# genome-vendor/bsmap

Measured on AMD Instinct MI355X. Metric: aligned reads/sec (whole node), 2x150 bp hg38 WGBS -v 6 -s 16, higher is better.
Workload: dtype u32; 1 GPU; C3: 2x150(->144) bp PE WGBS vs hg38-sized synthetic genome, -s 16 -v 6 -I 4 -m 28 -x 500; genome_bp=3088269832, index_entries=1475952693, parallelism=read-sharded x1, batches_in_flight=2, exact_mode=False, resident_ring_steps=4, records_flagged_BSX_F_LIMIT=0

## Files before the change

### bsmap_amd/csrc/bsx_align.hip

```cpp
#include "bsx_internal.h"
#include "bsx_dev.h"
#include "bsx_groups.h"
#include "bsx_rows.h"
#include "bsx_kernel_args.h"

namespace {

typedef unsigned long long u64;

struct __attribute__((packed, aligned(4))) U4 { uint32_t a, b, c, d; };
struct __attribute__((packed, aligned(4))) U2 { uint32_t a, b; };

#ifndef BSX_MAIN_NT
#define BSX_MAIN_NT 0
#endif
#ifndef BSX_MAIN_PREFETCH
#define BSX_MAIN_PREFETCH 1
#endif
typedef uint32_t v4u_a4 __attribute__((ext_vector_type(4), aligned(4)));
typedef uint32_t v2u_a4 __attribute__((ext_vector_type(2), aligned(4)));
__device__ __forceinline__ U4 ldm4(const uint32_t *p)
{
#if BSX_MAIN_NT
    const v4u_a4 v = __builtin_nontemporal_load(reinterpret_cast<const v4u_a4 *>(p));
    return U4{v.x, v.y, v.z, v.w};
#else
    return *reinterpret_cast<const U4 *>(p);
#endif
}
__device__ __forceinline__ U2 ldm2(const uint32_t *p)
{
#if BSX_MAIN_NT
    const v2u_a4 v = __builtin_nontemporal_load(reinterpret_cast<const v2u_a4 *>(p));
    return U2{v.x, v.y};
#else
    return *reinterpret_cast<const U2 *>(p);
#endif
}
__device__ __forceinline__ uint32_t ldm1(const uint32_t *p)
{
#if BSX_MAIN_NT
    return __builtin_nontemporal_load(p);
#else
    return *p;
#endif
}

__device__ __forceinline__ unsigned long long bsx_ballot(bool p) { return __builtin_amdgcn_ballot_w64(p); }
#define mad30(x, c) ({ uint32_t d_; asm("v_mad_u32_u24 %0, %1, 30, " #c : "=v"(d_) : "v"(x)); d_; })
__device__ __forceinline__ uint32_t rfl(uint32_t x) { return __builtin_amdgcn_readfirstlane(x); }
__device__ __forceinline__ uint32_t rl(uint32_t x, int l) { return __builtin_amdgcn_readlane(x, l); }
__device__ __forceinline__ uint32_t rl_u(uint32_t x, uint32_t l) { return __builtin_amdgcn_readlane(x, (int)__builtin_amdgcn_readfirstlane(l)); }
__device__ __forceinline__ u64 rl64(u64 x, int l) { return ((u64)rl((uint32_t)(x >> 32), l) << 32) | rl((uint32_t)x, l); }
__device__ __forceinline__ u64 lanemask_lt(int lane) { return lane ? (~0ull >> (64 - lane)) : 0ull; }
__device__ __forceinline__ void wave_fence() { __builtin_amdgcn_fence(__ATOMIC_SEQ_CST, "workgroup"); }

__device__ __forceinline__ int wave_argmin_u32(uint32_t v)
{
    uint32_t r = v;
#define BSX_DPP_MIN(ctrl) r = min(r, (uint32_t)__builtin_amdgcn_update_dpp((int)0xffffffffu, (int)r, ctrl, 0xf, 0xf, false))
    BSX_DPP_MIN(0x111); BSX_DPP_MIN(0x112); BSX_DPP_MIN(0x114); BSX_DPP_MIN(0x118);
#undef BSX_DPP_MIN
    const uint32_t m = min(min(rl(r, 15), rl(r, 31)), min(rl(r, 47), rl(r, 63)));
    return m == 0xffffffffu ? -1 : (int)__builtin_ctzll(bsx_ballot(v == m));
}
__device__ __forceinline__ uint32_t wave_sum(uint32_t v)
{
#pragma unroll
    for (int o = 32; o; o >>= 1) v += __shfl_xor(v, o);
    return v;
}

struct MateU {
    int len, raw_len, max_snp, seedseg, filtered;
    int nfull;
    uint32_t flags;
    uint32_t snp_thres;
    uint32_t nkeys;
    uint32_t index;
    int defer;
    uint32_t pad;
};
struct MateLds {
    uint8_t seq[160];
    uint8_t qual[160];
    uint32_t w[2][10], m[2][10];
    uint32_t cnt[2][160];
    uint8_t start[2][16];
    uint8_t order[2][16];
    uint32_t stale_key[2][16];
    uint8_t stale_so[2];
    MateU u, u2;
    __attribute__((aligned(16))) uint32_t fl[4][8];
};

template <bool PE> struct WaveLds { MateLds mate[PE ? 2 : 1]; };

struct BlockLds {
    uint8_t prof[16][16];
    uint8_t nt_tab[256];
    uint32_t anchor[BSX_LDS_CHR + 1], chr_size[BSX_LDS_CHR], rc_offset[BSX_LDS_CHR];
};

typedef __attribute__((address_space(3))) MateU LdsMateU;
struct Mate {
    LdsMateU *u;
    uint32_t cnt_reg;
    uint32_t key_reg;
    uint32_t bloom0, bloom1;
};
__device__ __forceinline__ LdsMateU *lds_mate(MateU *p) { return (LdsMateU *)p; }

struct Slab {
    u64 *hits;
    uint32_t *keys;
    uint32_t *kslot;
    uint32_t *hset;
    u64 *tmp;
    uint32_t rowcap, nclass;
    uint32_t kcap, hbits;
    __device__ __forceinline__ u64 *list(int orient, int w) const { return hits + ((size_t)(orient * (nclass + 1) + w)) * rowcap; }
};

struct Counters { u64 n_lookup, n_cand, sum_w, n_orient; };

__device__ __forceinline__ int nt_idx(uint32_t c)
{
    c |= 0x20;
    return c == 'a' ? 0 : c == 'c' ? 1 : c == 'g' ? 2 : c == 't' ? 3 : -1;
}

__device__ __forceinline__ uint32_t n_of(const Mate &M, int orient, int w) { return rl(M.cnt_reg, orient * 16 + w); }

__device__ void load_and_filter(const AlignArgs &A, MateLds &L, Mate &M, int mate, long j, int lane)
{
    const DevParams &P = A.P;
    const bool hist = j < 0;
    const uint64_t *off = hist ? A.hist_off[mate] : A.off[mate];
    const uint64_t jj = hist ? (uint64_t)((long)A.n_hist + j) : (uint64_t)j;
    const uint64_t b = off[jj], e = off[jj + 1];
    int len = (int)min((uint64_t)P.max_readlen, e - b);
    const uint8_t *sq = hist ? A.hist_seq[mate] : A.seq[mate], *qq = hist ? A.hist_qual[mate] : A.qual[mate];
    const uint8_t *s = sq + b, *q = qq ? qq + b : nullptr;
    for (int i = lane; i < 160; i += 64) {
        L.seq[i] = i < len ? s[i] : 0;
        L.qual[i] = (q && i < len) ? q[i] : 0;
    }
    wave_fence();
    M.u->raw_len = len;
    M.u->filtered = 0;
    if (P.n_adapter > 0 && len >= 5) {
        bool done = false;
        for (int a = 0; a < P.n_adapter && !done; a++) {
            const int al = P.adapter_len[a];
            for (int base = P.seed_size; base < len - (P.rrbs ? 5 : 4) && !done; base += 64) {
                const int pos = base + lane;
                bool hit = false;
// ... 2152 lines not shown
    uint32_t *bits = g_sector_bits;
    if (!bits) return;
    uint32_t prev = 0xffffffffu, touches = 0;
    for (int i = 0; i < n16; i++)
        for (uint32_t b = byte_off + 16u * (uint32_t)i; b <= byte_off + 16u * (uint32_t)i + 15u; b += 15u) {
            const uint32_t sct = b >> 6;
            if (sct == prev) continue;
            prev = sct; touches++;
            if (!((bits[sct >> 5] >> (sct & 31u)) & 1u)) atomicOr(&bits[sct >> 5], 1u << (sct & 31u));
        }
    const unsigned long long tw = (unsigned long long)wave_sum(touches);
    if ((threadIdx.x & 63) == 0) atomicAdd(&g_sector_touch, tw);
}
__global__ __launch_bounds__(256) void k_sector_pop(uint32_t n_words)
{
    unsigned long long c = 0;
    for (uint32_t i = blockIdx.x * 256 + threadIdx.x; i < n_words; i += gridDim.x * 256) { const uint32_t w = g_sector_bits[i]; if (w) { c += (unsigned long long)__popc(w); g_sector_bits[i] = 0; } }
    for (int o = 32; o; o >>= 1) c += __shfl_xor(c, o);
    if ((threadIdx.x & 63) == 0 && c) atomicAdd(&g_sector_distinct, c);
    if (blockIdx.x == 0 && threadIdx.x == 0) atomicAdd(&g_sector_passes, 1ull);
}
#endif

template <bool RRBS, int XP = 0>
__device__ __forceinline__ SameChunk same_load(const SameWin &W, const SameEntry &e)
{
    static_assert(XP >= 0 && XP <= 2, "r3 holds two pairs");
    SameChunk c;
    uint32_t off = W.ref_off;
    if (RRBS) {
        const uint32_t rchr = e.a & 0xffffu;
        c.valid = e.in && ((e.a ^ W.tag_xor) >> 16) == W.tag_want && e.b >= W.h;
        c.pm1 = c.valid ? W.anchor[rchr >> 1] + (e.b - W.h) - 1u : 31u;
        c.strand = rchr & 1u;
        off = c.strand ? W.rc_off : 0u;
    } else { c.valid = e.in; c.pm1 = e.a + W.h - 1u; c.strand = 0; }
    const uint8_t *src = W.plane + hp_boff(c.pm1, off);
    c.r0 = *reinterpret_cast<const U4 *>(src);
    c.r1.a = c.r1.b = c.r1.c = c.r1.d = 0; c.r2.a = c.r2.b = c.r2.c = c.r2.d = 0;
    if (W.nwr > 1) c.r1 = *reinterpret_cast<const U4 *>(src + 16);
    if (W.nwr > 3) c.r2 = *reinterpret_cast<const U4 *>(src + 32);
    c.r3.a = c.r3.b = c.r3.c = c.r3.d = 0;
    if (XP == 1) { const U2 x = *reinterpret_cast<const U2 *>(src + 48); c.r3.a = x.a; c.r3.b = x.b; }
    if (XP == 2) c.r3 = *reinterpret_cast<const U4 *>(src + 48);
#ifdef BSX_SECTOR_STATS
    if (c.valid) sector_mark(hp_boff(c.pm1, off), W.nwr > 3 ? 3 : W.nwr > 1 ? 2 : 1); else sector_mark(0u, 0);
#endif
    return c;
}

template <int NWR, bool PLAIN, bool SKIP, bool STATS>
__device__ __forceinline__ void same_counts(const uint32_t (&flo)[5], const uint32_t (&fhi)[5], uint32_t him, int nwr_rt, const uint4 &a0, const uint4 &a1, const uint4 &a2,
                                            const uint4 &a3, uint32_t thr, u64 alive, uint32_t &w0ref, uint32_t &w01ref, uint32_t &tot)
{
    static_assert(NWR != 0 || !PLAIN, "the plain form needs the word count");
    const int nwr = NWR ? NWR : nwr_rt;
#define SAME_MM(j, X, Y, M) ((PLAIN && (j) < NWR - 1) ? bsx_plane_mismatch_full(flo[j], fhi[j], X, Y) : bsx_plane_mismatch(flo[j], fhi[j], X, Y, M))
    const uint32_t m0 = SAME_MM(0, a0.x, a0.y, a0.z);
    const uint32_t c0 = __popc(m0);
    w0ref = STATS ? __popc(m0 & him) : 0u; tot = c0; w01ref = c0;
    if (nwr > 1) {
        const uint32_t m1 = SAME_MM(1, a0.w, a1.x, a1.y);
        tot = popc_acc(m1, c0); if (STATS) w01ref = popc_acc(m1 & him, c0);
        if (nwr > 2 && (!SKIP || (bsx_ballot(tot <= thr) & alive))) {
            tot = popc_acc(SAME_MM(2, a1.z, a1.w, a2.x), tot);
            if (nwr > 3) {
                tot = popc_acc(SAME_MM(3, a2.z, a2.w, a3.x), tot);
                if (nwr > 4) tot = popc_acc(SAME_MM(4, a3.y, a3.z, a3.w), tot);
            }
        }
    }
#undef SAME_MM
}

template <bool PLAIN>
__device__ __forceinline__ uint32_t same_word(int j, const uint32_t (&flo)[5], const uint32_t (&fhi)[5], const uint4 &a0, const uint4 &a1, const uint4 &a2, const uint4 &a3)
{
    uint32_t X, Y, M;
    switch (j) {
    case 0: X = a0.x; Y = a0.y; M = a0.z; break;
    case 1: X = a0.w; Y = a1.x; M = a1.y; break;
    case 2: X = a1.z; Y = a1.w; M = a2.x; break;
    case 3: X = a2.z; Y = a2.w; M = a3.x; break;
    default: X = a3.y; Y = a3.z; M = a3.w; break;
    }
    return (PLAIN && j < 4) ? bsx_plane_mismatch_full(flo[j], fhi[j], X, Y) : bsx_plane_mismatch(flo[j], fhi[j], X, Y, M);
}
template <bool PLAIN, bool FULL>
__device__ __forceinline__ u64 same_exit(const uint32_t (&flo)[5], const uint32_t (&fhi)[5], const uint4 &a0, const uint4 &a1, const uint4 &a2, const uint4 &a3,
                                         uint32_t thr, u64 valid, uint32_t &tot, uint32_t &words)
{
    u64 bp = 0;
    tot = 0;
#define SAME_STEP(i, j)                                                                \
    tot = popc_acc(same_word<PLAIN>(j, flo, fhi, a0, a1, a2, a3), tot);                \
    words = (i) + 1;                                                                   \
    if ((i) == 4 || ((HG_EXIT >> (i)) & 1)) {                                          \
        bp = bsx_ballot(tot <= thr);                                                   \
        if (!FULL) bp &= valid;                                                        \
        if (!bp) return 0;                                                             \
    }
    SAME_STEP(0, 0) SAME_STEP(1, 4) SAME_STEP(2, 3) SAME_STEP(3, 2) SAME_STEP(4, 1)
#undef SAME_STEP
    return bp;
}

template <int NWR, bool RRBS, bool PLAIN, bool FULL, bool STATS>
__device__ __forceinline__ void hs_eval_read(const uint32_t (&flo)[HG_C][5], const uint32_t (&fhi)[HG_C][5], const uint32_t (&him)[HG_C], const u64 (&vm)[HG_C],
                                             const uint32_t (&ordsh)[HG_C], const uint32_t (&hchr)[HG_C], const uint32_t (&hloc)[HG_C], int nwr, const uint4 &a0, const uint4 &a1,
                                             const uint4 &a2, const uint4 &a3, uint32_t thr, SurvRec *sv, uint32_t &nsk, uint32_t &add15)
{
#pragma unroll
    for (int u = 0; u < HG_C; u++) {
        uint32_t w0ref = 0, w01ref = 0, tot;
        u64 bp;
        if (HG_EXIT && !STATS && !RRBS && NWR == 5) {
            uint32_t words;
            bp = same_exit<PLAIN, FULL>(flo[u], fhi[u], a0, a1, a2, a3, thr, vm[u], tot, words);
#ifdef BSX_SCAN_WORDS
            if (vm[u]) add15 += 1u + (words << 16);
#else
            (void)words;
#endif
        } else {
            same_counts<NWR, PLAIN, RRBS, STATS>(flo[u], fhi[u], him[u], nwr, a0, a1, a2, a3, thr, vm[u], w0ref, w01ref, tot);
            bp = bsx_ballot(tot <= thr);
            if (!FULL) bp &= vm[u];
        }
        if (STATS) {
            u64 b1 = bsx_ballot(w0ref > thr), b5 = bsx_ballot(w01ref <= thr);
            if (!FULL) { b1 &= vm[u]; b5 &= vm[u]; }
            add15 += (uint32_t)__builtin_popcountll(b1) + ((uint32_t)__builtin_popcountll(b5) << 16);
        }
        if (bp) {
            const uint32_t pos = __builtin_amdgcn_mbcnt_hi((uint32_t)(bp >> 32), __builtin_amdgcn_mbcnt_lo((uint32_t)bp, nsk));
            if (__builtin_amdgcn_inverse_ballot_w64(bp) && pos < HS_SCAP) { SurvRec r; r.w_ord = tot | ordsh[u]; r.hchr = hchr[u]; r.hloc = hloc[u]; r.hkey = 0; sv[pos] = r; }
            nsk += (uint32_t)__builtin_popcountll(bp);
        }
    }
}

template <bool PLAIN, bool SPLIT>
__device__ __forceinline__ uint32_t lean_word(int i, const uint32_t (&flo)[5], const uint32_t (&fhi)[5], const uint4 &q0, const uint4 &q1, const uint4 &q2, const uint4 &q3)
{
    const int j = bsx_row_eval_word(i);
    if (!SPLIT) return same_word<PLAIN>(j, flo, fhi, q0, q1, q2, q3);
    uint32_t X, Y, M;
    bsx_row_word(i, q0, q1, q2, q3, X, Y, M);
    return (PLAIN && j < 4) ? bsx_plane_mismatch_full(flo[j], fhi[j], X, Y) : bsx_plane_mismatch(flo[j], fhi[j], X, Y, M);
}
template <bool PLAIN, bool FULL, bool SPLIT, int JOINT>
__device__ __forceinline__ void hs_eval_lean(const HeavyArgs &H, const uint32_t (&flo)[HG_C][5], const uint32_t (&fhi)[HG_C][5], const u64 (&vm)[HG_C], const uint32_t (&hloc)[HG_C],
                                             const uint4 &q0, const uint4 &q1, const uint4 &p2, const uint4 &p3, const uint4 *row, uint32_t thr, uint32_t k, uint32_t tid, uint32_t &nsv,
                                             int lane, uint32_t cb, uint32_t dcur, uint32_t strand, uint32_t &dgw)
{
    u64 al[HG_C];
    uint32_t tot[HG_C];
    uint4 q2 = p2, q3 = p3;
#pragma unroll
    for (int u = 0; u < HG_C; u++) { al[u] = FULL ? ~0ull : vm[u]; tot[u] = 0; }
#ifdef BSX_SCAN_WORDS
#pragma unroll
    for (int u = 0; u < HG_C; u++) if (al[u]) dgw += 1u;
#define LEAN_DG dgw += 1u << 16;
#else
#define LEAN_DG
#endif
#define LEAN_WORD(u, i) {                                                                                \
        tot[u] = popc_acc(lean_word<PLAIN, SPLIT>(i, flo[u], fhi[u], q0, q1, q2, q3), tot[u]);           \
        const u64 b_ = bsx_ballot(tot[u] <= thr);                                                        \
        al[u] = (FULL && JOINT < 2) ? b_ : (b_ & al[u]);                                                 \
        LEAN_DG }
#define LEAN_ANY() (al[0] | al[1] | al[2] | al[3])
#define LEAN_HALF() asm volatile("" : "+v"(q2.x), "+v"(q2.y), "+v"(q2.z), "+v"(q2.w), "+v"(q3.x), "+v"(q3.y), "+v"(q3.z), "+v"(q3.w));
    static_assert(HG_C == 4, "written out for four chunks");
    if (JOINT == 3 && FULL) {
#pragma unroll
        for (int i = 0; i < 5; i++) {
            if (SPLIT && i == 2) { q2 = row[2]; q3 = row[3]; LEAN_HALF() }
#pragma unroll
            for (int u = 0; u < HG_C; u++) { tot[u] = popc_acc(lean_word<PLAIN, SPLIT>(i, flo[u], fhi[u], q0, q1, q2, q3), tot[u]); LEAN_DG }
            if (HG_JOINT_FIRST && i == 0) continue;
            if (!bsx_ballot(min(min(tot[0], tot[1]), min(tot[2], tot[3])) <= thr)) return;
        }
#pragma unroll
        for (int u = 0; u < HG_C; u++) al[u] = bsx_ballot(tot[u] <= thr);
    } else if (JOINT) {
#pragma unroll
        for (int i = 0; i < 5; i++) {
            if (SPLIT && i == 2) { q2 = row[2]; q3 = row[3]; LEAN_HALF() }
#pragma unroll
            for (int u = 0; u < HG_C; u++) if (JOINT >= 2 || al[u]) LEAN_WORD(u, i)
            if (HG_JOINT_FIRST && i == 0) continue;
            if (!LEAN_ANY()) return;
        }
    } else {
#pragma unroll
        for (int u = 0; u < HG_C; u++) if (al[u]) { LEAN_WORD(u, 0) if (al[u]) LEAN_WORD(u, 1) }
        if (!LEAN_ANY()) return;
        if (SPLIT) { q2 = row[2]; q3 = row[3]; LEAN_HALF() }
#pragma unroll
        for (int u = 0; u < HG_C; u++) if (al[u]) { LEAN_WORD(u, 2) if (al[u]) { LEAN_WORD(u, 3) if (al[u]) LEAN_WORD(u, 4) } }
        if (!LEAN_ANY()) return;
    }
#undef LEAN_WORD
#undef LEAN_ANY
#undef LEAN_HALF
#undef LEAN_DG
    SurvRec *const sv = H.tout[rl_u(tid, k)].surv;
    uint32_t nsk = rl_u(nsv, k);
#pragma unroll
    for (int u = 0; u < HG_C; u++) {
        const u64 bp = al[u];
        if (bp) {
            const uint32_t pos = __builtin_amdgcn_mbcnt_hi((uint32_t)(bp >> 32), __builtin_amdgcn_mbcnt_lo((uint32_t)bp, nsk));
            if (__builtin_amdgcn_inverse_ballot_w64(bp) && pos < HS_SCAP) {
                SurvRec r; r.w_ord = tot[u] | ((cb + (uint32_t)(u * 64 + lane)) << 8); r.hchr = strand; r.hloc = hloc[u] + 32u * dcur; r.hkey = 0; sv[pos] = r;
            }
            nsk += (uint32_t)__builtin_popcountll(bp);
        }
    }
    if ((uint32_t)lane == k) nsv = nsk;
}

template <int NWR, bool RRBS, bool STATS>
__device__ __forceinline__ void hs_group(const AlignArgs &A, const HeavyArgs &H, SameLds &L, int lane, int wv, uint32_t K, uint32_t tid, uint32_t th, uint32_t tc0,
                                         uint32_t key, uint32_t n, uint32_t hh, uint32_t sub_h, uint32_t flags, uint32_t tag_xor, uint32_t tag_want)
{
    const DevParams &P = A.P;
    uint32_t *uw = &L.W[wv].UW[0][0];
    const int nwr = NWR ? NWR : (int)((flags >> 8) & 15u);
    constexpr int XD = (!RRBS && NWR == 5) ? HG_D : 0, XP = XD;
    static_assert(HG_D >= 0 && HG_D <= 2 && 6 + HG_D <= BSX_PLANE_PAD, "the gather holds two pairs more at most, and stays inside the pad behind the strand copy");
    constexpr bool LEAN = HG_LEAN && HG_EXIT == 15 && NWR == 5 && !RRBS && !STATS, SPLIT = LEAN && HG_SPLIT;
    static_assert(BSX_ROW_DWORDS == 20 && sizeof(L.W[0].UW[0]) == 4 * BSX_ROW_DWORDS, "bsx_rows.h describes a row of SameLds");
#ifdef BSX_SIGHIST_DUPS
    u64 rowsig = 0;
#endif
#ifdef BSX_SCAN_CLOCKS
    constexpr bool CLK = NWR == 5 && !RRBS && !STATS;
    u64 ck_gather = 0, ck_reads = 0;
    const u64 ck_begin = __builtin_amdgcn_s_memtime();
#endif
    if ((uint32_t)lane < K) {
        const ListReq &R = H.state[th & 0x3fffffffu].req[th >> 30];
        uint32_t *row = uw + (uint32_t)lane * 20u;
        uint32_t inner = 0xFFFFFFFFu;
#pragma unroll
        for (int j = 0; j < 5; j++) {
            const int f = 3 * j, o = j < 3 ? 0 : 1;
            const uint32_t pm = R.pm[j];
            if (!SPLIT) { row[f + o] = R.px[j]; row[f + 1 + o] = R.py[j]; row[f + 2 + o] = pm; }
            if (j < nwr - 1) inner &= pm;
        }
        const uint32_t tword = R.thres | (inner == 0xFFFFFFFFu ? 0x10000u : 0u) | (XD ? ((sub_h - hh) >> 5) << 17 : 0u);
        if (SPLIT) bsx_row_pack(row, R.px, R.py, R.pm, tword);
        else row[9] = tword;
        row[BSX_ROW_TASK] = tid; row[BSX_ROW_ORD] = tc0;
#ifdef BSX_SIGHIST_DUPS
        u64 hsh = R.thres;
#pragma unroll
        for (int j = 0; j < 5; j++) { hsh = (hsh ^ R.px[j]) * 0x9E3779B97F4A7C15ull; hsh = (hsh ^ R.py[j]) * 0xBF58476D1CE4E5B9ull; hsh = (hsh ^ R.pm[j]) * 0x94D049BB133111EBull; hsh ^= hsh >> 29; }
        rowsig = hsh;
#endif
    }
    uint32_t n_dup = 0; (void)n_dup;
#ifdef BSX_SIGHIST_DUPS
    for (uint32_t j = 1; j < K; j++) {
        const u64 sj = ((u64)rl_u((uint32_t)(rowsig >> 32), j) << 32) | rl_u((uint32_t)rowsig, j);
        if (bsx_ballot((uint32_t)lane < j && rowsig == sj)) n_dup++;
    }
#endif
    wave_fence();
    const uint32_t strand = flags & 1u;
    SameWin W;
    W.ent = P.entries + (RRBS ? 2u * (size_t)key : (size_t)key); W.n = n; W.h = hh; W.tag_xor = tag_xor; W.tag_want = tag_want; W.rc_off = P.plane_rc_off;
    W.ref_off = strand ? P.plane_rc_off : 0u; W.anchor = P.anchor; W.plane = reinterpret_cast<const uint8_t *>(P.refplane); W.nwr = nwr;
    uint32_t c15 = 0, nsv = 0;
    uint32_t n_cand = 0;
#ifdef BSX_SCAN_WORDS
    u64 dg_ev = 0, dg_words = 0;
#endif
    constexpr uint32_t STEP = 64u * HG_C;
    SameChunk nx[HG_C];
    SameEntry en[HG_C];
#if HG_PREFETCH
#pragma unroll
    for (int u = 0; u < HG_C; u++) nx[u] = same_load<RRBS, XP>(W, same_entry<RRBS>(W, (uint32_t)(u * 64 + lane)));
#pragma unroll
    for (int u = 0; u < HG_C; u++) en[u] = same_entry<RRBS>(W, STEP + (uint32_t)(u * 64 + lane));
#pragma unroll
    for (int u = 0; u < HG_C; u++) asm volatile("" :: "v"(nx[u].r0.a), "v"(nx[u].r1.a), "v"(nx[u].r2.a));
#else
#pragma unroll
    for (int u = 0; u < HG_C; u++) en[u] = same_entry<RRBS>(W, (uint32_t)(u * 64 + lane));
#endif
    for (uint32_t cb = 0; cb < n; cb += STEP) {
#ifdef BSX_SCAN_CLOCKS
        __builtin_amdgcn_sched_barrier(0);
        const u64 ck_step = __builtin_amdgcn_s_memtime();
        __builtin_amdgcn_sched_barrier(0);
#endif
#if !HG_PREFETCH
#pragma unroll
        for (int u = 0; u < HG_C; u++) nx[u] = same_load<RRBS, XP>(W, en[u]);
#pragma unroll
        for (int u = 0; u < HG_C; u++) en[u] = same_entry<RRBS>(W, cb + STEP + (uint32_t)(u * 64 + lane));
#endif
        uint32_t flo[HG_C][5], fhi[HG_C][5], xlo[HG_C][XD ? XD : 1], xhi[HG_C][XD ? XD : 1], him[HG_C], hloc[HG_C], ordsh[HG_C], hchr[HG_C];
        u64 vm[HG_C];
#pragma unroll
        for (int u = 0; u < HG_C; u++) {
            const SameChunk &c = nx[u];
            const uint32_t wd[16] = {c.r0.a, c.r0.b, c.r0.c, c.r0.d, c.r1.a, c.r1.b, c.r1.c, c.r1.d, c.r2.a, c.r2.b, c.r2.c, c.r2.d, c.r3.a, c.r3.b, c.r3.c, c.r3.d};
            const uint32_t shf = 31u - (c.pm1 & 31u);
            him[u] = 0xFFFFFFFFu << ((c.pm1 + 1u) & 15u);
#pragma unroll
            for (int t = 0; t < 5; t++) { flo[u][t] = __builtin_amdgcn_alignbit(wd[2 * t], wd[2 * t + 2], shf); fhi[u][t] = __builtin_amdgcn_alignbit(wd[2 * t + 1], wd[2 * t + 3], shf); }
#pragma unroll
            for (int t = 5; t < 5 + XD; t++) { xlo[u][t - 5] = __builtin_amdgcn_alignbit(wd[2 * t], wd[2 * t + 2], shf); xhi[u][t - 5] = __builtin_amdgcn_alignbit(wd[2 * t + 1], wd[2 * t + 3], shf); }
            if (!XD) xlo[u][0] = xhi[u][0] = 0;
            hloc[u] = c.pm1 + 1u;
            hchr[u] = RRBS ? c.strand : strand;
            ordsh[u] = (cb + (uint32_t)(u * 64 + lane)) << 8;
            vm[u] = bsx_ballot(c.valid);
            if (RRBS) n_cand += (uint32_t)__builtin_popcountll(vm[u]);
        }
#if HG_PREFETCH
        if (cb + STEP < n) {
#pragma unroll
            for (int u = 0; u < HG_C; u++) nx[u] = same_load<RRBS, XP>(W, en[u]);
#pragma unroll
            for (int u = 0; u < HG_C; u++) en[u] = same_entry<RRBS>(W, cb + 2u * STEP + (uint32_t)(u * 64 + lane));
        }
#endif
        const bool full = !RRBS && cb + STEP <= n;
#ifdef BSX_SCAN_CLOCKS
#pragma unroll
        for (int u = 0; u < HG_C; u++) asm volatile("" :: "v"(flo[u][0]), "v"(fhi[u][4]), "v"(xlo[u][XD ? XD - 1 : 0]), "v"(xhi[u][XD ? XD - 1 : 0]));
        __builtin_amdgcn_sched_barrier(0);
        const u64 ck_frame = __builtin_amdgcn_s_memtime();
        __builtin_amdgcn_sched_barrier(0);
        ck_gather += ck_frame - ck_step;
#endif
#if HG_ROWPF
        uint4 p0, p1, p2, p3 = make_uint4(0u, 0u, 0u, 0u);
        { const uint4 *row = reinterpret_cast<const uint4 *>(uw); p0 = row[0]; p1 = row[1]; p2 = row[2]; if (nwr > 3) p3 = row[3]; }
#endif
        uint32_t dcur = 0;
        if constexpr (LEAN) {
            const uint4 *const rows = reinterpret_cast<const uint4 *>(uw);
            const uint4 zero4 = make_uint4(0u, 0u, 0u, 0u);
            auto one_read = [&](uint32_t k, const uint4 &h0, const uint4 &h1) __attribute__((always_inline)) {
                const uint4 *const row = rows + k * 5u;
                uint4 q0 = h0, q1 = h1, p2 = zero4, p3 = zero4;
                if (!SPLIT) { q0 = row[0]; q1 = row[1]; p2 = row[2]; p3 = row[3]; }
                const uint32_t tp = rfl(SPLIT ? bsx_row_t(q0) : p2.y), thr = tp & 0xffffu;
                const bool plain = ((tp >> 16) & 1u) != 0;
                for (; dcur < (tp >> 17); dcur++) {
#pragma unroll
                    for (int u = 0; u < HG_C; u++) {
#pragma unroll
                        for (int t = 0; t < 4; t++) { flo[u][t] = flo[u][t + 1]; fhi[u][t] = fhi[u][t + 1]; }
                        flo[u][4] = xlo[u][0]; fhi[u][4] = xhi[u][0];
#pragma unroll
                        for (int t = 0; t + 1 < XD; t++) { xlo[u][t] = xlo[u][t + 1]; xhi[u][t] = xhi[u][t + 1]; }
                    }
                }
                uint32_t dgw = 0;
                if (full) {
                    if (plain) hs_eval_lean<true, true, SPLIT, HG_JOINT>(H, flo, fhi, vm, hloc, q0, q1, p2, p3, row, thr, k, tid, nsv, lane, cb, dcur, strand, dgw);
                    else hs_eval_lean<false, true, SPLIT, HG_JOINT>(H, flo, fhi, vm, hloc, q0, q1, p2, p3, row, thr, k, tid, nsv, lane, cb, dcur, strand, dgw);
                } else {
                    if (plain) hs_eval_lean<true, false, SPLIT, HG_JOINT>(H, flo, fhi, vm, hloc, q0, q1, p2, p3, row, thr, k, tid, nsv, lane, cb, dcur, strand, dgw);
                    else hs_eval_lean<false, false, SPLIT, HG_JOINT>(H, flo, fhi, vm, hloc, q0, q1, p2, p3, row, thr, k, tid, nsv, lane, cb, dcur, strand, dgw);
                }
#ifdef BSX_SCAN_WORDS
                dg_ev += dgw & 0xffffu; dg_words += dgw >> 16;
#else
                (void)dgw;
#endif
            };
            if (SPLIT) {
                uint4 a0 = rows[0], a1 = rows[1], b0, b1;
                for (uint32_t k = 0;; k += 2) {
                    { const uint4 *const nr = rows + min(k + 1u, K - 1u) * 5u; b0 = nr[0]; b1 = nr[1]; }
                    one_read(k, a0, a1);
                    if (k + 1 >= K) break;
                    { const uint4 *const nr = rows + min(k + 2u, K - 1u) * 5u; a0 = nr[0]; a1 = nr[1]; }
                    one_read(k + 1, b0, b1);
                    if (k + 2 >= K) break;
                }
            } else
                for (uint32_t k = 0; k < K; k++) one_read(k, zero4, zero4);
        } else
        for (uint32_t k = 0; k < K; k++) {
#if HG_ROWPF
            const uint4 a0 = p0, a1 = p1, a2 = p2, a3 = p3;
            if (k + 1 < K) { const uint4 *row = reinterpret_cast<const uint4 *>(uw + (k + 1u) * 20u); p0 = row[0]; p1 = row[1]; p2 = row[2]; if (nwr > 3) p3 = row[3]; }
#else
            const uint4 *row = reinterpret_cast<const uint4 *>(uw + k * 20u);
            const uint4 a0 = row[0], a1 = row[1], a2 = row[2];
            uint4 a3 = make_uint4(0u, 0u, 0u, 0u);
            if (nwr > 3) a3 = row[3];
#endif
            const uint32_t tp = rfl(a2.y), thr = tp & 0xffffu;
            const bool plain = NWR != 0 && ((tp >> 16) & 1u) != 0;
            if (XD) {
                for (; dcur < (tp >> 17); dcur++) {
#pragma unroll
                    for (int u = 0; u < HG_C; u++) {
#pragma unroll
                        for (int t = 0; t < 4; t++) { flo[u][t] = flo[u][t + 1]; fhi[u][t] = fhi[u][t + 1]; }
                        flo[u][4] = xlo[u][0]; fhi[u][4] = xhi[u][0];
#pragma unroll
                        for (int t = 0; t + 1 < XD; t++) { xlo[u][t] = xlo[u][t + 1]; xhi[u][t] = xhi[u][t + 1]; }
                        hloc[u] += 32u;
                    }
                }
            }
            SurvRec *const sv = H.tout[rl_u(tid, k)].surv;
            uint32_t nsk = rl_u(nsv, k), add15 = 0;
            if (full) {
                if (plain) hs_eval_read<NWR, RRBS, NWR != 0, !RRBS, STATS>(flo, fhi, him, vm, ordsh, hchr, hloc, nwr, a0, a1, a2, a3, thr, sv, nsk, add15);
                else hs_eval_read<NWR, RRBS, false, !RRBS, STATS>(flo, fhi, him, vm, ordsh, hchr, hloc, nwr, a0, a1, a2, a3, thr, sv, nsk, add15);
            } else {
                if (plain) hs_eval_read<NWR, RRBS, NWR != 0, false, STATS>(flo, fhi, him, vm, ordsh, hchr, hloc, nwr, a0, a1, a2, a3, thr, sv, nsk, add15);
                else hs_eval_read<NWR, RRBS, false, false, STATS>(flo, fhi, him, vm, ordsh, hchr, hloc, nwr, a0, a1, a2, a3, thr, sv, nsk, add15);
            }
            if ((uint32_t)lane == k) { if (STATS) c15 += add15; nsv = nsk; }
#ifdef BSX_SCAN_WORDS
            if (!STATS) { dg_ev += add15 & 0xffffu; dg_words += add15 >> 16; }
#endif
        }
#ifdef BSX_SCAN_CLOCKS
        asm volatile("" :: "v"(nsv));
        __builtin_amdgcn_sched_barrier(0);
        ck_reads += __builtin_amdgcn_s_memtime() - ck_frame;
        __builtin_amdgcn_sched_barrier(0);
#endif
    }
    wave_fence();
    if (!RRBS) n_cand = n;
    const bool mine = (uint32_t)lane < K;
    const uint32_t n1 = c15 & 0xffffu, n5 = c15 >> 16, ns = nsv;
    const bool ov = ns > HS_SCAP;
    if (mine) {
        HTaskOut *o = &H.tout[tid];
        o->count = min(ns, (uint32_t)HS_SCAP); o->overflow = ov ? 1 : 0; o->acc[0] = n_cand; o->acc[1] = STATS ? 2u * n_cand - n1 + 3u * n5 : 0u; o->acc[2] = 0; o->acc[3] = 0; o->c0 = tc0; o->n = n;
    }
    const bool cnt = mine && !ov;
    const uint32_t kk = (uint32_t)__builtin_popcountll(bsx_ballot(cnt));
    const uint32_t s1 = wave_sum(cnt ? n1 : 0), s5 = wave_sum(cnt ? n5 : 0);
    if (lane == 0 && kk) {
        u64 *sh = (u64 *)A.scan_stats + (size_t)((blockIdx.x * (uint32_t)HG_WPB + (uint32_t)wv) & 63u) * 8;
        atomicAdd((u64 *)&sh[0], (u64)kk * n_cand);
        if (STATS) { atomicAdd((u64 *)&sh[1], 2ull * kk * n_cand - s1 + 3ull * s5); atomicAdd((u64 *)&sh[2], (u64)s1); atomicAdd((u64 *)&sh[3], (u64)s5); }
        if (K > 1) atomicAdd((u64 *)&sh[4], (u64)kk * n_cand);
#if !defined(BSX_SCAN_WORDS) && !defined(BSX_SCAN_CLOCKS)
        atomicAdd((u64 *)&sh[5], (u64)kk * n_cand * K); if (K >= 4) atomicAdd((u64 *)&sh[6], (u64)kk * n_cand); if (n_dup) atomicAdd((u64 *)&sh[7], (u64)n_dup * n_cand);
#endif
    }
#ifdef BSX_SCAN_WORDS
    if (lane == 0 && dg_ev) {
        u64 *sh = (u64 *)A.scan_stats;
        atomicAdd((u64 *)&sh[5], dg_ev); atomicAdd((u64 *)&sh[6], dg_words);
    }
#endif
#ifdef BSX_SCAN_CLOCKS
    if (CLK && lane == 0) {
        u64 *sh = (u64 *)A.scan_stats;
        atomicAdd((u64 *)&sh[5], ck_gather); atomicAdd((u64 *)&sh[6], ck_reads); atomicAdd((u64 *)&sh[7], (u64)__builtin_amdgcn_s_memtime() - ck_begin);
    }
#endif
    wave_fence();
}

template <bool STATS>
__global__ __launch_bounds__(64 * HG_WPB, BSX_HSAME_WAVES) void k_hscan_same(AlignArgs A, HeavyArgs H)
{
    __shared__ SameLds L;
    const int lane = threadIdx.x & 63, wv = (int)rfl(threadIdx.x >> 6);
    const uint32_t n_big = min(H.glist[H.task_cap], H.task_cap), n_groups = min(n_big + H.glist[H.task_cap + 1], H.task_cap);
    const uint32_t nvb = (n_groups + HG_WPB - 1) / HG_WPB;
    for (uint32_t vb = blockIdx.x;; vb += gridDim.x) {
        uint32_t b_;
        const int st_ = bsx_order_block(vb, nvb, H.xcd_map >= 2 ? max(2u, H.xcd_map * BSX_HSCAN_WPB / (HG_XCD_DIV * HG_WPB)) : H.xcd_map, b_);
        if (st_ == 2) break;
        if (st_ == 1) continue;
        const uint32_t g = b_ * HG_WPB + (uint32_t)wv;
        if (g >= n_groups) continue;
        const uint32_t slot = rfl(H.glist[g < n_big ? g : H.task_cap - 1u - (g - n_big)]);
        const uint32_t K = rfl(H.ghead[slot]);
        uint32_t tid = 0, th = 0, tc0 = 0, tn = 0, key = 0, hh = 0, flags = 0, tx = 0, tw = 0;
        if ((uint32_t)lane < K) {
            tid = H.order[slot + lane];
            const HTask tk = H.tasks[tid];
            th = tk.h; tc0 = tk.c0; tn = tk.n; key = tk.key; hh = tk.sub_h; flags = tk.flags; tx = tk.pad[0]; tw = tk.pad[1];
        }
        const uint32_t n0 = rfl(tn), f0 = rfl(flags);
        if (n0 == 0) {
            if ((uint32_t)lane < K) { HTaskOut *o = &H.tout[tid]; o->count = 0; o->overflow = 0; o->acc[0] = o->acc[1] = o->acc[2] = o->acc[3] = 0; o->c0 = 0; o->n = 0; }
        } else if (f0 & 4u) {
            if (((f0 >> 8) & 15u) == 3u) hs_group<3, true, STATS>(A, H, L, lane, wv, K, tid, th, tc0, rfl(key), n0, rfl(hh), hh, f0, rfl(tx), rfl(tw));
            else hs_group<0, true, STATS>(A, H, L, lane, wv, K, tid, th, tc0, rfl(key), n0, rfl(hh), hh, f0, rfl(tx), rfl(tw));
        }
        else if (K > 1) {
            if (((f0 >> 8) & 15u) == 5u) hs_group<5, false, STATS>(A, H, L, lane, wv, K, tid, th, tc0, rfl(key), n0, rfl(hh), hh, f0, 0u, 0u);
            else if (((f0 >> 8) & 15u) == 4u) hs_group<4, false, STATS>(A, H, L, lane, wv, K, tid, th, tc0, rfl(key), n0, rfl(hh), hh, f0, 0u, 0u);
            else hs_group<0, false, STATS>(A, H, L, lane, wv, K, tid, th, tc0, rfl(key), n0, rfl(hh), hh, f0, 0u, 0u);
        }
        else hp_task<STATS>(A, H, rfl(tid), lane, L.W[wv].one.TAB, L.W[wv].one.PT, L.W[wv].one.Q);
        wave_fence();
    }
}

#ifndef HG_TILE
#define HG_TILE 1024u
#endif
#define HG_TILE_MAX 2048u
static_assert(HG_TILE >= 64u && HG_TILE <= HG_TILE_MAX && (HG_TILE & (HG_TILE - 1u)) == 0, "a power of two of whole waves");
__device__ __forceinline__ bool tg_less(const uint4 &a, const uint4 &b)
{
    if (a.x != b.x) return a.x < b.x;
    if (a.y != b.y) return a.y < b.y;
    if (a.z != b.z) return a.z < b.z;
    return a.w < b.w;
}
__device__ __forceinline__ bool tg_same_run(const HTask &a, const HTask &b)
{
    if (a.n == 0 || b.n == 0) return a.n == b.n;
    return (a.flags & 2u) && a.flags == b.flags && a.key == b.key && a.n == b.n && a.pad[0] == b.pad[0] && a.pad[1] == b.pad[1] && ((a.sub_h ^ b.sub_h) & 31u) == 0;
}
__global__ __launch_bounds__(256) void k_task_groups(const HTask *tasks, const uint32_t *n_tasks_ptr, uint32_t cap, uint32_t *order, uint32_t *ghead, uint32_t *glist, uint32_t D, uint32_t Rg,
                                                     uint32_t T, uint32_t big)
{
    extern __shared__ uint4 tg_lds[];
    uint4 *K = tg_lds;
    uint32_t *head = (uint32_t *)(K + T);
    u64 *brk = (u64 *)(head + T);
    uint32_t *cnt = (uint32_t *)(brk + HG_TILE_MAX / 64u);
    const int lane = threadIdx.x & 63;
    const uint32_t wv = threadIdx.x >> 6, n_ch = T >> 6;
    const uint32_t n_tasks = min(*n_tasks_ptr, cap);
    for (uint32_t s0 = blockIdx.x * T; s0 < n_tasks; s0 += gridDim.x * T) {
        const uint32_t nj = min(T, n_tasks - s0);
        for (uint32_t i = threadIdx.x; i < T; i += 256u) {
            uint4 k = make_uint4(0xffffffffu, 0xffffffffu, 0xffffffffu, 0xffffffffu);
            if (i < nj) {
                const uint32_t tid = order[s0 + i];
                const HTask tk = tasks[tid];
                if (tk.n == 0) k = make_uint4(0xffffffffu, 0xfffffffeu, 0u, tid);
                else {
                    uint32_t hs = tk.n * 0x9E3779B1u ^ tk.flags * 0x85EBCA6Bu ^ tk.pad[0] * 0xC2B2AE35u ^ tk.pad[1] * 0x27D4EB2Fu;
                    hs ^= hs >> 15; hs *= 0x2C1B3C6Du; hs ^= hs >> 13;
                    k = make_uint4(tk.key, (hs & ~31u) | (tk.sub_h & 31u), tk.sub_h ^ 0x80000000u, tid);
                }
            }
            K[i] = k;
        }
        __syncthreads();
        for (uint32_t kk = 2; kk <= T; kk <<= 1)
            for (uint32_t j = kk >> 1; j; j >>= 1) {
                for (uint32_t t = threadIdx.x; t < (T >> 1); t += 256u) {
                    const uint32_t i = 2u * t - (t & (j - 1u)), l = i + j;
                    const uint4 a = K[i], b = K[l];
                    if (tg_less(b, a) == ((i & kk) == 0)) { K[i] = b; K[l] = a; }
                }
                __syncthreads();
            }
        uint32_t info[HG_TILE_MAX / 256u];
#pragma unroll
        for (uint32_t m = 0; m < HG_TILE_MAX / 256u; m++) {
            const uint32_t c = wv + 4u * m, i = c * 64u + (uint32_t)lane;
            info[m] = 0;
            if (c >= n_ch) continue;
            bool start = false;
            if (i < nj) {
                const uint4 k = K[i];
                const HTask tk = tasks[k.w];
                start = true;
                if (i) {
                    const uint4 kp = K[i - 1u];
                    if (kp.x == k.x && kp.y == k.y) start = !tg_same_run(tasks[kp.w], tk);
                }
                const uint32_t Dg = (!(tk.flags & 4u) && ((tk.flags >> 8) & 15u) == 5u) ? D : 0u;
                if (start) info[m] = 1u | (tk.n == 0 ? 64u << 8 : !(tk.flags & 2u) ? 1u << 8 : Dg << 1 | Rg << 8);
            }
            const u64 bm = bsx_ballot(start);
            if (lane == 0) brk[c] = bm;
        }
        __syncthreads();
#pragma unroll
        for (uint32_t m = 0; m < HG_TILE_MAX / 256u; m++) {
            if (!info[m]) continue;
            const uint32_t i = (wv + 4u * m) * 64u + (uint32_t)lane;
            uint32_t c = i >> 6;
            u64 w = brk[c] & ~((2ull << (i & 63u)) - 1ull);
            while (!w && ++c < n_ch) w = brk[c];
            const uint32_t e = w ? c * 64u + (uint32_t)__builtin_ctzll(w) : nj;
            bsx_group_cut(&K[i].z, 4u, e - i, (info[m] >> 1) & 127u, info[m] >> 8, head + i, 1u);
        }
        __syncthreads();
        for (uint32_t c = wv; c < n_ch; c += 4u) {
            const uint32_t i = c * 64u + (uint32_t)lane, hd = i < nj ? head[i] : 0u;
            if (i < nj) { order[s0 + i] = K[i].w; ghead[s0 + i] = hd; }
            const u64 hb = bsx_ballot(hd >= big), hsm = bsx_ballot(hd != 0 && hd < big);
            if (lane == 0) { cnt[c] = (uint32_t)__builtin_popcountll(hb); cnt[32u + c] = (uint32_t)__builtin_popcountll(hsm); }
        }
        __syncthreads();
        if (threadIdx.x < 2u) {
            uint32_t *q = cnt + 32u * threadIdx.x, tot = 0;
            for (uint32_t c = 0; c < n_ch; c++) tot += q[c];
            uint32_t run = tot ? atomicAdd(&glist[cap + threadIdx.x], tot) : 0u;
            for (uint32_t c = 0; c < n_ch; c++) { const uint32_t v = q[c]; q[c] = run; run += v; }
        }
        __syncthreads();
        for (uint32_t c = wv; c < n_ch; c += 4u) {
            const uint32_t i = c * 64u + (uint32_t)lane, hd = i < nj ? head[i] : 0u;
            const u64 hb = bsx_ballot(hd >= big), hsm = bsx_ballot(hd != 0 && hd < big);
            if (hd >= big) glist[cnt[c] + (uint32_t)__builtin_popcountll(hb & lanemask_lt(lane))] = s0 + i;
            else if (hd != 0) glist[cap - 1u - (cnt[32u + c] + (uint32_t)__builtin_popcountll(hsm & lanemask_lt(lane)))] = s0 + i;
        }
        __syncthreads();
    }
}

#define HS_SHARE 16u
#ifndef BSX_HSHARED_W3
#define BSX_HSHARED_W3 1
#endif
#ifndef BSX_HSHARED_C2
#define BSX_HSHARED_C2 1
#endif
#ifndef BSX_HSHARED_WAVES
#define BSX_HSHARED_WAVES 5
#endif
struct SharedChunk { uint32_t wd[12]; uint32_t pm1, strand; bool valid; };

__device__ __forceinline__ U2 shared_entry(const U2 *__restrict__ ent2, uint32_t idx, bool in_range)
{
    U2 e; e.a = 0xFFFFFFFFu; e.b = 0;
    if (in_range) e = ent2[idx];
    return e;
}
template <int NWR, bool LDS_CHR>
__device__ __forceinline__ SharedChunk shared_gather(const U2 e, bool in_range, uint32_t h, uint32_t tag_xor, uint32_t tag_want, const uint32_t *anch_lds,
                                                     const uint32_t *__restrict__ anch_glb, const uint8_t *plane, uint32_t rc_off, int nwr)
{
    SharedChunk c;
    const uint32_t rchr = e.a & 0xffffu;
    c.valid = in_range && ((e.a ^ tag_xor) >> 16) == tag_want && e.b >= h;
    uint32_t an = 0;
    typedef __attribute__((address_space(3))) const uint32_t LdsU32;
    if (c.valid) an = LDS_CHR ? ((LdsU32 *)anch_lds)[rchr >> 1] : ldm1(anch_glb + (rchr >> 1));
    c.pm1 = c.valid ? an + (e.b - h) - 1u : 31u;
    c.strand = rchr & 1u;
    const uint32_t boff = c.valid ? hp_boff(c.pm1, c.strand ? rc_off : 0u) : 0u;
    const U4 r0 = *reinterpret_cast<const U4 *>(plane + boff);
    U4 r1, r2;
    r1.a = r1.b = r1.c = r1.d = 0; r2.a = r2.b = r2.c = r2.d = 0;
    if (c.valid && nwr > 1) r1 = *reinterpret_cast<const U4 *>(plane + boff + 16);
    if ((NWR == 0 || NWR > 3) && c.valid && nwr > 3) r2 = *reinterpret_cast<const U4 *>(plane + boff + 32);
    c.wd[0] = r0.a; c.wd[1] = r0.b; c.wd[2] = r0.c; c.wd[3] = r0.d; c.wd[4] = r1.a; c.wd[5] = r1.b; c.wd[6] = r1.c; c.wd[7] = r1.d;
    c.wd[8] = r2.a; c.wd[9] = r2.b; c.wd[10] = r2.c; c.wd[11] = r2.d;
    return c;
}

template <int NWR, bool PLAIN, bool STATS>
__device__ __forceinline__ void shared_eval(const HeavyArgs &H, const uint32_t *uw, uint32_t k, const uint32_t (&flo)[5], const uint32_t (&fhi)[5], uint32_t him, u64 vm, uint32_t ord,
                                            uint32_t strand, uint32_t hloc, int nwr, const uint4 &a0, const uint4 &a1, const uint4 &a2, const uint4 &a3, uint32_t thr, int lane,
                                            uint32_t &c15, uint32_t &nsv)
{
    uint32_t w0ref, w01ref, tot;
    same_counts<NWR, PLAIN, true, STATS>(flo, fhi, him, nwr, a0, a1, a2, a3, thr, vm, w0ref, w01ref, tot);
    const u64 bp = bsx_ballot(tot <= thr) & vm;
    if (STATS) {
        const u64 b1 = bsx_ballot(w0ref > thr) & vm, b5 = bsx_ballot(w01ref <= thr) & vm;
        const uint32_t add15 = (uint32_t)__builtin_popcountll(b1) | ((uint32_t)__builtin_popcountll(b5) << 16);
        if ((uint32_t)lane == k) c15 += add15;
    }
    if (bp) {
        const uint32_t base = rl_u(nsv, k);
        const uint32_t pos = base + (uint32_t)__builtin_popcountll(bp & lanemask_lt(lane));
        if (((bp >> lane) & 1) && pos < HS_SCAP) {
            SurvRec r; r.w_ord = tot | ord; r.hchr = strand; r.hloc = hloc; r.hkey = 0;
            H.tout[uw[k * 20u + 16u]].surv[pos] = r;
        }
        if ((uint32_t)lane == k) nsv += (uint32_t)__builtin_popcountll(bp);
    }
}

template <int NWR, bool STATS, bool LDS_CHR>
__device__ __forceinline__ void shared_window(const HeavyArgs &H, const uint32_t *uw, const U2 *ent2, uint32_t n, uint32_t h, uint32_t tx, uint32_t tw,
                                              const uint32_t *anch_lds, const uint32_t *anch_glb, const uint8_t *plane, uint32_t rc_off, int nwr, uint32_t K, int lane,
                                              uint32_t &c15, uint32_t &nsv, uint32_t &nv)
{
    constexpr int C = (NWR == 3 && !STATS && BSX_HSHARED_C2) ? 2 : 1;
    constexpr uint32_t STEP = 64u * C;
    SharedChunk cur[C], nxt[C];
    U2 en[C];
#pragma unroll
    for (int u = 0; u < C; u++) { const uint32_t i_ = (uint32_t)(u * 64 + lane); cur[u] = shared_gather<NWR, LDS_CHR>(shared_entry(ent2, i_, i_ < n), i_ < n, h, tx, tw, anch_lds, anch_glb, plane, rc_off, nwr); }
#pragma unroll
    for (int u = 0; u < C; u++) { const uint32_t i_ = STEP + (uint32_t)(u * 64 + lane); en[u] = shared_entry(ent2, i_, i_ < n); }
    asm volatile("" :: "v"(cur[C - 1].wd[NWR == 3 ? 7 : 11]), "v"(cur[0].wd[NWR == 3 ? 7 : 11]));
    for (uint32_t cb = 0; cb < n; cb += STEP) {
        const bool more = cb + STEP < n;
        if (more) {
#pragma unroll
            for (int u = 0; u < C; u++) { const uint32_t i_ = cb + STEP + (uint32_t)(u * 64 + lane); nxt[u] = shared_gather<NWR, LDS_CHR>(en[u], i_ < n, h, tx, tw, anch_lds, anch_glb, plane, rc_off, nwr); }
#pragma unroll
            for (int u = 0; u < C; u++) { const uint32_t i_ = cb + 2u * STEP + (uint32_t)(u * 64 + lane); en[u] = shared_entry(ent2, i_, i_ < n); }
        }
        uint32_t flo[C][5], fhi[C][5], him[C], ord[C];
        u64 vm[C];
#pragma unroll
        for (int u = 0; u < C; u++) {
            const uint32_t shf = 31u - (cur[u].pm1 & 31u);
            him[u] = 0xFFFFFFFFu << ((cur[u].pm1 + 1u) & 15u);
#pragma unroll
            for (int t = 0; t < 5; t++) { flo[u][t] = __builtin_amdgcn_alignbit(cur[u].wd[2 * t], cur[u].wd[2 * t + 2], shf); fhi[u][t] = __builtin_amdgcn_alignbit(cur[u].wd[2 * t + 1], cur[u].wd[2 * t + 3], shf); }
            nv += cur[u].valid ? 1u : 0u;
            ord[u] = (cb + (uint32_t)(u * 64 + lane)) << 8;
            vm[u] = bsx_ballot(cur[u].valid);
        }
        const uint4 *up = reinterpret_cast<const uint4 *>(uw);
        for (uint32_t k = 0; k < K; k++, up += 5) {
            if (NWR == 3) {
                const uint4 u0 = up[0], u1 = up[1];
                const uint32_t tp = rfl(u1.w), thr = tp & 0xffffu;
                const uint4 a2 = make_uint4(u1.z, 0u, 0u, 0u), a3 = make_uint4(0u, 0u, 0u, 0u);
                if (tp >> 16) {
                    const uint4 a0 = make_uint4(u0.x, u0.y, 0xFFFFFFFFu, u0.z), a1 = make_uint4(u0.w, 0xFFFFFFFFu, u1.x, u1.y);
#pragma unroll
                    for (int u = 0; u < C; u++) {
                        if (u && !vm[u]) continue;
                        shared_eval<NWR == 3 ? 3 : 0, NWR == 3, STATS>(H, uw, k, flo[u], fhi[u], him[u], vm[u], ord[u], cur[u].strand, cur[u].pm1 + 1u, nwr, a0, a1, a2, a3, thr, lane, c15, nsv);
                    }
                } else {
                    const uint4 u2 = up[2];
                    const uint4 a0 = make_uint4(u0.x, u0.y, u2.x, u0.z), a1 = make_uint4(u0.w, u2.y, u1.x, u1.y);
#pragma unroll
                    for (int u = 0; u < C; u++) {
                        if (u && !vm[u]) continue;
                        shared_eval<NWR == 3 ? 3 : 0, false, STATS>(H, uw, k, flo[u], fhi[u], him[u], vm[u], ord[u], cur[u].strand, cur[u].pm1 + 1u, nwr, a0, a1, a2, a3, thr, lane, c15, nsv);
                    }
                }
            } else {
                const uint4 a0 = up[0], a1 = up[1], a2 = up[2];
                uint4 a3 = make_uint4(0u, 0u, 0u, 0u);
                if (nwr > 3) a3 = up[3];
                const uint32_t thr = rfl(a2.y) & 0xffffu;
                shared_eval<0, false, STATS>(H, uw, k, flo[0], fhi[0], him[0], vm[0], ord[0], cur[0].strand, cur[0].pm1 + 1u, nwr, a0, a1, a2, a3, thr, lane, c15, nsv);
            }
        }
        if (more) {
#pragma unroll
            for (int u = 0; u < C; u++) cur[u] = nxt[u];
// ... 62 lines not shown
                UW[wv][k][at] = v;
            }
        }
        uint32_t c15 = 0, nsv = 0;
        wave_fence();
        const U2 *ent2 = reinterpret_cast<const U2 *>(P.entries) + key;
        uint32_t nv = 0;
        if (lds_chr) {
            if (BSX_HSHARED_W3 && nwr == 3) shared_window<3, STATS, true>(H, &UW[wv][0][0], ent2, n, h, tx, tw, ANCH, P.anchor, plane, rc_off, nwr, K, lane, c15, nsv, nv);
            else shared_window<0, STATS, true>(H, &UW[wv][0][0], ent2, n, h, tx, tw, ANCH, P.anchor, plane, rc_off, nwr, K, lane, c15, nsv, nv);
        } else {
            if (BSX_HSHARED_W3 && nwr == 3) shared_window<3, STATS, false>(H, &UW[wv][0][0], ent2, n, h, tx, tw, ANCH, P.anchor, plane, rc_off, nwr, K, lane, c15, nsv, nv);
            else shared_window<0, STATS, false>(H, &UW[wv][0][0], ent2, n, h, tx, tw, ANCH, P.anchor, plane, rc_off, nwr, K, lane, c15, nsv, nv);
        }
        wave_fence();
        const uint32_t n_cand = wave_sum(nv);
        {
            const bool mine = (uint32_t)lane < K;
            const uint32_t my_c0 = (uint32_t)__shfl((int)tc0, (int)min(i0 + (uint32_t)lane, 63u));
            const uint32_t ns = nsv, n1 = c15 & 0xffffu, n5 = c15 >> 16;
            const bool ov = ns > HS_SCAP;
            if (mine) {
                HTaskOut *o = &H.tout[UW[wv][lane][16]];
                o->count = min(ns, (uint32_t)HS_SCAP); o->overflow = ov ? 1 : 0; o->acc[0] = n_cand; o->acc[1] = STATS ? 2u * n_cand - n1 + 3u * n5 : 0u; o->acc[2] = 0; o->acc[3] = 0; o->c0 = my_c0; o->n = n;
            }
            const bool cnt = mine && !ov;
            const uint32_t kk = (uint32_t)__builtin_popcountll(bsx_ballot(cnt));
            const uint32_t s1 = wave_sum(cnt ? n1 : 0), s5 = wave_sum(cnt ? n5 : 0);
            st_cand += (u64)kk * n_cand;
            if (STATS) { st_n1 += s1; st_n5 += s5; st_words += 2ull * kk * n_cand - s1 + 3ull * s5; }
        }
        wave_fence();
        i0 += K;
    }
    if (lane == 0) {
        u64 *sh = (u64 *)A.scan_stats + (size_t)(blockIdx.x & 63u) * 8;
        atomicAdd((u64 *)&sh[0], st_cand); atomicAdd((u64 *)&sh[1], st_words); atomicAdd((u64 *)&sh[2], st_n1); atomicAdd((u64 *)&sh[3], st_n5);
    }
    wave_fence();
    }
}
}

#ifdef BSX_ALL_HITS_TU
void bsx_launch_align_ah(const AlignArgs &A, int paired, int grid_blocks, hipStream_t stream, const AllHitsArgs &X)
{
    const bool ctx = A.P.ctx && !A.work_counters && A.P.index_interval <= 4 && !A.P.rrbs;
    if (A.leak_exact && ctx) {
        if (paired) hipLaunchKernelGGL((k_align_ah<true, true, true>), dim3(grid_blocks), dim3(256), 0, stream, A, X);
        else hipLaunchKernelGGL((k_align_ah<false, true, true>), dim3(grid_blocks), dim3(256), 0, stream, A, X);
    } else if (A.leak_exact) {
        if (paired) hipLaunchKernelGGL((k_align_ah<true, true>), dim3(grid_blocks), dim3(256), 0, stream, A, X);
        else hipLaunchKernelGGL((k_align_ah<false, true>), dim3(grid_blocks), dim3(256), 0, stream, A, X);
    } else if (ctx) {
        if (paired) hipLaunchKernelGGL((k_align_ah<true, false, true>), dim3(grid_blocks), dim3(256), 0, stream, A, X);
        else hipLaunchKernelGGL((k_align_ah<false, false, true>), dim3(grid_blocks), dim3(256), 0, stream, A, X);
    } else if (paired) hipLaunchKernelGGL((k_align_ah<true, false>), dim3(grid_blocks), dim3(256), 0, stream, A, X);
    else hipLaunchKernelGGL((k_align_ah<false, false>), dim3(grid_blocks), dim3(256), 0, stream, A, X);
}
void bsx_launch_hctrl_ah(const AlignArgs &A, const HeavyArgsRaw &R, int paired, int grid_blocks, hipStream_t stream, const AllHitsArgs &X)
{
    const HeavyArgs H = typed(R);
    if (paired) hipLaunchKernelGGL(k_hctrl_ah<true>, dim3(grid_blocks), dim3(256), 0, stream, A, H, X);
    else hipLaunchKernelGGL(k_hctrl_ah<false>, dim3(grid_blocks), dim3(256), 0, stream, A, H, X);
}
#else

void bsx_launch_leak(const AlignArgs &A, int paired, int n_cu, bool with_meta, bool resolve, void *final_out, hipStream_t stream)
{
    const uint32_t n_stream = A.n_hist + A.n_units_all;
    if (with_meta) {
        const int g = (int)std::max<uint32_t>(1, std::min<uint32_t>((n_stream + 3) / 4, (uint32_t)n_cu * 8));
        if (paired) hipLaunchKernelGGL(k_leak_meta<true>, dim3(g), dim3(256), 0, stream, A);
        else hipLaunchKernelGGL(k_leak_meta<false>, dim3(g), dim3(256), 0, stream, A);
    }
    if (resolve) {
        const int g = (int)std::max<uint32_t>(1, std::min<uint32_t>((A.n_units - A.first_unit + 3) / 4, (uint32_t)n_cu * 8));
        if (paired) hipLaunchKernelGGL(k_leak_resolve<true>, dim3(g), dim3(256), 0, stream, A);
        else hipLaunchKernelGGL(k_leak_resolve<false>, dim3(g), dim3(256), 0, stream, A);
    }
    if (final_out) {
        if (paired) hipLaunchKernelGGL(k_leak_final<true>, dim3(2), dim3(64), 0, stream, A, (LeakState *)final_out);
        else hipLaunchKernelGGL(k_leak_final<false>, dim3(2), dim3(64), 0, stream, A, (LeakState *)final_out);
    }
}
size_t bsx_leakrec_bytes(void) { return sizeof(LeakRec); }
size_t bsx_leakstate_bytes(void) { return sizeof(LeakState); }
uint32_t bsx_leak_blk(void) { return LEAK_BLK; }

void bsx_launch_align(const AlignArgs &A, int paired, int grid_blocks, hipStream_t stream, const AllHitsArgs *ah)
{
    if (ah) { bsx_launch_align_ah(A, paired, grid_blocks, stream, *ah); return; }
    const bool ctx = A.P.ctx && !A.work_counters && A.P.index_interval <= 4 && !A.P.rrbs;
    if (A.leak_exact && ctx) {
        if (paired) hipLaunchKernelGGL((k_align<true, true, true>), dim3(grid_blocks), dim3(256), 0, stream, A);
        else hipLaunchKernelGGL((k_align<false, true, true>), dim3(grid_blocks), dim3(256), 0, stream, A);
    } else if (A.leak_exact) {
        if (paired) hipLaunchKernelGGL((k_align<true, true>), dim3(grid_blocks), dim3(256), 0, stream, A);
        else hipLaunchKernelGGL((k_align<false, true>), dim3(grid_blocks), dim3(256), 0, stream, A);
    } else if (A.P.ctx && !A.work_counters && A.P.index_interval <= 4 && !A.P.rrbs) {
        if (paired) hipLaunchKernelGGL((k_align<true, false, true>), dim3(grid_blocks), dim3(256), 0, stream, A);
        else hipLaunchKernelGGL((k_align<false, false, true>), dim3(grid_blocks), dim3(256), 0, stream, A);
    } else if (paired) hipLaunchKernelGGL((k_align<true, false>), dim3(grid_blocks), dim3(256), 0, stream, A);
    else hipLaunchKernelGGL((k_align<false, false>), dim3(grid_blocks), dim3(256), 0, stream, A);
}

void bsx_launch_hctrl(const AlignArgs &A, const HeavyArgsRaw &R, int paired, int grid_blocks, hipStream_t stream, const AllHitsArgs *ah)
{
    if (ah) { bsx_launch_hctrl_ah(A, R, paired, grid_blocks, stream, *ah); return; }
    const HeavyArgs H = typed(R);
    if (paired) hipLaunchKernelGGL(k_hctrl<true>, dim3(grid_blocks), dim3(256), 0, stream, A, H);
    else hipLaunchKernelGGL(k_hctrl<false>, dim3(grid_blocks), dim3(256), 0, stream, A, H);
}

void bsx_launch_hscan_shared(const AlignArgs &A, const HeavyArgsRaw &R, hipStream_t stream, uint32_t max_tasks)
{
    const HeavyArgs H = typed(R);
    const uint32_t jobs = ((max_tasks ? std::min(max_tasks, R.task_cap) : R.task_cap) + HS_SHARE - 1) / HS_SHARE;
    if (A.work_counters) hipLaunchKernelGGL(k_hscan_shared<true>, dim3(((jobs + 3) / 4 + 7u) & ~7u), dim3(256), 0, stream, A, H);
    else hipLaunchKernelGGL(k_hscan_shared<false>, dim3(((jobs + 3) / 4 + 7u) & ~7u), dim3(256), 0, stream, A, H);
}

void bsx_launch_hscan_same(const AlignArgs &A, const HeavyArgsRaw &R, hipStream_t stream, uint32_t max_tasks)
{
    const HeavyArgs H = typed(R);
    static const uint32_t grid_div = getenv("BSX_SAME_GRID_DIV") ? (uint32_t)std::max(1, atoi(getenv("BSX_SAME_GRID_DIV"))) : 4u;
    uint32_t blocks = ((max_tasks ? std::min(max_tasks, R.task_cap) : R.task_cap / grid_div) + HG_WPB - 1) / HG_WPB;
    blocks = (blocks + 7u) & ~7u;
    if (A.work_counters) hipLaunchKernelGGL(k_hscan_same<true>, dim3(blocks), dim3(64 * HG_WPB), 0, stream, A, H);
    else hipLaunchKernelGGL(k_hscan_same<false>, dim3(blocks), dim3(64 * HG_WPB), 0, stream, A, H);
}

uint32_t bsx_same_d_max(void) { return HG_D; }
uint32_t bsx_same_r_max(void) { return HG_R; }

void bsx_launch_hscan(const AlignArgs &A, const HeavyArgsRaw &R, hipStream_t stream, uint32_t max_tasks)
{
    const HeavyArgs H = typed(R);
    uint32_t blocks = ((max_tasks ? std::min(max_tasks, R.task_cap) : R.task_cap) + BSX_HSCAN_WPB - 1) / BSX_HSCAN_WPB;
    blocks = (blocks + 7u) & ~7u;
    if (A.work_counters) hipLaunchKernelGGL(k_hscan<true>, dim3(blocks), dim3(64 * BSX_HSCAN_WPB), 0, stream, A, H);
    else hipLaunchKernelGGL(k_hscan<false>, dim3(blocks), dim3(64 * BSX_HSCAN_WPB), 0, stream, A, H);
}

namespace {
#define BIN_CHUNK 2048u
#define BIN_LDS 2048u
__device__ __forceinline__ uint32_t task_bin(const HTask &tk, uint32_t shift, uint32_t n_bins, uint32_t spread)
{
    uint32_t bin = tk.key >> shift;
    if (spread && (tk.flags & 2u)) {
        const uint32_t span = tk.n >> shift;
        const uint32_t nb = span >= 16u ? 16u : span >= 8u ? 8u : span >= 4u ? 4u : span >= 2u ? 2u : 1u;
        const bool congruent = spread == 2u && !(tk.flags & 4u) && ((tk.flags >> 8) & 15u) == 5u;
        bin += (((congruent ? tk.sub_h & 31u : tk.sub_h) * 0x9E3779B1u) >> 28) & (nb - 1u);
    }
    return min(bin, n_bins - 1u);
}
__global__ __launch_bounds__(256) void k_task_bins(const HTask *tasks, const uint32_t *n_tasks_ptr, uint32_t cap, uint32_t shift, uint32_t n_bins, uint32_t spread, uint32_t *bins,
                                                    uint32_t *rank, uint32_t *zero_blk)
{
    __shared__ uint32_t hkey[BIN_LDS], hcnt[BIN_LDS];
    if (zero_blk && blockIdx.x == 0 && threadIdx.x < 3) zero_blk[threadIdx.x == 0 ? 0u : threadIdx.x == 1 ? BSX_HCNT_TASKS : BSX_HCNT_QUEUE] = 0;
    const uint32_t n = min(*n_tasks_ptr, cap);
    for (uint32_t chunk = blockIdx.x * 1024u; chunk < n; chunk += gridDim.x * 1024u) {
        for (uint32_t i = threadIdx.x; i < BIN_LDS; i += 256) { hkey[i] = 0xffffffffu; hcnt[i] = 0; }
        __syncthreads();
        uint32_t sl[4], lr[4];
#pragma unroll
        for (int k = 0; k < 4; k++) {
            const uint32_t i = chunk + (uint32_t)k * 256u + threadIdx.x;
            sl[k] = 0; lr[k] = 0;
            if (i < n) {
                const uint32_t bin = task_bin(tasks[i], shift, n_bins, spread);
                uint32_t slot = (bin * 0x9E3779B1u) >> 21;
                for (;;) {
                    const uint32_t prev = atomicCAS(&hkey[slot], 0xffffffffu, bin);
                    if (prev == 0xffffffffu || prev == bin) break;
                    slot = (slot + 1) & (BIN_LDS - 1);
                }
                sl[k] = slot; lr[k] = atomicAdd(&hcnt[slot], 1u);
            }
        }
        __syncthreads();
        for (uint32_t i = threadIdx.x; i < BIN_LDS; i += 256)
            if (hkey[i] != 0xffffffffu) hcnt[i] = atomicAdd(&bins[hkey[i]], hcnt[i]);
        __syncthreads();
#pragma unroll
        for (int k = 0; k < 4; k++) {
            const uint32_t i = chunk + (uint32_t)k * 256u + threadIdx.x;
            if (i < n) rank[i] = hcnt[sl[k]] + lr[k];
        }
        __syncthreads();
    }
}
__global__ __launch_bounds__(256) void k_bin_scan(const uint32_t *n_tasks_ptr, uint32_t *bins, uint32_t *bstart, uint32_t *chunk_tot, uint32_t n_bins, uint32_t *zero_word)
{
    __shared__ uint32_t part[256];
    if (zero_word && blockIdx.x == 0 && threadIdx.x < 2) zero_word[threadIdx.x] = 0;
    if (*n_tasks_ptr == 0) return;
    const uint32_t base = blockIdx.x * BIN_CHUNK + threadIdx.x * 8u;
    uint32_t v[8], sum = 0;
#pragma unroll
    for (int k = 0; k < 8; k++) { v[k] = base + k < n_bins ? bins[base + k] : 0u; sum += v[k]; }
    part[threadIdx.x] = sum;
    __syncthreads();
    for (uint32_t o = 1; o < 256; o <<= 1) {
        const uint32_t t = threadIdx.x >= o ? part[threadIdx.x - o] : 0u;
        __syncthreads();
        part[threadIdx.x] += t;
        __syncthreads();
    }
    uint32_t run = part[threadIdx.x] - sum;
#pragma unroll
    for (int k = 0; k < 8; k++) { if (base + k < n_bins) { bstart[base + k] = run; if (v[k]) bins[base + k] = 0; } run += v[k]; }
    if (threadIdx.x == 255) chunk_tot[blockIdx.x] = part[255];
}
__global__ __launch_bounds__(256) void k_task_order(const HTask *tasks, const uint32_t *n_tasks_ptr, uint32_t cap, uint32_t shift, uint32_t n_bins, uint32_t spread, const uint32_t *bstart,
                                                     const uint32_t *chunk_tot, uint32_t n_chunks, const uint32_t *rank, uint32_t *order)
{
    __shared__ uint32_t cstart[1024];
    const uint32_t n = min(*n_tasks_ptr, cap);
    if (n == 0) return;
    for (uint32_t i = threadIdx.x; i < 1024; i += 256) cstart[i] = i < n_chunks ? chunk_tot[i] : 0u;
    __syncthreads();
    for (uint32_t o = 1; o < 1024; o <<= 1) {
        uint32_t t[4];
        for (int k = 0; k < 4; k++) { const uint32_t i = threadIdx.x + 256 * k; t[k] = i >= o ? cstart[i - o] : 0u; }
        __syncthreads();
        for (int k = 0; k < 4; k++) cstart[threadIdx.x + 256 * k] += t[k];
        __syncthreads();
    }
    for (uint32_t i = blockIdx.x * 256 + threadIdx.x; i < n; i += gridDim.x * 256) {
        const uint32_t b = task_bin(tasks[i], shift, n_bins, spread), c = b / BIN_CHUNK;
        order[(c ? cstart[c - 1] : 0u) + bstart[b] + rank[i]] = i;
    }
}
}

uint32_t bsx_group_tile(uint32_t tile)
{
    uint32_t T = 64u;
    while (T < HG_TILE_MAX && T < (tile ? tile : HG_TILE)) T <<= 1;
    return T;
}
uint32_t bsx_bin_chunks(uint32_t n_bins) { return (n_bins + BIN_CHUNK - 1) / BIN_CHUNK; }

void bsx_launch_task_order(const HeavyArgsRaw &R, uint32_t shift, uint32_t n_bins, uint32_t *bins, uint32_t *bstart, uint32_t *chunk_tot, uint32_t *rank, uint32_t *order,
                           uint32_t *zero_blk, hipStream_t stream, uint32_t spread, bool groups, uint32_t same_d, uint32_t same_r, uint32_t tile, uint32_t big)
{
    const uint32_t grid = std::max(1u, std::min(512u, (R.task_cap + 255u) / 256u)), n_chunks = bsx_bin_chunks(n_bins);
    hipLaunchKernelGGL(k_task_bins, dim3(std::max(1u, std::min(256u, (R.task_cap + 1023u) / 1024u))), dim3(256), 0, stream, (const HTask *)R.tasks, R.n_tasks, R.task_cap, shift, n_bins, spread, bins, rank, zero_blk);
    hipLaunchKernelGGL(k_bin_scan, dim3(n_chunks), dim3(256), 0, stream, R.n_tasks, bins, bstart, chunk_tot, n_bins, groups ? R.glist + R.task_cap : (uint32_t *)nullptr);
    hipLaunchKernelGGL(k_task_order, dim3(grid), dim3(256), 0, stream, (const HTask *)R.tasks, R.n_tasks, R.task_cap, shift, n_bins, spread, bstart, chunk_tot, n_chunks, rank, order);
    if (groups) {
        const uint32_t T = bsx_group_tile(tile);
        const size_t lds = (size_t)T * 20u + HG_TILE_MAX / 64u * 8u + 64u * 4u;
        hipLaunchKernelGGL(k_task_groups, dim3(std::max(1u, std::min(1024u, (R.task_cap + T - 1u) / T))), dim3(256), lds, stream, (const HTask *)R.tasks, R.n_tasks, R.task_cap, order, rank, R.glist,
                           std::min<uint32_t>(same_d, HG_D), same_r ? std::min<uint32_t>(same_r, HG_R) : HG_R, T, big ? std::min<uint32_t>(big, HG_R + 1u) : HG_BIG);
    }
}

namespace {
__device__ __forceinline__ unsigned long long sig_of(const HTask &tk, bool with_h)
{
    unsigned long long x = ((unsigned long long)tk.key << 32) ^ ((unsigned long long)tk.n << 9) ^ (tk.flags & 1u) ^ (with_h ? (unsigned long long)tk.sub_h * 0x9E3779B97F4A7C15ull : 0ull);
    x ^= x >> 29; x *= 0xBF58476D1CE4E5B9ull; x ^= x >> 32;
    return x | 1ull;
}
__global__ __launch_bounds__(256) void k_sig_count(const HTask *tasks, const uint32_t *n_tasks_ptr, uint32_t cap, unsigned long long *tab, uint32_t mask, int with_h)
{
    const uint32_t n = min(*n_tasks_ptr, cap);
    for (uint32_t i = blockIdx.x * 256 + threadIdx.x; i < n; i += gridDim.x * 256) {
        const HTask tk = tasks[i];
        if (!tk.n || !(tk.flags & 2u)) continue;
        const unsigned long long sg = sig_of(tk, with_h != 0);
        for (uint32_t slot = (uint32_t)(sg >> 20) & mask;; slot = (slot + 1) & mask) {
            const unsigned long long prev = atomicCAS(&tab[2 * (size_t)slot], 0ull, sg);
            if (prev == 0ull || prev == sg) { atomicAdd(&tab[2 * (size_t)slot + 1], 1ull); break; }
        }
    }
}
__global__ __launch_bounds__(256) void k_sig_hist(const HTask *tasks, const uint32_t *n_tasks_ptr, uint32_t cap, const unsigned long long *tab, uint32_t mask, int with_h, unsigned long long *hist)
{
    const uint32_t n = min(*n_tasks_ptr, cap);
    for (uint32_t i = blockIdx.x * 256 + threadIdx.x; i < n; i += gridDim.x * 256) {
        const HTask tk = tasks[i];
        if (!tk.n) continue;
        uint32_t k = 31;
        if (tk.flags & 2u) {
            const unsigned long long sg = sig_of(tk, with_h != 0);
            uint32_t slot = (uint32_t)(sg >> 20) & mask, probes = 0;
            while (tab[2 * (size_t)slot] != sg && probes <= mask) { slot = (slot + 1) & mask; probes++; }
            if (probes <= mask) {
                const unsigned long long r = tab[2 * (size_t)slot + 1];
                k = r <= 1 ? 0u : 32u - (uint32_t)__builtin_clz((uint32_t)r - 1u);
            }
        }
        atomicAdd(&hist[k], (unsigned long long)tk.n);
        atomicAdd(&hist[32 + k], 1ull);
    }
}
__device__ __forceinline__ unsigned long long sigc_of(const HTask &tk)
{
    HTask t = tk; t.sub_h &= 31u;
    return sig_of(t, true);
}
__device__ __forceinline__ uint32_t sigc_class(const HTask &tk) { return (tk.sub_h ^ 0x80000000u) >> 5; }
__global__ __launch_bounds__(256) void k_sigc_min(const HTask *tasks, const uint32_t *n_tasks_ptr, uint32_t cap, unsigned long long *tab, uint32_t mask)
{
    const uint32_t n = min(*n_tasks_ptr, cap);
    for (uint32_t i = blockIdx.x * 256 + threadIdx.x; i < n; i += gridDim.x * 256) {
        const HTask tk = tasks[i];
        if (!tk.n || !(tk.flags & 2u)) continue;
        const unsigned long long sg = sigc_of(tk);
        for (uint32_t slot = (uint32_t)(sg >> 20) & mask;; slot = (slot + 1) & mask) {
            const unsigned long long prev = atomicCAS(&tab[2 * (size_t)slot], 0ull, sg);
            if (prev == 0ull || prev == sg) { atomicMax(&tab[2 * (size_t)slot + 1], (unsigned long long)(0x0fffffffu - sigc_class(tk))); break; }
        }
    }
}
__global__ __launch_bounds__(256) void k_sigc_count(const HTask *tasks, const uint32_t *n_tasks_ptr, uint32_t cap, unsigned long long *tab, uint32_t mask, uint32_t D, int pass, unsigned long long *hist)
{
    const uint32_t n = min(*n_tasks_ptr, cap);
    for (uint32_t i = blockIdx.x * 256 + threadIdx.x; i < n; i += gridDim.x * 256) {
        const HTask tk = tasks[i];
        if (!tk.n) continue;
        uint32_t k = 31;
        if (tk.flags & 2u) {
            const unsigned long long sg = sigc_of(tk);
            uint32_t slot = (uint32_t)(sg >> 20) & mask, probes = 0;
            while (tab[2 * (size_t)slot] != sg && probes <= mask) { slot = (slot + 1) & mask; probes++; }
            if (probes > mask) continue;
            const unsigned long long w = tab[2 * (size_t)slot + 1];
            const bool within = sigc_class(tk) - (0x0fffffffu - (uint32_t)(w & 0xffffffffull)) <= D;
            if (!pass) { if (within) atomicAdd(&tab[2 * (size_t)slot + 1], 1ull << 32); continue; }
            const uint32_t r = (uint32_t)(w >> 32);
            k = !within ? 30u : r <= 1 ? 0u : 32u - (uint32_t)__builtin_clz(r - 1u);
        }
        if (pass) { atomicAdd(&hist[k], (unsigned long long)tk.n); atomicAdd(&hist[32 + k], 1ull); }
    }
}
__global__ __launch_bounds__(256) void k_group_fetches(const HTask *tasks, uint32_t cap, const uint32_t *order, const uint32_t *ghead, const uint32_t *glist, unsigned long long *st)
{
    const uint32_t n_big = min(glist[cap], cap), n_groups = min(n_big + glist[cap + 1], cap);
    unsigned long long ev = 0, ch = 0;
    for (uint32_t g = blockIdx.x * 256 + threadIdx.x; g < n_groups; g += gridDim.x * 256) {
        const uint32_t slot = glist[g < n_big ? g : cap - 1u - (g - n_big)], n = tasks[order[slot]].n;
        ev += (unsigned long long)ghead[slot] * n; ch += (n + 63u) / 64u;
    }
    if (ev) { atomicAdd(&st[0], ev); atomicAdd(&st[1], ch); }
}
__global__ __launch_bounds__(256) void k_sigc_tiles(const HTask *tasks, const uint32_t *n_tasks_ptr, uint32_t cap, const uint32_t *order, unsigned long long *tab, uint32_t mask, uint32_t T, int pass, unsigned long long *st)
{
    const uint32_t n = min(*n_tasks_ptr, cap);
    for (uint32_t s = blockIdx.x * 256 + threadIdx.x; s < n; s += gridDim.x * 256) {
        const HTask tk = tasks[order[s]];
        if (!tk.n || !(tk.flags & 2u)) continue;
        const unsigned long long sg = sigc_of(tk);
        if (!pass) {
            for (uint32_t slot = (uint32_t)(sg >> 20) & mask;; slot = (slot + 1) & mask) {
                const unsigned long long prev = atomicCAS(&tab[2 * (size_t)slot], 0ull, sg);
                if (prev == 0ull || prev == sg) { atomicOr(&tab[2 * (size_t)slot + 1], 1ull << ((s / T) & 63u)); break; }
            }
            continue;
        }
        uint32_t slot = (uint32_t)(sg >> 20) & mask, probes = 0;
        while (tab[2 * (size_t)slot] != sg && probes <= mask) { slot = (slot + 1) & mask; probes++; }
        if (probes > mask) continue;
        const unsigned long long w = tab[2 * (size_t)slot + 1];
        atomicAdd(&st[2], (unsigned long long)tk.n);
        if (w & (w - 1ull)) atomicAdd(&st[3], (unsigned long long)tk.n);
    }
}
const int SIG_KINDS = 5;
unsigned long long *g_sig_tab = nullptr, *g_sig_hist = nullptr;
const uint32_t SIG_SLOTS = 1u << 23;
}

void bsx_sig_hist_pass(const HeavyArgsRaw &R, hipStream_t stream, bool groups, uint32_t tile)
{
    if (!g_sig_tab) {
        if (hipMalloc((void **)&g_sig_tab, (size_t)SIG_SLOTS * 16) != hipSuccess || hipMalloc((void **)&g_sig_hist, (SIG_KINDS * 64 + 4) * 8) != hipSuccess) { g_sig_tab = nullptr; return; }
        (void)hipMemsetAsync(g_sig_hist, 0, (SIG_KINDS * 64 + 4) * 8, stream);
    }
    for (int with_h = 0; with_h < 2; with_h++) {
        (void)hipMemsetAsync(g_sig_tab, 0, (size_t)SIG_SLOTS * 16, stream);
        hipLaunchKernelGGL(k_sig_count, dim3(1024), dim3(256), 0, stream, (const HTask *)R.tasks, R.n_tasks, R.task_cap, g_sig_tab, SIG_SLOTS - 1, with_h);
        hipLaunchKernelGGL(k_sig_hist, dim3(1024), dim3(256), 0, stream, (const HTask *)R.tasks, R.n_tasks, R.task_cap, g_sig_tab, SIG_SLOTS - 1, with_h, g_sig_hist + 64 * with_h);
    }
    for (int kind = 2; kind < SIG_KINDS; kind++) {
        const uint32_t D = kind == 2 ? 1u : kind == 3 ? 2u : 4u;
        (void)hipMemsetAsync(g_sig_tab, 0, (size_t)SIG_SLOTS * 16, stream);
        hipLaunchKernelGGL(k_sigc_min, dim3(1024), dim3(256), 0, stream, (const HTask *)R.tasks, R.n_tasks, R.task_cap, g_sig_tab, SIG_SLOTS - 1);
        for (int pass = 0; pass < 2; pass++)
            hipLaunchKernelGGL(k_sigc_count, dim3(1024), dim3(256), 0, stream, (const HTask *)R.tasks, R.n_tasks, R.task_cap, g_sig_tab, SIG_SLOTS - 1, D, pass, g_sig_hist + 64 * kind);
    }
    if (groups) {
        hipLaunchKernelGGL(k_group_fetches, dim3(1024), dim3(256), 0, stream, (const HTask *)R.tasks, R.task_cap, R.order, R.ghead, R.glist, g_sig_hist + 64 * SIG_KINDS);
        (void)hipMemsetAsync(g_sig_tab, 0, (size_t)SIG_SLOTS * 16, stream);
        for (int pass = 0; pass < 2; pass++)
            hipLaunchKernelGGL(k_sigc_tiles, dim3(1024), dim3(256), 0, stream, (const HTask *)R.tasks, R.n_tasks, R.task_cap, R.order, g_sig_tab, SIG_SLOTS - 1, bsx_group_tile(tile), pass, g_sig_hist + 64 * SIG_KINDS);
    }
}

bool bsx_sig_group_stats(unsigned long long st[4])
{
    return g_sig_tab && hipDeviceSynchronize() == hipSuccess && hipMemcpy(st, g_sig_hist + 64 * SIG_KINDS, 32, hipMemcpyDeviceToHost) == hipSuccess;
}

void bsx_sig_hist_report(void)
{
    if (!g_sig_tab) return;
    unsigned long long h[SIG_KINDS * 64];
    if (hipDeviceSynchronize() != hipSuccess || hipMemcpy(h, g_sig_hist, sizeof h, hipMemcpyDeviceToHost) != hipSuccess) return;
    static const char *const kind_name[SIG_KINDS] = {"", " and offset", " and offset mod 32, offset / 32 within 1 of the smallest", " and offset mod 32, offset / 32 within 2 of the smallest",
                                                     " and offset mod 32, offset / 32 within 4 of the smallest"};
    for (int with_h = 0; with_h < SIG_KINDS; with_h++) {
        unsigned long long tot = 0, tt = 0;
        for (int k = 0; k < 32; k++) { tot += h[64 * with_h + k]; tt += h[64 * with_h + 32 + k]; }
        fprintf(stderr, "[sighist] same window%s: candidates %llu tasks %llu\n", kind_name[with_h], tot, tt);
        for (int k = 0; k < 32; k++)
            if (h[64 * with_h + 32 + k])
                fprintf(stderr, "[sighist]   %s %-6u cand %.4f tasks %.4f\n", k == 31 ? "spanning" : k == 30 && with_h >= 2 ? "beyond" : "R <=", k == 31 || (k == 30 && with_h >= 2) ? 0u : 1u << k, (double)h[64 * with_h + k] / (double)std::max(1ull, tot), (double)h[64 * with_h + 32 + k] / (double)std::max(1ull, tt));
    }
    (void)hipMemset(g_sig_hist, 0, (SIG_KINDS * 64 + 4) * 8);
}

void bsx_sector_pass(const bsx_ref *r, hipStream_t stream)
{
#ifdef BSX_SECTOR_STATS
    const uint32_t n_words = (uint32_t)(((uint64_t)r->plane_rc_off * 2 / 64 + 31) / 32 + 64);
    static uint32_t *bits = nullptr;
    if (!bits) {
        if (hipMalloc((void **)&bits, (size_t)n_words * 4) != hipSuccess) return;
        (void)hipMemset(bits, 0, (size_t)n_words * 4);
        (void)hipMemcpyToSymbol(HIP_SYMBOL(g_sector_bits), &bits, sizeof(bits));
        return;
    }
    hipLaunchKernelGGL(k_sector_pop, dim3(1024), dim3(256), 0, stream, n_words);
#else
    (void)r; (void)stream;
#endif
}
void bsx_sector_report(void)
{
#ifdef BSX_SECTOR_STATS
    unsigned long long t = 0, d = 0, p = 0;
    if (hipDeviceSynchronize() != hipSuccess) return;
    (void)hipMemcpyFromSymbol(&t, HIP_SYMBOL(g_sector_touch), 8); (void)hipMemcpyFromSymbol(&d, HIP_SYMBOL(g_sector_distinct), 8); (void)hipMemcpyFromSymbol(&p, HIP_SYMBOL(g_sector_passes), 8);
    fprintf(stderr, "[sectors] group scan: %llu lane-sector touches, %llu distinct sectors summed over %llu scan launches (compulsory), ratio %.2f\n", t, d, p, d ? (double)t / (double)d : 0.0);
    const unsigned long long z = 0;
    (void)hipMemcpyToSymbol(HIP_SYMBOL(g_sector_touch), &z, 8); (void)hipMemcpyToSymbol(HIP_SYMBOL(g_sector_distinct), &z, 8); (void)hipMemcpyToSymbol(HIP_SYMBOL(g_sector_passes), &z, 8);
#endif
}

size_t bsx_hstate_bytes(void) { return sizeof(HState); }
size_t bsx_htask_bytes(void) { return sizeof(HTask); }
size_t bsx_htaskout_bytes(void) { return sizeof(HTaskOut); }

int bsx_align_occupancy(int paired)
{
    int nb = 0;
    hipError_t e = paired ? hipOccupancyMaxActiveBlocksPerMultiprocessor(&nb, k_align<true, false>, 256, 0)
                          : hipOccupancyMaxActiveBlocksPerMultiprocessor(&nb, k_align<false, false>, 256, 0);
    if (e != hipSuccess || nb < 1) nb = 2;
    return nb;
}

int bsx_hctrl_occupancy(int paired)
{
    int nb = 0;
    hipError_t e = paired ? hipOccupancyMaxActiveBlocksPerMultiprocessor(&nb, k_hctrl<true>, 256, 0) : hipOccupancyMaxActiveBlocksPerMultiprocessor(&nb, k_hctrl<false>, 256, 0);
    if (e != hipSuccess || nb < 1) nb = 1;
    return nb;
}
#endif
```

### bsmap_amd/csrc/bsx_api.hip

```cpp
#include <fcntl.h>
#include <sys/mman.h>
#include <sys/stat.h>
#include <unistd.h>
#include <time.h>

#include <cstdio>
#include <cstdlib>
#include <cstring>
#include <fstream>
#include <cmath>
#include <memory>
#include <utility>
#include <vector>

#include "bsx_devbuf.h"
#include "bsx_internal.h"
#include "bsx_kernel_args.h"

static int g_waves_per_cu = 0;
static int g_heavy_threshold = 0;

extern "C" int bsx_set_waves_per_cu(int w) { g_waves_per_cu = w; return BSX_OK; }
extern "C" int bsx_set_heavy_threshold(int t) { g_heavy_threshold = t < 0 ? 0 : t; return BSX_OK; }
static uint32_t heavy_threshold_for(const bsx_params &p) { return g_heavy_threshold > 0 ? (uint32_t)g_heavy_threshold : (p.rrbs ? 2048u : 32768u); }
// ... 68 lines not shown
}

extern "C" int bsx_ref_create_from_fasta(const bsx_params *p, const char *text, uint64_t n_bytes, int device, bsx_ref **out)
{
    if (!p || !text || !out) return BSX_ERR_ARG;
    int rc = check_device(device);
    if (rc) return rc;
    bsx_ref *r = new bsx_ref();
    r->P = *p; r->device = device;
    std::vector<uint32_t> refcat, crefcat;
    rc = bsx_pack_fasta_device(*p, text, n_bytes, *r);
    if (rc == BSX_OK) { r->packed_on_device = true; rc = r->n_chr == 0 ? BSX_ERR_IO : finish_ref_tables(r); }
    else if (rc == 1) {
        rc = bsx_pack_fasta(*p, text, n_bytes, *r, refcat, crefcat);
        if (rc == BSX_OK && r->n_chr == 0) rc = BSX_ERR_IO;
        if (rc == BSX_OK) rc = finish_ref_upload(r, refcat, crefcat);
    }
    if (rc == BSX_OK && p->rrbs) rc = bsx_index_build_rrbs(r, refcat, crefcat);
    if (rc == BSX_OK && hipDeviceSynchronize() != hipSuccess) rc = BSX_ERR_DEVICE;
    if (rc != BSX_OK) { bsx_ref_destroy(r); return rc; }
    *out = r;
    return BSX_OK;
}

extern "C" int bsx_ref_create_from_file(const bsx_params *p, const char *path, int device, bsx_ref **out)
{
    if (!path) return BSX_ERR_ARG;
    const int fd = ::open(path, O_RDONLY);
    if (fd < 0) { g_bsx_err = std::string("cannot open ") + path; return BSX_ERR_IO; }
    struct stat st;
    if (fstat(fd, &st) != 0 || st.st_size <= 0) { ::close(fd); g_bsx_err = std::string("cannot read ") + path; return BSX_ERR_IO; }
    void *m = mmap(nullptr, (size_t)st.st_size, PROT_READ, MAP_PRIVATE, fd, 0);
    ::close(fd);
    if (m == MAP_FAILED) { g_bsx_err = std::string("cannot map ") + path; return BSX_ERR_IO; }
    const int rc = bsx_ref_create_from_fasta(p, (const char *)m, (uint64_t)st.st_size, device, out);
    munmap(m, (size_t)st.st_size);
    return rc;
}

extern "C" void bsx_ref_destroy(bsx_ref *r)
{
    if (!r) return;
    (void)hipSetDevice(r->device);
    for (void *q : {(void *)r->d_refcat, (void *)r->d_refplane, (void *)r->d_anchor, (void *)r->d_chr_size, (void *)r->d_rc_offset,
                    (void *)r->d_bucket_off, (void *)r->d_bucket_nfwd, (void *)r->d_entries, (void *)r->d_ctx, (void *)r->d_sites, (void *)r->d_site_off, (void *)r->d_rrbs_goff, (void *)r->d_site_bin, (void *)r->d_site_bin_off})
        if (q) (void)hipFree(q);
    delete r;
}

extern "C" uint32_t bsx_ref_n_chr(const bsx_ref *r) { return r ? r->n_chr : 0; }
extern "C" int bsx_ref_packed_on_device(const bsx_ref *r) { return r && r->packed_on_device ? 1 : 0; }
extern "C" uint64_t bsx_ref_n_words(const bsx_ref *r) { return r ? r->n_words : 0; }
extern "C" uint32_t bsx_ref_n_blocks(const bsx_ref *r) { return r ? (uint32_t)r->blocks.size() : 0; }
extern "C" int bsx_ref_info(const bsx_ref *r, uint32_t *anchor, uint32_t *chr_size, uint32_t *rc_offset)
{
    if (!r) return BSX_ERR_ARG;
    if (anchor) memcpy(anchor, r->anchor.data(), r->anchor.size() * 4);
    if (chr_size) memcpy(chr_size, r->chr_size.data(), r->chr_size.size() * 4);
    if (rc_offset) memcpy(rc_offset, r->rc_offset.data(), r->rc_offset.size() * 4);
    return BSX_OK;
}
extern "C" const char *bsx_ref_chr_name(const bsx_ref *r, uint32_t c) { return (r && c < r->names.size()) ? r->names[c].c_str() : ""; }
extern "C" int bsx_ref_blocks(const bsx_ref *r, uint32_t *id, uint32_t *begin, uint32_t *end)
{
    if (!r) return BSX_ERR_ARG;
    for (size_t i = 0; i < r->blocks.size(); i++) { id[i] = r->blocks[i].id; begin[i] = r->blocks[i].begin; end[i] = r->blocks[i].end; }
    return BSX_OK;
}
extern "C" int bsx_ref_download_words(const bsx_ref *r, uint32_t *refcat, uint32_t *crefcat)
{
    if (!r) return BSX_ERR_ARG;
    HIP_TRY(hipSetDevice(r->device));
    if (refcat) HIP_TRY(hipMemcpy(refcat, r->d_refcat, r->n_words * 4, hipMemcpyDeviceToHost));
    if (crefcat) HIP_TRY(hipMemcpy(crefcat, r->d_crefcat, r->n_words * 4, hipMemcpyDeviceToHost));
    return BSX_OK;
}

extern "C" int bsx_index_build(bsx_ref *r)
{
    if (!r) return BSX_ERR_ARG;
    if (r->P.rrbs) return r->has_index ? BSX_OK : BSX_ERR_STATE;
    return bsx_index_build_wgbs(r);
}
extern "C" uint64_t bsx_index_n_entries(const bsx_ref *r) { return r ? r->n_entries : 0; }

extern "C" int bsx_ref_set_context(bsx_ref *r, int mode, uint64_t headroom_bytes)
{
    if (!r || mode < 0 || mode > 2) return BSX_ERR_ARG;
    r->ctx_mode = mode;
    r->ctx_headroom = headroom_bytes ? headroom_bytes : BSX_CTX_HEADROOM_DEFAULT;
    return BSX_OK;
}
extern "C" uint64_t bsx_ref_context_bytes(const bsx_ref *r) { return r ? r->ctx_bytes : 0; }
extern "C" int bsx_ref_drop_context(bsx_ref *r)
{
    if (!r) return BSX_ERR_ARG;
    if (r->n_batches > 0) { g_bsx_err = "the context table can only be dropped while no batch of the reference exists"; return BSX_ERR_STATE; }
    if (r->d_ctx) { HIP_TRY(hipSetDevice(r->device)); (void)hipFree(r->d_ctx); r->d_ctx = nullptr; r->ctx_bytes = 0; }
    return BSX_OK;
}
extern "C" int bsx_index_download(const bsx_ref *r, uint32_t *bucket_off, uint32_t *bucket_nfwd, uint32_t *entries)
{
    if (!r) return BSX_ERR_ARG;
    if (!r->has_index) return BSX_ERR_STATE;
    HIP_TRY(hipSetDevice(r->device));
    const size_t K = r->P.total_kmers;
    if (bucket_off) HIP_TRY(hipMemcpy(bucket_off, r->d_bucket_off, (K + 1) * 4, hipMemcpyDeviceToHost));
    if (bucket_nfwd) HIP_TRY(hipMemcpy(bucket_nfwd, r->d_bucket_nfwd, K * 4, hipMemcpyDeviceToHost));
    if (entries && r->n_entries) {
        if (r->P.rrbs && !r->rrbs_entries_host.empty()) memcpy(entries, r->rrbs_entries_host.data(), r->n_entries * 8);
        else HIP_TRY(hipMemcpy(entries, r->d_entries, r->n_entries * (r->P.rrbs ? 8 : 4), hipMemcpyDeviceToHost));
    }
    return BSX_OK;
}
extern "C" uint32_t bsx_ref_n_sites(const bsx_ref *r, uint32_t c) { return (r && c < r->sites.size()) ? (uint32_t)r->sites[c].size() : 0; }
extern "C" int bsx_ref_sites(const bsx_ref *r, uint32_t c, uint32_t *sites)
{
    if (!r || c >= r->sites.size()) return BSX_ERR_ARG;
    memcpy(sites, r->sites[c].data(), r->sites[c].size() * 4);
    return BSX_OK;
}

void bsx_fill_devparams(const bsx_ref *r, DevParams &d)
{
    const bsx_params &p = r->P;
    memset(&d, 0, sizeof(d));
    d.seed_size = p.seed_size; d.index_interval = p.index_interval; d.max_snp_num = p.max_snp_num; d.max_num_hits = p.max_num_hits;
    d.chains = p.chains; d.pairend = p.pairend; d.min_insert = p.min_insert; d.max_insert = p.max_insert;
    d.report_repeat_hits = p.report_repeat_hits; d.randseed = p.randseed; d.qual_threshold = p.qual_threshold; d.zero_qual = p.zero_qual;
    d.max_ns = p.max_ns; d.max_readlen = p.max_readlen; d.rrbs = p.rrbs; d.n_adapter = p.n_adapter;
    d.digest_len = (int)strlen(p.digest_site); d.digest_pos = p.digest_pos;
    d.seed_bits = p.seed_bits;
    d.bit_nt_packed = p.bit_nt[0] | (p.bit_nt[1] << 8) | (p.bit_nt[2] << 16) | ((uint32_t)p.bit_nt[3] << 24);
    memcpy(d.profile_a, p.profile_a, sizeof(d.profile_a));
    for (int i = 0; i < p.n_adapter; i++) {
        size_t l = strlen(p.adapter[i]);
        d.adapter_len[i] = (uint8_t)(l > 15 ? 15 : l);
        memcpy(d.adapter[i], p.adapter[i], d.adapter_len[i]);
    }
    memcpy(d.digest_site, p.digest_site, 16);
    d.n_chr = r->n_chr;
    d.refplane = r->d_refplane; d.plane_rc_off = r->plane_rc_off;
    d.refcat = r->d_refcat; d.crefcat = r->d_crefcat; d.anchor = r->d_anchor; d.chr_size = r->d_chr_size; d.rc_offset = r->d_rc_offset;
    d.bucket_off = r->d_bucket_off; d.bucket_nfwd = r->d_bucket_nfwd; d.entries = r->d_entries; d.ctx = r->d_ctx;
    d.sites = r->d_sites; d.site_off = r->d_site_off; d.rrbs_goff = r->d_rrbs_goff; d.site_bin = r->d_site_bin; d.site_bin_off = r->d_site_bin_off;
}

#define BSX_MAX_GROUPS 8
#define BSX_POLL_SLOTS 4

struct BatchKnobs {
    uint32_t kcap, heavy_kcap, bin_log2;
    int n_groups, chunk_passes, hctrl_blocks, same, work_counters;
    uint32_t xcd_map, tail_tasks, tail_grid_tasks, same_d, same_r, group_tile, group_big, spread;
    bool spread_set, trace, sig_hist, sector_stats, poison;
};
static long knob(const char *name, long dflt, long lo, long hi, bool *set = nullptr)
{
    const char *e = getenv(name);
    if (set) *set = e != nullptr;
    return e ? std::min(hi, std::max(lo, atol(e))) : dflt;
}
static BatchKnobs read_knobs()
{
    const long none = 0, any = 0x7fffffffL;
    BatchKnobs K;
    K.kcap = (uint32_t)knob("BSX_KCAP", 1 << 18, 64, any);
    K.heavy_kcap = (uint32_t)knob("BSX_HEAVY_KCAP", none, 64, any);
    K.bin_log2 = (uint32_t)knob("BSX_BIN_LOG2", none, 8, 21);
    K.n_groups = (int)knob("BSX_HEAVY_GROUPS", 1, 1, BSX_MAX_GROUPS);
    K.chunk_passes = (int)knob("BSX_HEAVY_CHUNK", 2, 1, 64);
    K.hctrl_blocks = (int)knob("BSX_HCTRL_BLOCKS", 1, 1, any);
    K.same = (int)knob("BSX_SAME", 1, -any, any);
    K.work_counters = knob("BSX_WORK_COUNTERS", 1, -any, any) != 0;
    K.xcd_map = (uint32_t)knob("BSX_XCD_MAP", 128, 0, any);
    K.tail_tasks = (uint32_t)knob("BSX_TAIL_TASKS", 16384, 0, any);
    K.tail_grid_tasks = (uint32_t)knob("BSX_TAIL_GRID", 4096, 64, any);
    K.same_d = (uint32_t)knob("BSX_SAME_D", (long)bsx_same_d_max(), 0, (long)bsx_same_d_max());
    K.same_r = (uint32_t)knob("BSX_SAME_R", (long)bsx_same_r_max(), 1, (long)bsx_same_r_max());
    K.group_tile = (uint32_t)knob("BSX_GROUP_TILE", none, 0, 0x7fffffffffffffffL);
    K.group_big = (uint32_t)knob("BSX_GROUP_BIG", none, 0, 0x7fffffffffffffffL);
    K.spread = (uint32_t)knob("BSX_SPREAD", none, -any - 1, any, &K.spread_set);
    K.trace = getenv("BSX_TRACE_HEAVY") != nullptr;
    K.sig_hist = getenv("BSX_SIGHIST") != nullptr;
    K.sector_stats = getenv("BSX_SECTOR_STATS") != nullptr;
    K.poison = getenv("BSX_POISON") != nullptr;
    return K;
}

struct bsx_batch {
    bsx_ref *ref = nullptr;
    BatchKnobs K = {};
    int paired = 0, debug = 0, has_qual = 0, leak_exact = 0, work_counters = 1;
    uint32_t n_hist = 0;
    DevBuf<uint8_t> d_hist_seq[2], d_hist_qual[2];
    DevBuf<uint64_t> d_hist_off[2];
    DevBuf<uint8_t> d_leak_rec;
    DevBuf<uint16_t> d_leak_meta[2];
    DevBuf<uint32_t> d_leak_blk;
    uint32_t leak_nblk = 0;
    DevBuf<uint8_t> d_leak_init, d_leak_final;
    bool leak_meta_valid = false, leak_has_init = false;
    uint32_t max_units = 0, n_units = 0, first_index = 0;
    DevStream stream;
    struct Group {
        DevStream s_ctrl;
        DevEvent ev_ctrl, ev_scan, ev_poll[BSX_POLL_SLOTS];
        DevBuf<uint32_t> d_bins, d_bstart, d_chunk_tot, d_rank, d_order, d_glist;
    } grp[BSX_MAX_GROUPS];
    int hctrl_blocks_per_cu = 1;
    uint32_t bin_shift = 0, n_bins = 1;
    DevEvent ev_sync, ev_wait;
    std::vector<DevEvent> scan_ev;
    size_t scan_ev_used = 0;
    DevEvent ev0, ev1;
    DevBuf<uint8_t> d_seq[2], d_qual[2];
    DevBuf<uint64_t> d_off[2];
    size_t seq_cap[2] = {0, 0};
    DevBuf<bsx_hit> d_hits;
    DevBuf<bsx_pair> d_pairs;
    DevBuf<bsx_class_counts> d_cc[2];
    DevBuf<uint16_t> d_npairs;
    DevBuf<uint8_t> d_scratch, d_dbg;
    DevBuf<uint32_t> d_cycles;
    DevBuf<uint32_t> d_heavy_list, d_heavy_count;
    struct Pools {
        DevBuf<uint8_t> hstate, hslabs, htasks, htout;
        DevBuf<uint32_t> hactive[2];
    } pool;
    DevBuf<uint32_t> d_hcnt;
    uint32_t hcap = 0, task_cap = 0;
    bool same_kernel = false;
    uint32_t spread = 0;
    uint32_t *h_pinned = nullptr;
    int n_cu = 0;
    uint32_t last_heavy = 0, last_heavy_iters = 0, last_redo = 0;
    size_t scratch_bytes = 0;
    DevBuf<uint32_t> d_queue;
    DevBuf<uint64_t> d_counters, d_scan_stats;
    uint64_t slab_bytes = 0, hslab_bytes = 0;
    DevBuf<uint32_t> d_redo;
    uint32_t rowcap = 0, kcap = 0, hkcap = 0;
    int grid_blocks = 0;
    std::vector<DevEvent> ctrl_ev;
    size_t ctrl_ev_used = 0;
    DevEvent ev_align;
    bool stage_timing = false;
    DevBuf<uint32_t> d_ah_pool;
    uint64_t ah_cap = 0;
    DevBuf<uint64_t> d_ah_ctl;
    DevBuf<bsx_span> d_ah_spans;
    uint32_t run_first = 0, run_units = 0;
    bool ah_ran = false;
    bool ran = false;
    bool counted = false;
    ~bsx_batch() { if (h_pinned) (void)hipHostFree(h_pinned); }
};

static hipError_t wait_event(hipEvent_t ev)
{
    for (int n = 0;; n++) {
        const hipError_t e = hipEventQuery(ev);
        if (e == hipSuccess) return hipSuccess;
        if (e != hipErrorNotReady) return e;
        (void)hipGetLastError();
        struct timespec ts = {0, n < 8 ? 50000L : 200000L};
        nanosleep(&ts, nullptr);
    }
}
static hipError_t stream_wait(bsx_batch *b)
{
    if (!b->ev_wait) return hipStreamSynchronize(b->stream);
    hipError_t e = hipEventRecord(b->ev_wait, b->stream);
    if (e != hipSuccess) return e;
    return wait_event(b->ev_wait);
}
static int grow_events(std::vector<DevEvent> &pool, size_t need)
{
    while (pool.size() < need) {
        DevEvent e;
        HIP_TRY(e.create());
        pool.push_back(std::move(e));
    }
    return BSX_OK;
}

static uint32_t key_cap(const bsx_params &p, const BatchKnobs &K, uint32_t rowcap) { return (p.rrbs && !p.pairend) ? K.kcap : (uint32_t)(p.max_snp_num + 2) * rowcap; }
static uint32_t hset_bits(const bsx_params &p) { return (p.rrbs && !p.pairend) ? 19u : (uint32_t)BSX_HSET_BITS; }
static uint32_t heavy_key_cap(const bsx_params &p, const BatchKnobs &K, uint32_t rowcap) { return K.heavy_kcap ? K.heavy_kcap : (uint32_t)(p.max_snp_num + 2) * rowcap; }

static uint64_t mate_bytes(const bsx_params &p, uint32_t rowcap, uint64_t kcap, uint64_t hbits)
{
    const uint64_t rows = (uint64_t)p.max_snp_num + 2;
    return 2 * rows * rowcap * 8 + 2 * kcap * 4 + ((uint64_t)4 << hbits) + (uint64_t)BSX_SORT_TMP * 8;
}
static uint64_t slab_size(const bsx_params &p, int paired, uint32_t rowcap, uint64_t kcap, uint64_t hbits)
{
    const uint64_t mate = mate_bytes(p, rowcap, kcap, hbits);
    uint64_t s = mate;
    if (paired) s = 2 * mate + (2 * (uint64_t)p.max_snp_num + 2) * rowcap * 24;
    return (s + 255) & ~255ull;
}

static void init_shape(bsx_batch &b, const bsx_params &P, uint32_t max_units, int paired)
{
    b.K = read_knobs();
    b.paired = paired ? 1 : 0; b.max_units = max_units; b.work_counters = b.K.work_counters;
    b.rowcap = BSX_ROWCAP;
    b.kcap = key_cap(P, b.K, b.rowcap); b.hkcap = heavy_key_cap(P, b.K, b.rowcap);
    b.slab_bytes = slab_size(P, b.paired, b.rowcap, b.kcap, hset_bits(P));
    b.hslab_bytes = slab_size(P, b.paired, b.rowcap, b.hkcap, BSX_HSET_BITS);
    b.same_kernel = P.rrbs ? b.K.same == 2 : b.K.same != 0;
    b.spread = b.K.spread_set ? b.K.spread : (b.same_kernel ? (b.K.same_d ? 2u : 1u) : 0u);
}

struct PlanRow {
    uint64_t bytes;
    void *buf;
    hipError_t (*reserve)(void *, size_t);
    void (*reset)(void *);
    template <class T>
    PlanRow(DevBuf<T> &b, uint64_t n, bool wanted = true)
        : bytes(n), buf(wanted ? &b : nullptr), reserve([](void *q, size_t k) { return ((DevBuf<T> *)q)->reserve(k); }), reset([](void *q) { ((DevBuf<T> *)q)->reset(); }) {}
};
typedef std::vector<PlanRow> PlanRows;
static uint64_t rows_bytes(const PlanRows &rows) { uint64_t s = 0; for (const PlanRow &r : rows) s += r.bytes; return s; }
static void rows_reset(const PlanRows &rows) { for (const PlanRow &r : rows) if (r.buf) r.reset(r.buf); }
static hipError_t rows_alloc(const PlanRows &rows)
{
    for (const PlanRow &r : rows) {
        const hipError_t e = r.buf ? r.reserve(r.buf, (size_t)r.bytes) : hipSuccess;
        if (e != hipSuccess) return e;
    }
    return hipSuccess;
}

struct BatchPlan {
    PlanRows per_unit;
    PlanRows pools;
    PlanRows fixed;
    uint64_t scratch_bytes = 0;
    uint32_t hcap = 0, task_cap = 0, n_bins = 1, bin_shift = 0;
    int grid_blocks = 0;
};
#define BSX_PINNED_BYTES 1024

static PlanRows pool_rows(bsx_batch &b, uint32_t hcap, uint32_t task_cap, uint32_t n_bins)
{
    const int n_groups = b.K.n_groups;
    const uint64_t tcap = task_cap / (uint32_t)n_groups;
    PlanRows rows = {{b.pool.hstate, (uint64_t)hcap * bsx_hstate_bytes()}, {b.pool.hslabs, (uint64_t)hcap * b.hslab_bytes},
                     {b.pool.htasks, (uint64_t)task_cap * bsx_htask_bytes()}, {b.pool.htout, (uint64_t)task_cap * bsx_htaskout_bytes()},
                     {b.pool.hactive[0], (uint64_t)hcap * 4}, {b.pool.hactive[1], (uint64_t)hcap * 4}};
    for (int g = 0; g < n_groups; g++) {
        bsx_batch::Group &q = b.grp[g];
        rows.insert(rows.end(), {{q.d_bins, (uint64_t)n_bins * 4}, {q.d_bstart, (uint64_t)n_bins * 4}, {q.d_chunk_tot, (uint64_t)bsx_bin_chunks(n_bins) * 4},
                                 {q.d_rank, tcap * 4}, {q.d_order, tcap * 4},
                                 {q.d_glist, (tcap + 4) * 4, b.same_kernel}});
    }
    return rows;
}
static void default_pools(const bsx_params &P, uint64_t hslab, uint32_t units, uint32_t &hcap, uint32_t &task_cap)
{
    const uint64_t slab_budget = P.rrbs ? (40ull << 30) : (26ull << 30);
    uint64_t hc = std::min<uint64_t>(262144, std::max<uint64_t>(24576, slab_budget / hslab));
    if (!P.rrbs) hc = std::max<uint64_t>(hc, std::min<uint64_t>((uint64_t)units / 100, (64ull << 30) / hslab));
    hcap = (uint32_t)std::min<uint64_t>(units, hc);
    uint32_t task_default = P.rrbs ? 2u * 1048576u : 1048576u;
    if (!P.rrbs) task_default = (uint32_t)std::min<uint64_t>(1ull << 22, std::max<uint64_t>(task_default, (uint64_t)units / 2));
    task_cap = std::min<uint32_t>(task_default, std::max<uint32_t>(4096u, 64u * hcap));
}
extern "C" int bsx_default_heavy_limits(const bsx_params *p, uint32_t units, int paired, uint32_t *units_per_round, uint32_t *task_pool)
{
    if (!p || !units || !units_per_round || !task_pool) return BSX_ERR_ARG;
    default_pools(*p, slab_size(*p, paired ? 1 : 0, BSX_ROWCAP, heavy_key_cap(*p, read_knobs(), BSX_ROWCAP), BSX_HSET_BITS), units, *units_per_round, *task_pool);
    return BSX_OK;
}

static BatchPlan plan_batch(bsx_batch &b, const bsx_params &P, uint64_t n_entries, int n_cu, int blocks_per_cu)
{
    BatchPlan pl;
    const uint64_t mu = b.max_units;
    int grid = n_cu * std::min(8, std::max(1, blocks_per_cu));
    const int need = (int)((b.max_units + 3) / 4);
    if (grid > need) grid = need > 0 ? need : 1;
    pl.grid_blocks = grid;
    pl.scratch_bytes = (b.debug ? mu : (uint64_t)grid * 4) * b.slab_bytes;
    for (int m = 0; m < (b.paired ? 2 : 1); m++)
        pl.per_unit.insert(pl.per_unit.end(), {{b.d_seq[m], mu * 160 + 256}, {b.d_qual[m], mu * 160 + 256}, {b.d_off[m], (mu + 1) * 8}, {b.d_cc[m], mu * sizeof(bsx_class_counts)}});
    if (b.paired) pl.per_unit.insert(pl.per_unit.end(), {{b.d_pairs, mu * sizeof(bsx_pair)}, {b.d_npairs, mu * 64}});
    else pl.per_unit.push_back({b.d_hits, mu * sizeof(bsx_hit)});
    pl.per_unit.insert(pl.per_unit.end(), {{b.d_heavy_list, (mu + 1) * 4}, {b.d_redo, (mu + 1) * 4}});
    static_assert(BSX_N_COUNTERS <= 24, "the diagnostic clocks start at word 24");
    pl.fixed = {{b.d_queue, 256}, {b.d_counters, 24 * 8 + 256}, {b.d_scan_stats, 64 * 64}, {b.d_heavy_count, 256}, {b.d_hcnt, (uint64_t)BSX_MAX_GROUPS * 2 * BSX_HCNT_BLOCK * 4}};
    if (g_user_limits) { pl.hcap = std::min<uint32_t>(b.max_units, g_hcap); pl.task_cap = g_task_cap; }
    else default_pools(P, b.hslab_bytes, b.max_units, pl.hcap, pl.task_cap);
    const uint64_t ne = std::max<uint64_t>(1, n_entries);
    const uint32_t bin_log2 = b.K.bin_log2 ? b.K.bin_log2 : (P.rrbs ? 20u : 21u);
    while (((ne >> pl.bin_shift) + 1) > (1u << bin_log2)) pl.bin_shift++;
    pl.n_bins = (uint32_t)(ne >> pl.bin_shift) + 1;
    pl.pools = pool_rows(b, pl.hcap, pl.task_cap, pl.n_bins);
    return pl;
}

static uint64_t g_pool_reserve = 0;
extern "C" int bsx_set_pool_reserve(uint64_t bytes) { g_pool_reserve = bytes; return BSX_OK; }

extern "C" int bsx_batch_plan_bytes(const bsx_params *p, uint32_t max_units, int paired, uint64_t n_entries, uint32_t n_cu, uint32_t blocks_per_cu, uint64_t *out3)
{
    if (!p || !out3 || max_units == 0 || n_cu == 0) return BSX_ERR_ARG;
    bsx_batch shape;
    init_shape(shape, *p, max_units, paired);
    const BatchPlan pl = plan_batch(shape, *p, n_entries, (int)n_cu, (int)blocks_per_cu);
    out3[0] = rows_bytes(pl.per_unit); out3[1] = pl.scratch_bytes; out3[2] = rows_bytes(pl.pools);
    return BSX_OK;
}

static int plan_on_device(bsx_batch *b, BatchPlan &pl)
{
    hipDeviceProp_t prop;
    HIP_TRY(hipGetDeviceProperties(&prop, b->ref->device));
    int blocks_per_cu = bsx_align_occupancy(b->paired);
    if (g_waves_per_cu > 0) blocks_per_cu = std::max(1, std::min(blocks_per_cu, g_waves_per_cu / 4));
    b->n_cu = prop.multiProcessorCount;
    pl = plan_batch(*b, b->ref->P, b->ref->n_entries, b->n_cu, blocks_per_cu);
    b->grid_blocks = pl.grid_blocks;
    return BSX_OK;
}

static int ensure_scratch(bsx_batch *b, const BatchPlan &pl)
{
    if (pl.scratch_bytes <= b->scratch_bytes) return BSX_OK;
    b->d_scratch.reset();
    HIP_TRY(b->d_scratch.reserve((size_t)pl.scratch_bytes));
    HIP_TRY(hipMemsetAsync(b->d_scratch, 0, (size_t)pl.scratch_bytes, b->stream));
    b->scratch_bytes = (size_t)pl.scratch_bytes;
    return BSX_OK;
}

static int fit_pools(bsx_batch *b, const BatchPlan &pl)
{
    b->hcap = pl.hcap; b->task_cap = pl.task_cap;
    b->bin_shift = pl.bin_shift; b->n_bins = pl.n_bins;
    const uint64_t reserve = g_pool_reserve ? g_pool_reserve : ((4ull << 30) + pl.scratch_bytes + rows_bytes(pl.per_unit));
    for (int attempt = 0;; attempt++) {
        size_t fr = 0, tot = 0;
        const bool smallest = b->hcap <= std::min<uint32_t>(1024u, b->max_units) && b->task_cap <= 4096;
        const PlanRows rows = pool_rows(*b, b->hcap, b->task_cap, b->n_bins);
        hipError_t e = hipErrorOutOfMemory;
        if (smallest || hipMemGetInfo(&fr, &tot) != hipSuccess || rows_bytes(rows) + reserve <= fr) {
            e = rows_alloc(rows);
            if (e == hipSuccess) break;
            rows_reset(rows);
        }
        if (e != hipErrorOutOfMemory || attempt == 12 || smallest) return bsx_hip_fail(e, "hipMalloc (work pools of the heavy pipeline)", __FILE__, __LINE__);
        (void)hipGetLastError();
        b->hcap = std::min<uint32_t>(b->hcap, std::max<uint32_t>(std::min<uint32_t>(1024u, b->max_units), b->hcap / 2));
        b->task_cap = std::min<uint32_t>(b->task_cap, std::max<uint32_t>(4096u, b->task_cap / 2));
    }
    if (b->K.trace) fprintf(stderr, "[bsx] batch %p: pools for %u deferred units per round, %u scan tasks (planned %u / %u)\n", (void *)b, b->hcap, b->task_cap, pl.hcap, pl.task_cap);
    if (b->K.poison) HIP_TRY(hipMemsetAsync(b->pool.hstate, 0xA5, (size_t)b->hcap * bsx_hstate_bytes(), b->stream));
    HIP_TRY(hipMemsetAsync(b->pool.hslabs, 0, (size_t)b->hcap * b->hslab_bytes, b->stream));
    if (b->K.poison) {
        HIP_TRY(hipMemsetAsync(b->pool.htout, 0xA5, (size_t)b->task_cap * bsx_htaskout_bytes(), b->stream));
        HIP_TRY(hipMemsetAsync(b->pool.htasks, 0xA5, (size_t)b->task_cap * bsx_htask_bytes(), b->stream));
    }
// ... 146 lines not shown

extern "C" int bsx_batch_set_history(bsx_batch *b, uint32_t n, const char *seqs_a, const uint64_t *off_a, const char *quals_a, const char *seqs_b,
                                     const uint64_t *off_b, const char *quals_b)
{
    if (!b || n > 65536) return BSX_ERR_ARG;
    if (n && (!seqs_a || !off_a || (b->paired && (!seqs_b || !off_b)))) return BSX_ERR_ARG;
    HIP_TRY(hipSetDevice(b->ref->device));
    HIP_TRY(stream_wait(b));
    const char *sq[2] = {seqs_a, seqs_b}, *ql[2] = {quals_a, quals_b};
    const uint64_t *of[2] = {off_a, off_b};
    for (int m = 0; m < (b->paired ? 2 : 1); m++) {
        b->d_hist_seq[m].reset(); b->d_hist_qual[m].reset(); b->d_hist_off[m].reset();
        if (!n) continue;
        if (of[m][0] != 0) { g_bsx_err = "off[0] must be 0"; return BSX_ERR_ARG; }
        const uint64_t bytes = of[m][n];
        HIP_TRY(b->d_hist_seq[m].reserve(bytes + 256));
        HIP_TRY(b->d_hist_off[m].reserve(((size_t)n + 1) * 8));
        HIP_TRY(hipMemcpy(b->d_hist_seq[m], sq[m], bytes, hipMemcpyHostToDevice));
        HIP_TRY(hipMemcpy(b->d_hist_off[m], of[m], ((size_t)n + 1) * 8, hipMemcpyHostToDevice));
        if (ql[m]) { HIP_TRY(b->d_hist_qual[m].reserve(bytes + 256)); HIP_TRY(hipMemcpy(b->d_hist_qual[m], ql[m], bytes, hipMemcpyHostToDevice)); }
    }
    b->n_hist = n; b->leak_meta_valid = false;
    return BSX_OK;
}

extern "C" int bsx_batch_pool_sizes(const bsx_batch *b, uint32_t *units_per_round, uint32_t *task_pool)
{
    if (!b) return BSX_ERR_ARG;
    if (units_per_round) *units_per_round = b->hcap;
    if (task_pool) *task_pool = b->task_cap;
    return BSX_OK;
}

extern "C" int bsx_batch_set_debug(bsx_batch *b, int keep)
{
    if (!b) return BSX_ERR_ARG;
    HIP_TRY(hipSetDevice(b->ref->device));
    b->debug = keep == 1 ? 1 : 0;
    if (keep == 2) HIP_TRY(b->d_cycles.reserve((size_t)b->max_units * 4));
    if (keep == 0) b->d_cycles.reset();
    if (keep == 1) HIP_TRY(b->d_dbg.reserve((size_t)b->max_units * 128));
    BatchPlan pl;
    const int rc = plan_on_device(b, pl);
    return rc ? rc : ensure_scratch(b, pl);
}

static int leak_prepare(bsx_batch *b, AlignArgs &A)
{
    const uint32_t cap = b->max_units + 65536u, nblk = cap / bsx_leak_blk() + 2;
    if (!b->d_leak_meta[0]) {
        for (int m = 0; m < (b->paired ? 2 : 1); m++) HIP_TRY(b->d_leak_meta[m].reserve((size_t)cap * 2));
        HIP_TRY(b->d_leak_blk.reserve((size_t)nblk * 16));
        HIP_TRY(b->d_leak_final.reserve(bsx_leakstate_bytes()));
        HIP_TRY(b->d_leak_rec.reserve((size_t)b->max_units * 2 * bsx_leakrec_bytes()));
        b->leak_nblk = nblk;
    }
    for (int m = 0; m < 2; m++) { A.leak_meta[m] = b->d_leak_meta[m]; A.leak_blkmax[m] = b->d_leak_blk + (size_t)m * nblk; A.leak_blkset[m] = b->d_leak_blk + (size_t)(2 + m) * nblk; }
    A.leak_init = b->leak_has_init ? b->d_leak_init.p : nullptr;
    A.leak_rec = b->d_leak_rec;
    A.n_units_all = b->n_units;
    A.n_hist = b->n_hist;
    if (!b->leak_meta_valid) HIP_TRY(hipMemsetAsync(b->d_leak_blk, 0, (size_t)nblk * 16, b->stream));
    return BSX_OK;
}

static void fill_args(bsx_batch *b, AlignArgs &A)
{
    memset(&A, 0, sizeof(A));
    bsx_fill_devparams(b->ref, A.P);
    A.first_index = b->first_index; A.debug = b->debug; A.rowcap = b->rowcap; A.kcap = b->kcap; A.hbits = hset_bits(b->ref->P);
    A.hkcap = b->hkcap; A.hhbits = BSX_HSET_BITS; A.hslab_bytes = b->hslab_bytes;
    A.redo_count = b->d_redo; A.redo_list = b->d_redo + 1; A.unit_list = nullptr;
    for (int m = 0; m < 2; m++) {
        A.seq[m] = b->d_seq[m]; A.off[m] = b->d_off[m]; A.qual[m] = b->has_qual ? b->d_qual[m].p : nullptr; A.cc[m] = b->d_cc[m];
        A.hist_seq[m] = b->d_hist_seq[m]; A.hist_off[m] = b->d_hist_off[m]; A.hist_qual[m] = b->d_hist_qual[m];
    }
    A.hits_out = b->d_hits; A.pairs_out = b->d_pairs; A.npairs_out = b->d_npairs;
    A.scratch = b->d_scratch; A.slab_bytes = b->slab_bytes; A.queue = b->d_queue; A.counters = b->d_counters; A.scan_stats = b->d_scan_stats; A.work_counters = (uint32_t)b->work_counters;
    A.dbg_plan = b->d_dbg; A.dbg_cycles = b->d_cycles; A.dbg_cat = b->d_cycles ? b->d_counters + 24 : nullptr;
    A.heavy_list = b->d_heavy_list; A.heavy_count = b->d_heavy_count;
    A.leak_exact = b->leak_exact; A.n_hist = b->leak_exact ? b->n_hist : 0; A.n_units_all = b->n_units;
    A.heavy_threshold = heavy_threshold_for(b->ref->P);
}

extern "C" int bsx_batch_set_leak_state(bsx_batch *b, const void *state, size_t bytes)
{
    if (!b || (state && bytes != bsx_leakstate_bytes())) return BSX_ERR_ARG;
    HIP_TRY(hipSetDevice(b->ref->device));
    HIP_TRY(stream_wait(b));
    if (!state) { b->leak_has_init = false; return BSX_OK; }
    HIP_TRY(b->d_leak_init.reserve(bsx_leakstate_bytes()));
    HIP_TRY(hipMemcpy(b->d_leak_init, state, bytes, hipMemcpyHostToDevice));
    b->leak_has_init = true;
    return BSX_OK;
}

extern "C" int bsx_batch_get_leak_state(bsx_batch *b, void *state, size_t bytes)
{
    if (!b || !state || bytes != bsx_leakstate_bytes()) return BSX_ERR_ARG;
    if (b->n_units == 0) return BSX_ERR_STATE;
    if (b->ref->P.rrbs) { memset(state, 0, bytes); return BSX_OK; }
    HIP_TRY(hipSetDevice(b->ref->device));
    AlignArgs A;
    fill_args(b, A);
    A.n_units = b->n_units; A.first_unit = 0;
    int rc = leak_prepare(b, A);
    if (rc) return rc;
    bsx_launch_leak(A, b->paired, b->n_cu, !b->leak_meta_valid, false, b->d_leak_final, b->stream);
    HIP_TRY(hipGetLastError());
    b->leak_meta_valid = true;
    HIP_TRY(hipMemcpyAsync(state, b->d_leak_final, bytes, hipMemcpyDeviceToHost, b->stream));
    HIP_TRY(stream_wait(b));
    return BSX_OK;
}

namespace {
struct HeavyRound {
    bsx_batch *b;
    const AlignArgs &A;
    const AllHitsArgs *ah;
    uint32_t base;
    int n_open = 0;
    struct GroupState { uint32_t n0 = 0, passes = 0, polls = 0, polled = 0; int cur = 0; bool done = true, tail = false; HeavyArgsRaw H; uint32_t *blk[2]; } G[BSX_MAX_GROUPS];

    int enqueue_pass(int g);
    int enqueue_chunk();
    int poll();
    int run_round(uint32_t n_round);
};

int HeavyRound::enqueue_pass(int g)
{
    GroupState &q = G[g];
    bsx_batch::Group &hw = b->grp[g];
    uint32_t *in = q.blk[q.cur], *out = q.blk[q.cur ^ 1];
    const bool fresh = q.passes == 0;
    if (fresh) {
        HIP_TRY(hipStreamWaitEvent(hw.s_ctrl, b->ev_sync, 0));
        HIP_TRY(hipMemsetAsync(out, 0, (size_t)BSX_HCNT_BLOCK * 4, hw.s_ctrl));
    } else HIP_TRY(hipStreamWaitEvent(hw.s_ctrl, hw.ev_scan, 0));
    q.H.active_in = b->pool.hactive[q.cur] + q.H.hidx_base; q.H.active_out = b->pool.hactive[q.cur ^ 1] + q.H.hidx_base;
    q.H.n_active_in_ptr = in; q.H.n_active_in = q.n0; q.H.n_active_out = out; q.H.n_tasks = out + BSX_HCNT_TASKS; q.H.queue = out + BSX_HCNT_QUEUE;
    q.H.fresh = fresh ? 1 : 0;
    if (b->stage_timing) {
        int rc = grow_events(b->ctrl_ev, b->ctrl_ev_used + 3);
        if (rc) return rc;
        HIP_TRY(hipEventRecord(b->ctrl_ev[b->ctrl_ev_used], hw.s_ctrl));
    }
    bsx_launch_hctrl(A, q.H, b->paired, (int)std::min<uint32_t>((q.n0 + 3) / 4, (uint32_t)b->n_cu * b->hctrl_blocks_per_cu), hw.s_ctrl, ah);
    HIP_TRY(hipGetLastError());
    if (b->stage_timing) HIP_TRY(hipEventRecord(b->ctrl_ev[b->ctrl_ev_used + 1], hw.s_ctrl));
    q.H.order = hw.d_order; q.H.xcd_map = b->K.xcd_map; q.H.ghead = hw.d_rank; q.H.glist = hw.d_glist;
    bsx_launch_task_order(q.H, b->bin_shift, b->n_bins, hw.d_bins, hw.d_bstart, hw.d_chunk_tot, hw.d_rank, hw.d_order, in, hw.s_ctrl, b->spread, b->same_kernel, b->K.same_d, b->K.same_r,
                          b->K.group_tile, b->K.group_big);
    if (b->stage_timing) { HIP_TRY(hipEventRecord(b->ctrl_ev[b->ctrl_ev_used + 2], hw.s_ctrl)); b->ctrl_ev_used += 3; }
    if (b->K.sig_hist) bsx_sig_hist_pass(q.H, hw.s_ctrl, b->same_kernel, b->K.group_tile);
    hipStream_t s_scan = b->stream;
    if (q.tail) s_scan = hw.s_ctrl;
    else {
        HIP_TRY(hipEventRecord(hw.ev_ctrl, hw.s_ctrl));
        HIP_TRY(hipStreamWaitEvent(b->stream, hw.ev_ctrl, 0));
    }
    { int rc = grow_events(b->scan_ev, b->scan_ev_used + 2); if (rc) return rc; }
    HIP_TRY(hipEventRecord(b->scan_ev[b->scan_ev_used], s_scan));
    if (b->same_kernel) bsx_launch_hscan_same(A, q.H, s_scan, q.tail ? b->K.tail_grid_tasks : 0);
    else if (b->ref->P.rrbs) bsx_launch_hscan_shared(A, q.H, s_scan, q.tail ? b->K.tail_grid_tasks : 0);
    else bsx_launch_hscan(A, q.H, s_scan, q.tail ? b->K.tail_grid_tasks : 0);
    HIP_TRY(hipGetLastError());
    if (b->K.sector_stats) bsx_sector_pass(b->ref, s_scan);
    HIP_TRY(hipEventRecord(b->scan_ev[b->scan_ev_used + 1], s_scan));
    b->scan_ev_used += 2;
    HIP_TRY(hipEventRecord(hw.ev_scan, s_scan));
    q.cur ^= 1; q.passes++;
    b->last_heavy_iters++;
    return BSX_OK;
}

int HeavyRound::enqueue_chunk()
{
    const int n_groups = b->K.n_groups;
    for (int k = 0; k < b->K.chunk_passes; k++)
        for (int g = 0; g < n_groups; g++)
            if (!G[g].done) { int rc = enqueue_pass(g); if (rc) return rc; }
    for (int g = 0; g < n_groups; g++) {
        GroupState &q = G[g];
        if (q.done) continue;
        const uint32_t slot = q.polls % BSX_POLL_SLOTS;
        HIP_TRY(hipMemcpyAsync(b->h_pinned + 32 + 16 * g + 2 * slot, q.blk[q.cur], 4, hipMemcpyDeviceToHost, b->grp[g].s_ctrl));
        HIP_TRY(hipMemcpyAsync(b->h_pinned + 32 + 16 * g + 2 * slot + 1, q.blk[q.cur] + BSX_HCNT_TASKS, 4, hipMemcpyDeviceToHost, b->grp[g].s_ctrl));
        HIP_TRY(hipEventRecord(b->grp[g].ev_poll[slot], b->grp[g].s_ctrl));
        q.polls++;
    }
    return BSX_OK;
}

int HeavyRound::poll()
{
    volatile uint32_t *pinned = (volatile uint32_t *)b->h_pinned;
    for (int g = 0; g < b->K.n_groups; g++) {
        GroupState &q = G[g];
        if (q.done) continue;
        const uint32_t slot = q.polled % BSX_POLL_SLOTS;
        HIP_TRY(wait_event(b->grp[g].ev_poll[slot]));
        const uint32_t n_act = pinned[32 + 16 * g + 2 * slot], n_tasks = pinned[32 + 16 * g + 2 * slot + 1];
        q.polled++;
        if (b->K.trace) fprintf(stderr, "[bsx heavy] paired %d base %u group %d passes %u active %u tasks %u\n", b->paired, base, g, q.polled * b->K.chunk_passes, n_act, n_tasks);
        if (n_act == 0) { q.done = true; n_open--; }
        else {
            if (q.passes > 200000) { g_bsx_err = "heavy pipeline did not converge"; return BSX_ERR_DEVICE; }
            if (b->K.tail_tasks && n_tasks < b->K.tail_tasks) q.tail = true;
        }
    }
    return BSX_OK;
}

int HeavyRound::run_round(uint32_t n_round)
{
    const int n_groups = b->K.n_groups;
    HIP_TRY(hipEventRecord(b->ev_sync, b->stream));
    for (int g = 0; g < n_groups; g++) {
        GroupState &q = G[g];
        const uint32_t lo = (uint32_t)((uint64_t)n_round * g / n_groups), hi = (uint32_t)((uint64_t)n_round * (g + 1) / n_groups);
        q.n0 = hi - lo; q.done = q.n0 == 0;
        memset(&q.H, 0, sizeof(q.H));
        const uint32_t tcap = b->task_cap / n_groups, toff = tcap * g;
        q.H.state = b->pool.hstate; q.H.slabs = b->pool.hslabs;
        q.H.tasks = b->pool.htasks + (size_t)toff * bsx_htask_bytes(); q.H.tout = b->pool.htout + (size_t)toff * bsx_htaskout_bytes();
        q.H.task_cap = tcap; q.H.list_base = base; q.H.hidx_base = lo;
        q.blk[0] = b->d_hcnt + (size_t)(2 * g) * BSX_HCNT_BLOCK; q.blk[1] = b->d_hcnt + (size_t)(2 * g + 1) * BSX_HCNT_BLOCK;
        if (!q.done) n_open++;
    }
    for (int depth = 0; depth < 2; depth++) { int rc = enqueue_chunk(); if (rc) return rc; }
    while (n_open > 0) {
        int rc = poll();
        if (rc == BSX_OK && n_open > 0) rc = enqueue_chunk();
        if (rc) return rc;
    }
    for (int g = 0; g < n_groups; g++) {
        if (G[g].passes == 0) continue;
        HIP_TRY(hipEventRecord(b->grp[g].ev_ctrl, b->grp[g].s_ctrl));
        HIP_TRY(hipStreamWaitEvent(b->stream, b->grp[g].ev_ctrl, 0));
    }
    return BSX_OK;
}
}

static int run_heavy(bsx_batch *b, const AlignArgs &A, const AllHitsArgs *ah)
{
    HIP_TRY(hipMemcpyAsync(b->h_pinned, b->d_heavy_count, 4, hipMemcpyDeviceToHost, b->stream));
    HIP_TRY(stream_wait(b));
    const uint32_t n_heavy = b->h_pinned[0];
    b->last_heavy = n_heavy;
    const uint32_t n_rounds = (n_heavy + b->hcap - 1) / b->hcap, per_round = n_rounds ? (n_heavy + n_rounds - 1) / n_rounds : 0;
    for (uint32_t base = 0; base < n_heavy; base += per_round) {
        HeavyRound round{b, A, ah, base};
        const int rc = round.run_round(std::min(per_round, n_heavy - base));
        if (rc) return rc;
    }
    return BSX_OK;
}

static int run_redo(bsx_batch *b, const AlignArgs &A, const AllHitsArgs *ah)
{
    HIP_TRY(hipMemcpyAsync(b->h_pinned, b->d_redo, 4, hipMemcpyDeviceToHost, b->stream));
    HIP_TRY(stream_wait(b));
    const uint32_t n_redo = b->h_pinned[0];
    b->last_redo = n_redo;
    if (!n_redo) return BSX_OK;
    AlignArgs R = A;
    R.unit_list = b->d_redo + 1; R.first_unit = 0; R.n_units = n_redo; R.heavy_threshold = 0;
    HIP_TRY(hipMemsetAsync(b->d_queue, 0, 4, b->stream));
    bsx_launch_align(R, b->paired, std::min<int>(b->grid_blocks, (int)((n_redo + 3) / 4)), b->stream, ah);
    HIP_TRY(hipGetLastError());
    return BSX_OK;
}

extern "C" int bsx_batch_run(bsx_batch *b) { return b ? bsx_batch_run_range(b, 0, b->n_units) : BSX_ERR_ARG; }

extern "C" int bsx_batch_run_range(bsx_batch *b, uint32_t first_unit, uint32_t n_units)
{
    if (!b) return BSX_ERR_ARG;
    if (b->n_units == 0) return BSX_ERR_STATE;
    if (n_units == 0 || (uint64_t)first_unit + n_units > b->n_units) return BSX_ERR_ARG;
    HIP_TRY(hipSetDevice(b->ref->device));
    AlignArgs A;
    fill_args(b, A);
    A.n_units = first_unit + n_units; A.first_unit = first_unit;
    HIP_TRY(hipMemsetAsync(b->d_queue, 0, 4, b->stream));
    HIP_TRY(hipMemsetAsync(b->d_heavy_count, 0, 4, b->stream));
    HIP_TRY(hipMemsetAsync(b->d_redo, 0, 4, b->stream));
    b->run_first = first_unit; b->run_units = n_units;
    AllHitsArgs X;
    const AllHitsArgs *ah = b->d_ah_pool ? &X : nullptr;
    if (ah) {
        X.pool = b->d_ah_pool; X.cap = b->ah_cap; X.cursor = (unsigned long long *)b->d_ah_ctl.p; X.dropped = (uint32_t *)(b->d_ah_ctl + 1); X.spans = b->d_ah_spans;
        HIP_TRY(hipMemsetAsync(b->d_ah_ctl, 0, 16, b->stream));
        HIP_TRY(hipMemsetAsync(b->d_ah_spans + (size_t)first_unit * 3, 0, (size_t)n_units * 3 * sizeof(bsx_span), b->stream));
    }
    if (b->debug) HIP_TRY(hipMemsetAsync(b->d_scratch, 0, (size_t)b->max_units * b->slab_bytes, b->stream));
    HIP_TRY(hipEventRecord(b->ev0, b->stream));
    if (b->leak_exact && !b->ref->P.rrbs) {
        int rc = leak_prepare(b, A);
        if (rc) return rc;
        bsx_launch_leak(A, b->paired, b->n_cu, !b->leak_meta_valid, true, nullptr, b->stream);
        HIP_TRY(hipGetLastError());
        b->leak_meta_valid = true;
    }
    bsx_launch_align(A, b->paired, b->grid_blocks, b->stream, ah);
    HIP_TRY(hipGetLastError());
// ... 338 lines not shown
```

### bsmap_amd/csrc/bsx_groups.h

```cpp
#pragma once
#include <hip/hip_runtime.h>
#include <stdint.h>

__host__ __device__ inline uint32_t bsx_group_cut(const uint32_t *off, uint32_t stride, uint32_t n, uint32_t D, uint32_t Rg, uint32_t *head, uint32_t hstride)
{
    if (Rg == 0) Rg = 1;
    uint32_t groups = 0;
    for (uint32_t p = 0; p < n; groups++) {
        const uint32_t frame = off[(size_t)p * stride];
        uint32_t lo = p + 1, hi = n;
        while (lo < hi) {
            const uint32_t mid = lo + ((hi - lo) >> 1);
            if (off[(size_t)mid * stride] - frame <= 32u * D) lo = mid + 1; else hi = mid;
        }
        const uint32_t N = lo - p, G = (N + Rg - 1u) / Rg, k = (N + G - 1u) / G;
        head[(size_t)p * hstride] = k;
        for (uint32_t j = 1; j < k; j++) head[(size_t)(p + j) * hstride] = 0;
        p += k;
    }
    return groups;
}
```

### bsmap_amd/csrc/bsx_kernel_args.h

```cpp
#pragma once
#include "bsx_internal.h"

struct AlignArgs {
    DevParams P;
    uint32_t n_units, first_index;
    uint32_t first_unit;
    int32_t debug;
    uint32_t rowcap;
    uint32_t kcap, hbits;
    uint32_t hkcap, hhbits;
    uint64_t hslab_bytes;
    uint32_t *redo_list, *redo_count;
    const uint32_t *unit_list;
    const uint8_t *seq[2];
    const uint64_t *off[2];
    const uint8_t *qual[2];
    bsx_hit *hits_out;
    bsx_pair *pairs_out;
    bsx_class_counts *cc[2];
    uint16_t *npairs_out;
    uint8_t *scratch;
    uint64_t slab_bytes;
    uint32_t work_counters;
    uint32_t heavy_threshold;
    uint32_t *heavy_list;
    uint32_t *heavy_count;
    uint32_t *queue;
    uint64_t *counters;
    uint64_t *scan_stats;
    uint32_t *dbg_cycles;
    uint64_t *dbg_cat;
    uint8_t *dbg_plan;
    int32_t leak_exact;
    const uint8_t *leak_rec;
    uint32_t n_hist;
    uint32_t n_units_all;
    uint16_t *leak_meta[2];
    uint32_t *leak_blkmax[2], *leak_blkset[2];
    const void *leak_init;
    const uint8_t *hist_seq[2];
    const uint64_t *hist_off[2];
    const uint8_t *hist_qual[2];
};

struct AllHitsArgs {
    uint32_t *pool;
    uint64_t cap;
    unsigned long long *cursor;
    uint32_t *dropped;
    bsx_span *spans;
};

#ifndef BSX_HCNT_TASKS
#define BSX_HCNT_TASKS 1088u
#define BSX_HCNT_QUEUE 2176u
#endif
#define BSX_HCNT_BLOCK 3072u
#ifndef BSX_HCTRL_BATCH
#define BSX_HCTRL_BATCH 1
#endif

struct HeavyArgsRaw {
    uint8_t *state;
    uint8_t *slabs;
    uint32_t *active_in, *active_out, *n_active_out;
    uint8_t *tasks, *tout;
    uint32_t *n_tasks;
    uint32_t *queue;
    const uint32_t *n_active_in_ptr;
    uint32_t n_active_in, task_cap, fresh, list_base, hidx_base;
    const uint32_t *order;
    uint32_t xcd_map;
    const uint32_t *ghead;
    uint32_t *glist;
};

void bsx_launch_align(const AlignArgs &A, int paired, int grid_blocks, hipStream_t stream, const AllHitsArgs *ah = nullptr);
void bsx_launch_align_ah(const AlignArgs &A, int paired, int grid_blocks, hipStream_t stream, const AllHitsArgs &X);
void bsx_launch_hctrl_ah(const AlignArgs &A, const HeavyArgsRaw &H, int paired, int grid_blocks, hipStream_t stream, const AllHitsArgs &X);
void bsx_launch_leak(const AlignArgs &A, int paired, int n_cu, bool with_meta, bool resolve, void *final_out, hipStream_t stream);
size_t bsx_leakrec_bytes(void);
size_t bsx_leakstate_bytes(void);
uint32_t bsx_leak_blk(void);
void bsx_launch_hctrl(const AlignArgs &A, const HeavyArgsRaw &H, int paired, int grid_blocks, hipStream_t stream, const AllHitsArgs *ah = nullptr);
void bsx_launch_hscan(const AlignArgs &A, const HeavyArgsRaw &H, hipStream_t stream, uint32_t max_tasks = 0);
void bsx_launch_hscan_same(const AlignArgs &A, const HeavyArgsRaw &H, hipStream_t stream, uint32_t max_tasks = 0);
void bsx_launch_hscan_shared(const AlignArgs &A, const HeavyArgsRaw &H, hipStream_t stream, uint32_t max_tasks = 0);
uint32_t bsx_bin_chunks(uint32_t n_bins);
void bsx_launch_task_order(const HeavyArgsRaw &H, uint32_t shift, uint32_t n_bins, uint32_t *bins, uint32_t *bstart, uint32_t *chunk_tot, uint32_t *rank, uint32_t *order,
                           uint32_t *zero_blk, hipStream_t stream, uint32_t spread = 0, bool groups = false, uint32_t same_d = 0, uint32_t same_r = 0, uint32_t tile = 0, uint32_t big = 0);
uint32_t bsx_same_d_max(void);
uint32_t bsx_same_r_max(void);
void bsx_sig_hist_pass(const HeavyArgsRaw &H, hipStream_t stream, bool groups = false, uint32_t tile = 0);
bool bsx_sig_group_stats(unsigned long long st[4]);
uint32_t bsx_group_tile(uint32_t tile);
void bsx_sig_hist_report(void);
void bsx_sector_pass(const bsx_ref *r, hipStream_t stream);
void bsx_sector_report(void);
size_t bsx_hstate_bytes(void);
size_t bsx_htask_bytes(void);
size_t bsx_htaskout_bytes(void);
int bsx_align_occupancy(int paired);
int bsx_hctrl_occupancy(int paired);
```

### bsmap_amd/csrc/bsx_rows.h

```cpp
#pragma once
#include <stdint.h>
#if defined(__HIPCC__)
#include <hip/hip_runtime.h>
#define BSX_ROWS_HD __host__ __device__
#else
#define BSX_ROWS_HD
#endif

#define BSX_ROW_DWORDS 20
#define BSX_ROW_TASK 16
#define BSX_ROW_ORD 17

BSX_ROWS_HD inline int bsx_row_eval_word(int i) { return i == 0 ? 0 : 5 - i; }

BSX_ROWS_HD inline void bsx_row_pack(uint32_t *row, const uint32_t *px, const uint32_t *py, const uint32_t *pm, uint32_t t)
{
    row[0] = px[0]; row[1] = py[0]; row[2] = pm[0]; row[3] = t;
    row[4] = px[4]; row[5] = py[4]; row[6] = pm[4]; row[7] = pm[1];
    row[8] = px[3]; row[9] = py[3]; row[10] = pm[3]; row[11] = px[2];
    row[12] = py[2]; row[13] = pm[2]; row[14] = px[1]; row[15] = py[1];
}

template <class Q> BSX_ROWS_HD inline uint32_t bsx_row_t(const Q &q0) { return q0.w; }

template <class Q> BSX_ROWS_HD inline void bsx_row_word(int i, const Q &q0, const Q &q1, const Q &q2, const Q &q3, uint32_t &X, uint32_t &Y, uint32_t &M)
{
    switch (i) {
    case 0: X = q0.x; Y = q0.y; M = q0.z; break;
    case 1: X = q1.x; Y = q1.y; M = q1.z; break;
    case 2: X = q2.x; Y = q2.y; M = q2.z; break;
    case 3: X = q2.w; Y = q3.x; M = q3.y; break;
    default: X = q3.z; Y = q3.w; M = q1.w; break;
    }
}

BSX_ROWS_HD inline uint32_t bsx_rows_exit_model(int mode, const uint8_t (*cnt)[64][5], const uint64_t *valid, uint32_t thr, uint64_t *keep)
{
    uint32_t words = 0, tot[4][64];
    uint64_t al[4];
    for (int u = 0; u < 4; u++) { al[u] = valid[u]; for (int l = 0; l < 64; l++) tot[u][l] = 0; }
    if (mode == 3 && (valid[0] & valid[1] & valid[2] & valid[3]) == ~0ull) {
        for (int i = 0; i < 5; i++) {
            bool any = false;
            for (int l = 0; l < 64; l++) {
                uint32_t mn = 0xffffffffu;
                for (int u = 0; u < 4; u++) { tot[u][l] += cnt[u][l][i]; if (tot[u][l] < mn) mn = tot[u][l]; }
                any = any || mn <= thr;
            }
            words += 4;
            if (!any) { for (int u = 0; u < 4; u++) keep[u] = 0; return words; }
        }
        for (int u = 0; u < 4; u++) { keep[u] = 0; for (int l = 0; l < 64; l++) if (tot[u][l] <= thr) keep[u] |= 1ull << l; }
        return words;
    }
    if (mode == 3) mode = 2;
    for (int a = 0; a < (mode ? 5 : 4); a++) {
        if (mode && !(al[0] | al[1] | al[2] | al[3])) break;
        for (int b = 0; b < (mode ? 4 : 5); b++) {
            const int i = mode ? a : b, u = mode ? b : a;
            if (!al[u] && mode != 2) continue;
            uint64_t m = 0;
            for (int l = 0; l < 64; l++) { tot[u][l] += cnt[u][l][i]; if (tot[u][l] <= thr) m |= 1ull << l; }
            al[u] &= m;
            words++;
        }
    }
    for (int u = 0; u < 4; u++) keep[u] = al[u];
    return words;
}
```

Measured before the change: 49.90 million reads/s.

## Group heavy-scan tasks across sub-word offsets by shifting read patterns

Allows tasks whose hit positions differ by a sub-word offset (up to BSX_SAME_S bits, default 31) to share one group in the same-window scan. Each read's pattern planes are pre-shifted by the offset so one gathered reference frame serves more reads, and the survivor position adds the offset back. Task grouping gains a second sorting pass with slack-aware membership for 144 bp-ish reads. The aim is fewer reference gathers per read, at the cost of more complex grouping kernels, possible extra padding lanes, and a larger risk of correctness issues.

```diff
diff --git a/bsmap_amd/csrc/bsx_align.hip b/bsmap_amd/csrc/bsx_align.hip
--- a/bsmap_amd/csrc/bsx_align.hip
+++ b/bsmap_amd/csrc/bsx_align.hip
@@ -3,6 +3,10 @@
 #include "bsx_groups.h"
 #include "bsx_rows.h"
 #include "bsx_kernel_args.h"
+#include <algorithm>
+#include <cstring>
+#include <thread>
+#include <vector>
 
 namespace {
 
@@ -2461,7 +2465,7 @@
 template <bool PLAIN, bool FULL, bool SPLIT, int JOINT>
 __device__ __forceinline__ void hs_eval_lean(const HeavyArgs &H, const uint32_t (&flo)[HG_C][5], const uint32_t (&fhi)[HG_C][5], const u64 (&vm)[HG_C], const uint32_t (&hloc)[HG_C],
                                              const uint4 &q0, const uint4 &q1, const uint4 &p2, const uint4 &p3, const uint4 *row, uint32_t thr, uint32_t k, uint32_t tid, uint32_t &nsv,
-                                             int lane, uint32_t cb, uint32_t dcur, uint32_t strand, uint32_t &dgw)
+                                             int lane, uint32_t cb, uint32_t pdel, uint32_t strand, uint32_t &dgw)
 {
     u64 al[HG_C];
     uint32_t tot[HG_C];
@@ -2524,7 +2528,7 @@
         if (bp) {
             const uint32_t pos = __builtin_amdgcn_mbcnt_hi((uint32_t)(bp >> 32), __builtin_amdgcn_mbcnt_lo((uint32_t)bp, nsk));
             if (__builtin_amdgcn_inverse_ballot_w64(bp) && pos < HS_SCAP) {
-                SurvRec r; r.w_ord = tot[u] | ((cb + (uint32_t)(u * 64 + lane)) << 8); r.hchr = strand; r.hloc = hloc[u] + 32u * dcur; r.hkey = 0; sv[pos] = r;
+                SurvRec r; r.w_ord = tot[u] | ((cb + (uint32_t)(u * 64 + lane)) << 8); r.hchr = strand; r.hloc = hloc[u] + pdel; r.hkey = 0; sv[pos] = r;
             }
             nsk += (uint32_t)__builtin_popcountll(bp);
         }
@@ -2534,15 +2538,17 @@
 
 template <int NWR, bool RRBS, bool STATS>
 __device__ __forceinline__ void hs_group(const AlignArgs &A, const HeavyArgs &H, SameLds &L, int lane, int wv, uint32_t K, uint32_t tid, uint32_t th, uint32_t tc0,
-                                         uint32_t key, uint32_t n, uint32_t hh, uint32_t sub_h, uint32_t flags, uint32_t tag_xor, uint32_t tag_want)
+                                         uint32_t key, uint32_t n, uint32_t hh, uint32_t sub_h, uint32_t flags, uint32_t tag_xor, uint32_t tag_want, uint32_t Kstat = 0)
 {
     const DevParams &P = A.P;
     uint32_t *uw = &L.W[wv].UW[0][0];
+    if (!Kstat) Kstat = K;
     const int nwr = NWR ? NWR : (int)((flags >> 8) & 15u);
     constexpr int XD = (!RRBS && NWR == 5) ? HG_D : 0, XP = XD;
     static_assert(HG_D >= 0 && HG_D <= 2 && 6 + HG_D <= BSX_PLANE_PAD, "the gather holds two pairs more at most, and stays inside the pad behind the strand copy");
     constexpr bool LEAN = HG_LEAN && HG_EXIT == 15 && NWR == 5 && !RRBS && !STATS, SPLIT = LEAN && HG_SPLIT;
     static_assert(BSX_ROW_DWORDS == 20 && sizeof(L.W[0].UW[0]) == 4 * BSX_ROW_DWORDS, "bsx_rows.h describes a row of SameLds");
+    static_assert(!XD || LEAN || STATS, "groups across sub-word offsets need hs_eval_lean (HG_LEAN = 1, HG_EXIT = 15) where the work counters are off: build with BSX_SAME_S=0 groups only, or add s to the position in hs_eval_read's survivor arm");
 #ifdef BSX_SIGHIST_DUPS
     u64 rowsig = 0;
 #endif
@@ -2555,15 +2561,18 @@
         const ListReq &R = H.state[th & 0x3fffffffu].req[th >> 30];
         uint32_t *row = uw + (uint32_t)lane * 20u;
         uint32_t inner = 0xFFFFFFFFu;
+        const uint32_t sdel = XD ? (sub_h - hh) & 31u : 0u;
+        uint32_t sx[5], sy[5], sm[5];
+        bsx_row_shift(R.px, R.py, R.pm, sdel, sx, sy, sm);
 #pragma unroll
         for (int j = 0; j < 5; j++) {
             const int f = 3 * j, o = j < 3 ? 0 : 1;
-            const uint32_t pm = R.pm[j];
-            if (!SPLIT) { row[f + o] = R.px[j]; row[f + 1 + o] = R.py[j]; row[f + 2 + o] = pm; }
+            const uint32_t pm = sm[j];
+            if (!SPLIT) { row[f + o] = sx[j]; row[f + 1 + o] = sy[j]; row[f + 2 + o] = pm; }
             if (j < nwr - 1) inner &= pm;
         }
-        const uint32_t tword = R.thres | (inner == 0xFFFFFFFFu ? 0x10000u : 0u) | (XD ? ((sub_h - hh) >> 5) << 17 : 0u);
-        if (SPLIT) bsx_row_pack(row, R.px, R.py, R.pm, tword);
+        const uint32_t tword = R.thres | (inner == 0xFFFFFFFFu ? 0x10000u : 0u) | (XD ? ((sub_h - hh) >> 5) << 17 | sdel << 24 : 0u);
+        if (SPLIT) bsx_row_pack(row, sx, sy, sm, tword);
         else row[9] = tword;
         row[BSX_ROW_TASK] = tid; row[BSX_ROW_ORD] = tc0;
 #ifdef BSX_SIGHIST_DUPS
@@ -2666,7 +2675,7 @@
                 if (!SPLIT) { q0 = row[0]; q1 = row[1]; p2 = row[2]; p3 = row[3]; }
                 const uint32_t tp = rfl(SPLIT ? bsx_row_t(q0) : p2.y), thr = tp & 0xffffu;
                 const bool plain = ((tp >> 16) & 1u) != 0;
-                for (; dcur < (tp >> 17); dcur++) {
+                for (; dcur < ((tp >> 17) & 127u); dcur++) {
 #pragma unroll
                     for (int u = 0; u < HG_C; u++) {
 #pragma unroll
@@ -2677,12 +2686,13 @@
                     }
                 }
                 uint32_t dgw = 0;
+                const uint32_t pdel = 32u * dcur + (tp >> 24);
                 if (full) {
-                    if (plain) hs_eval_lean<true, true, SPLIT, HG_JOINT>(H, flo, fhi, vm, hloc, q0, q1, p2, p3, row, thr, k, tid, nsv, lane, cb, dcur, strand, dgw);
-                    else hs_eval_lean<false, true, SPLIT, HG_JOINT>(H, flo, fhi, vm, hloc, q0, q1, p2, p3, row, thr, k, tid, nsv, lane, cb, dcur, strand, dgw);
+                    if (plain) hs_eval_lean<true, true, SPLIT, HG_JOINT>(H, flo, fhi, vm, hloc, q0, q1, p2, p3, row, thr, k, tid, nsv, lane, cb, pdel, strand, dgw);
+                    else hs_eval_lean<false, true, SPLIT, HG_JOINT>(H, flo, fhi, vm, hloc, q0, q1, p2, p3, row, thr, k, tid, nsv, lane, cb, pdel, strand, dgw);
                 } else {
-                    if (plain) hs_eval_lean<true, false, SPLIT, HG_JOINT>(H, flo, fhi, vm, hloc, q0, q1, p2, p3, row, thr, k, tid, nsv, lane, cb, dcur, strand, dgw);
-                    else hs_eval_lean<false, false, SPLIT, HG_JOINT>(H, flo, fhi, vm, hloc, q0, q1, p2, p3, row, thr, k, tid, nsv, lane, cb, dcur, strand, dgw);
+                    if (plain) hs_eval_lean<true, false, SPLIT, HG_JOINT>(H, flo, fhi, vm, hloc, q0, q1, p2, p3, row, thr, k, tid, nsv, lane, cb, pdel, strand, dgw);
+                    else hs_eval_lean<false, false, SPLIT, HG_JOINT>(H, flo, fhi, vm, hloc, q0, q1, p2, p3, row, thr, k, tid, nsv, lane, cb, pdel, strand, dgw);
                 }
 #ifdef BSX_SCAN_WORDS
                 dg_ev += dgw & 0xffffu; dg_words += dgw >> 16;
@@ -2716,7 +2726,7 @@
             const uint32_t tp = rfl(a2.y), thr = tp & 0xffffu;
             const bool plain = NWR != 0 && ((tp >> 16) & 1u) != 0;
             if (XD) {
-                for (; dcur < (tp >> 17); dcur++) {
+                for (; dcur < ((tp >> 17) & 127u); dcur++) {
 #pragma unroll
                     for (int u = 0; u < HG_C; u++) {
 #pragma unroll
@@ -2765,9 +2775,9 @@
         u64 *sh = (u64 *)A.scan_stats + (size_t)((blockIdx.x * (uint32_t)HG_WPB + (uint32_t)wv) & 63u) * 8;
         atomicAdd((u64 *)&sh[0], (u64)kk * n_cand);
         if (STATS) { atomicAdd((u64 *)&sh[1], 2ull * kk * n_cand - s1 + 3ull * s5); atomicAdd((u64 *)&sh[2], (u64)s1); atomicAdd((u64 *)&sh[3], (u64)s5); }
-        if (K > 1) atomicAdd((u64 *)&sh[4], (u64)kk * n_cand);
+        if (Kstat > 1) atomicAdd((u64 *)&sh[4], (u64)kk * n_cand);
 #if !defined(BSX_SCAN_WORDS) && !defined(BSX_SCAN_CLOCKS)
-        atomicAdd((u64 *)&sh[5], (u64)kk * n_cand * K); if (K >= 4) atomicAdd((u64 *)&sh[6], (u64)kk * n_cand); if (n_dup) atomicAdd((u64 *)&sh[7], (u64)n_dup * n_cand);
+        atomicAdd((u64 *)&sh[5], (u64)kk * n_cand * Kstat); if (Kstat >= 4) atomicAdd((u64 *)&sh[6], (u64)kk * n_cand); if (n_dup) atomicAdd((u64 *)&sh[7], (u64)n_dup * n_cand);
 #endif
     }
 #ifdef BSX_SCAN_WORDS
@@ -2792,7 +2802,9 @@
     const int lane = threadIdx.x & 63, wv = (int)rfl(threadIdx.x >> 6);
     const uint32_t n_big = min(H.glist[H.task_cap], H.task_cap), n_groups = min(n_big + H.glist[H.task_cap + 1], H.task_cap);
     const uint32_t nvb = (n_groups + HG_WPB - 1) / HG_WPB;
-    for (uint32_t vb = blockIdx.x;; vb += gridDim.x) {
+    static_assert(!STATS || HG_WPB == 1, "rem is a wave's, vb a block's: with more waves per block the waves would disagree on whether the block moves on");
+    u64 rem = 0;
+    for (uint32_t vb = blockIdx.x;; vb += (STATS && rem) ? 0u : gridDim.x) {
         uint32_t b_;
         const int st_ = bsx_order_block(vb, nvb, H.xcd_map >= 2 ? max(2u, H.xcd_map * BSX_HSCAN_WPB / (HG_XCD_DIV * HG_WPB)) : H.xcd_map, b_);
         if (st_ == 2) break;
@@ -2808,6 +2820,20 @@
             th = tk.h; tc0 = tk.c0; tn = tk.n; key = tk.key; hh = tk.sub_h; flags = tk.flags; tx = tk.pad[0]; tw = tk.pad[1];
         }
         const uint32_t n0 = rfl(tn), f0 = rfl(flags);
+        uint32_t Kc = K;
+        if constexpr (STATS) {
+            if (n0 != 0 && !(f0 & 4u) && K > 1 && ((f0 >> 8) & 15u) == 5u) {
+                if (!rem) rem = bsx_ballot((uint32_t)lane < K);
+                const uint32_t sd = (hh - rfl(hh)) & 31u, s0 = rl_u(sd, (uint32_t)__builtin_ctzll(rem));
+                const bool in = ((rem >> lane) & 1ull) != 0 && sd == s0;
+                const u64 m = bsx_ballot(in);
+                rem &= ~m;
+                Kc = (uint32_t)__builtin_popcountll(m);
+                const int dst = (int)((in ? (uint32_t)__builtin_popcountll(m & lanemask_lt(lane)) : Kc + (uint32_t)__builtin_popcountll(~m & lanemask_lt(lane))) << 2);
+                tid = (uint32_t)__builtin_amdgcn_ds_permute(dst, (int)tid); th = (uint32_t)__builtin_amdgcn_ds_permute(dst, (int)th);
+                tc0 = (uint32_t)__builtin_amdgcn_ds_permute(dst, (int)tc0); hh = (uint32_t)__builtin_amdgcn_ds_permute(dst, (int)hh);
+            }
+        }
         if (n0 == 0) {
             if ((uint32_t)lane < K) { HTaskOut *o = &H.tout[tid]; o->count = 0; o->overflow = 0; o->acc[0] = o->acc[1] = o->acc[2] = o->acc[3] = 0; o->c0 = 0; o->n = 0; }
         } else if (f0 & 4u) {
@@ -2815,7 +2841,7 @@
             else hs_group<0, true, STATS>(A, H, L, lane, wv, K, tid, th, tc0, rfl(key), n0, rfl(hh), hh, f0, rfl(tx), rfl(tw));
         }
         else if (K > 1) {
-            if (((f0 >> 8) & 15u) == 5u) hs_group<5, false, STATS>(A, H, L, lane, wv, K, tid, th, tc0, rfl(key), n0, rfl(hh), hh, f0, 0u, 0u);
+            if (((f0 >> 8) & 15u) == 5u) hs_group<5, false, STATS>(A, H, L, lane, wv, Kc, tid, th, tc0, rfl(key), n0, rfl(hh), hh, f0, 0u, 0u, K);
             else if (((f0 >> 8) & 15u) == 4u) hs_group<4, false, STATS>(A, H, L, lane, wv, K, tid, th, tc0, rfl(key), n0, rfl(hh), hh, f0, 0u, 0u);
             else hs_group<0, false, STATS>(A, H, L, lane, wv, K, tid, th, tc0, rfl(key), n0, rfl(hh), hh, f0, 0u, 0u);
         }
@@ -2836,39 +2862,48 @@
     if (a.z != b.z) return a.z < b.z;
     return a.w < b.w;
 }
-__device__ __forceinline__ bool tg_same_run(const HTask &a, const HTask &b)
+__device__ __forceinline__ bool tg_same_run(const HTask &a, const HTask &b, bool any)
 {
     if (a.n == 0 || b.n == 0) return a.n == b.n;
-    return (a.flags & 2u) && a.flags == b.flags && a.key == b.key && a.n == b.n && a.pad[0] == b.pad[0] && a.pad[1] == b.pad[1] && ((a.sub_h ^ b.sub_h) & 31u) == 0;
-}
-__global__ __launch_bounds__(256) void k_task_groups(const HTask *tasks, const uint32_t *n_tasks_ptr, uint32_t cap, uint32_t *order, uint32_t *ghead, uint32_t *glist, uint32_t D, uint32_t Rg,
-                                                     uint32_t T, uint32_t big)
-{
+    return (a.flags & 2u) && a.flags == b.flags && a.key == b.key && a.n == b.n && a.pad[0] == b.pad[0] && a.pad[1] == b.pad[1] && (any || ((a.sub_h ^ b.sub_h) & 31u) == 0);
+}
+__device__ __forceinline__ bool tg_wide(const HTask &tk) { return tk.n != 0 && (tk.flags & 2u) && !(tk.flags & 4u) && ((tk.flags >> 8) & 15u) == 5u; }
+template <bool SUB>
+__global__ __launch_bounds__(256) void k_task_groups(const HTask *tasks, const HState *state, const uint32_t *n_tasks_ptr, uint32_t cap, uint32_t *order, uint32_t *ghead, uint32_t *glist, uint32_t D, uint32_t S_,
+                                                     uint32_t Rg, uint32_t T, uint32_t big, uint32_t split)
+{
+    const uint32_t S = SUB ? S_ : 0u;
     extern __shared__ uint4 tg_lds[];
     uint4 *K = tg_lds;
     uint32_t *head = (uint32_t *)(K + T);
-    u64 *brk = (u64 *)(head + T);
-    uint32_t *cnt = (uint32_t *)(brk + HG_TILE_MAX / 64u);
+    uint32_t *perm = head + T;
+    uint32_t *slk = perm + T;
+    u64 *brk = (u64 *)(SUB ? slk + T : head + T);
+    u64 *sbrk = brk + HG_TILE_MAX / 64u;
+    uint32_t *cnt = (uint32_t *)(sbrk + HG_TILE_MAX / 64u);
     const int lane = threadIdx.x & 63;
     const uint32_t wv = threadIdx.x >> 6, n_ch = T >> 6;
     const uint32_t n_tasks = min(*n_tasks_ptr, cap);
     for (uint32_t s0 = blockIdx.x * T; s0 < n_tasks; s0 += gridDim.x * T) {
         const uint32_t nj = min(T, n_tasks - s0);
+        bool anyw = false;
         for (uint32_t i = threadIdx.x; i < T; i += 256u) {
             uint4 k = make_uint4(0xffffffffu, 0xffffffffu, 0xffffffffu, 0xffffffffu);
             if (i < nj) {
                 const uint32_t tid = order[s0 + i];
                 const HTask tk = tasks[tid];
+                if (split) anyw = anyw || tg_wide(tk);
                 if (tk.n == 0) k = make_uint4(0xffffffffu, 0xfffffffeu, 0u, tid);
                 else {
                     uint32_t hs = tk.n * 0x9E3779B1u ^ tk.flags * 0x85EBCA6Bu ^ tk.pad[0] * 0xC2B2AE35u ^ tk.pad[1] * 0x27D4EB2Fu;
                     hs ^= hs >> 15; hs *= 0x2C1B3C6Du; hs ^= hs >> 13;
-                    k = make_uint4(tk.key, (hs & ~31u) | (tk.sub_h & 31u), tk.sub_h ^ 0x80000000u, tid);
+                    k = make_uint4(tk.key, (hs & ~31u) | (S && tg_wide(tk) ? 0u : tk.sub_h & 31u), tk.sub_h ^ 0x80000000u, tid);
                 }
             }
             K[i] = k;
         }
-        __syncthreads();
+        if (split) { if ((__syncthreads_or(anyw) != 0) != SUB) continue; }
+        else __syncthreads();
         for (uint32_t kk = 2; kk <= T; kk <<= 1)
             for (uint32_t j = kk >> 1; j; j >>= 1) {
                 for (uint32_t t = threadIdx.x; t < (T >> 1); t += 256u) {
@@ -2888,16 +2923,20 @@
             if (i < nj) {
                 const uint4 k = K[i];
                 const HTask tk = tasks[k.w];
+                const bool wide = tg_wide(tk);
                 start = true;
                 if (i) {
                     const uint4 kp = K[i - 1u];
-                    if (kp.x == k.x && kp.y == k.y) start = !tg_same_run(tasks[kp.w], tk);
+                    if (kp.x == k.x && kp.y == k.y) start = !tg_same_run(tasks[kp.w], tk, S && wide);
                 }
+                uint32_t sl = 0;
+                if (S && wide) { const uint32_t len = state[tk.h & 0x3fffffffu].req[tk.h >> 30].len; sl = len >= 129u && len <= 160u ? 160u - len : 0u; }
+                if (SUB) { slk[i] = sl; perm[i] = i; }
                 const uint32_t Dg = (!(tk.flags & 4u) && ((tk.flags >> 8) & 15u) == 5u) ? D : 0u;
-                if (start) info[m] = 1u | (tk.n == 0 ? 64u << 8 : !(tk.flags & 2u) ? 1u << 8 : Dg << 1 | Rg << 8);
-            }
-            const u64 bm = bsx_ballot(start);
-            if (lane == 0) brk[c] = bm;
+                if (start) info[m] = 1u | (tk.n == 0 ? 64u << 8 : !(tk.flags & 2u) ? 1u << 8 : Dg << 1 | Rg << 8 | (wide ? S << 16 : 0u));
+            }
+            const u64 bm = bsx_ballot(start), sbm = bsx_ballot(info[m] >> 16 != 0);
+            if (lane == 0) { brk[c] = bm; sbrk[c] = sbm; }
         }
         __syncthreads();
 #pragma unroll
@@ -2908,12 +2947,50 @@
             u64 w = brk[c] & ~((2ull << (i & 63u)) - 1ull);
             while (!w && ++c < n_ch) w = brk[c];
             const uint32_t e = w ? c * 64u + (uint32_t)__builtin_ctzll(w) : nj;
-            bsx_group_cut(&K[i].z, 4u, e - i, (info[m] >> 1) & 127u, info[m] >> 8, head + i, 1u);
-        }
+            if (!(info[m] >> 16)) bsx_group_cut(&K[i].z, 4u, e - i, (info[m] >> 1) & 127u, (info[m] >> 8) & 255u, head + i, 1u);
+        }
+        if (S)
+            for (uint32_t c0 = wv; c0 < n_ch; c0 += 4u)
+                for (u64 sb = sbrk[c0]; sb; sb &= sb - 1ull) {
+                    const uint32_t i = c0 * 64u + (uint32_t)__builtin_ctzll(sb);
+                    uint32_t c = c0;
+                    u64 w = brk[c] & ~((2ull << (i & 63u)) - 1ull);
+                    while (!w && ++c < n_ch) w = brk[c];
+                    const uint32_t e = w ? c * 64u + (uint32_t)__builtin_ctzll(w) : nj, reach = 32u * D + S;
+                    for (uint32_t p = i, q = i; p < e;) {
+                        const uint32_t frame = K[p].z;
+                        uint32_t N = 0;
+                        for (uint32_t base = p; base < e; base += 64u) {
+                            const uint32_t j = base + (uint32_t)lane, delta = j < e ? K[j].z - frame : 0xffffffffu;
+                            const uint32_t sl = j < e ? slk[j] : 0x80000000u;
+                            N += (uint32_t)__builtin_popcountll(bsx_ballot(delta <= reach && !(sl >> 31) && bsx_sub_member(delta, sl, D, S)));
+                            if (!(bsx_ballot(delta <= reach) >> 63)) break;
+                        }
+                        const uint32_t G = (N + Rg - 1u) / Rg, k = (N + G - 1u) / G;
+                        for (uint32_t base = p, t = 0; t < k; base += 64u) {
+                            const uint32_t j = base + (uint32_t)lane, delta = j < e ? K[j].z - frame : 0xffffffffu;
+                            const uint32_t sl = j < e ? slk[j] : 0x80000000u;
+                            const bool mem = delta <= reach && !(sl >> 31) && bsx_sub_member(delta, sl, D, S);
+                            const u64 bm = bsx_ballot(mem);
+                            const uint32_t r = t + (uint32_t)__builtin_popcountll(bm & lanemask_lt(lane));
+                            if (mem && r < k) { slk[j] = sl | 0x80000000u; perm[q + r] = j; head[q + r] = r ? 0u : k; }
+                            t += (uint32_t)__builtin_popcountll(bm);
+                        }
+                        q += k;
+                        wave_fence();
+                        for (;;) {
+                            const uint32_t j = p + (uint32_t)lane;
+                            const u64 pend = bsx_ballot(j < e && !(slk[j] >> 31));
+                            if (pend) { p += (uint32_t)__builtin_ctzll(pend); break; }
+                            p += 64u;
+                            if (p >= e) { p = e; break; }
+                        }
+                    }
+                }
         __syncthreads();
         for (uint32_t c = wv; c < n_ch; c += 4u) {
             const uint32_t i = c * 64u + (uint32_t)lane, hd = i < nj ? head[i] : 0u;
-            if (i < nj) { order[s0 + i] = K[i].w; ghead[s0 + i] = hd; }
+            if (i < nj) { order[s0 + i] = K[SUB ? perm[i] : i].w; ghead[s0 + i] = hd; }
             const u64 hb = bsx_ballot(hd >= big), hsm = bsx_ballot(hd != 0 && hd < big);
             if (lane == 0) { cnt[c] = (uint32_t)__builtin_popcountll(hb); cnt[32u + c] = (uint32_t)__builtin_popcountll(hsm); }
         }
@@ -3282,8 +3359,9 @@
     if (spread && (tk.flags & 2u)) {
         const uint32_t span = tk.n >> shift;
         const uint32_t nb = span >= 16u ? 16u : span >= 8u ? 8u : span >= 4u ? 4u : span >= 2u ? 2u : 1u;
-        const bool congruent = spread == 2u && !(tk.flags & 4u) && ((tk.flags >> 8) & 15u) == 5u;
-        bin += (((congruent ? tk.sub_h & 31u : tk.sub_h) * 0x9E3779B1u) >> 28) & (nb - 1u);
+        const bool wide = spread >= 2u && !(tk.flags & 4u) && ((tk.flags >> 8) & 15u) == 5u, congruent = wide && spread == 2u;
+        const uint32_t quad = (((tk.sub_h + 3u) & 15u) >> 2) + tk.key * 0x85EBCA6Bu;
+        bin += (((congruent ? tk.sub_h & 31u : wide ? quad : tk.sub_h) * 0x9E3779B1u) >> 28) & (nb - 1u);
     }
     return min(bin, n_bins - 1u);
 }
@@ -3377,7 +3455,7 @@
 uint32_t bsx_bin_chunks(uint32_t n_bins) { return (n_bins + BIN_CHUNK - 1) / BIN_CHUNK; }
 
 void bsx_launch_task_order(const HeavyArgsRaw &R, uint32_t shift, uint32_t n_bins, uint32_t *bins, uint32_t *bstart, uint32_t *chunk_tot, uint32_t *rank, uint32_t *order,
-                           uint32_t *zero_blk, hipStream_t stream, uint32_t spread, bool groups, uint32_t same_d, uint32_t same_r, uint32_t tile, uint32_t big)
+                           uint32_t *zero_blk, hipStream_t stream, uint32_t spread, bool groups, uint32_t same_d, uint32_t same_r, uint32_t tile, uint32_t big, uint32_t same_s)
 {
     const uint32_t grid = std::max(1u, std::min(512u, (R.task_cap + 255u) / 256u)), n_chunks = bsx_bin_chunks(n_bins);
     hipLaunchKernelGGL(k_task_bins, dim3(std::max(1u, std::min(256u, (R.task_cap + 1023u) / 1024u))), dim3(256), 0, stream, (const HTask *)R.tasks, R.n_tasks, R.task_cap, shift, n_bins, spread, bins, rank, zero_blk);
@@ -3385,9 +3463,13 @@
     hipLaunchKernelGGL(k_task_order, dim3(grid), dim3(256), 0, stream, (const HTask *)R.tasks, R.n_tasks, R.task_cap, shift, n_bins, spread, bstart, chunk_tot, n_chunks, rank, order);
     if (groups) {
         const uint32_t T = bsx_group_tile(tile);
-        const size_t lds = (size_t)T * 20u + HG_TILE_MAX / 64u * 8u + 64u * 4u;
-        hipLaunchKernelGGL(k_task_groups, dim3(std::max(1u, std::min(1024u, (R.task_cap + T - 1u) / T))), dim3(256), lds, stream, (const HTask *)R.tasks, R.n_tasks, R.task_cap, order, rank, R.glist,
-                           std::min<uint32_t>(same_d, HG_D), same_r ? std::min<uint32_t>(same_r, HG_R) : HG_R, T, big ? std::min<uint32_t>(big, HG_R + 1u) : HG_BIG);
+        const uint32_t S = same_d ? std::min<uint32_t>(same_s, 31u) : 0u, D = std::min<uint32_t>(same_d, HG_D), Rg = same_r ? std::min<uint32_t>(same_r, HG_R) : HG_R, bg = big ? std::min<uint32_t>(big, HG_R + 1u) : HG_BIG;
+        const dim3 tg_grid(std::max(1u, std::min(1024u, (R.task_cap + T - 1u) / T)));
+        hipLaunchKernelGGL(k_task_groups<false>, tg_grid, dim3(256), (size_t)T * 20u + HG_TILE_MAX / 64u * 16u + 64u * 4u, stream, (const HTask *)R.tasks, (const HState *)R.state, R.n_tasks, R.task_cap, order, rank,
+                           R.glist, D, 0u, Rg, T, bg, S ? 1u : 0u);
+        if (S)
+            hipLaunchKernelGGL(k_task_groups<true>, tg_grid, dim3(256), (size_t)T * 28u + HG_TILE_MAX / 64u * 16u + 64u * 4u, stream, (const HTask *)R.tasks, (const HState *)R.state, R.n_tasks, R.task_cap, order, rank,
+                               R.glist, D, S, Rg, T, bg, 1u);
     }
 }
 
@@ -3506,9 +3588,133 @@
 const int SIG_KINDS = 5;
 unsigned long long *g_sig_tab = nullptr, *g_sig_hist = nullptr;
 const uint32_t SIG_SLOTS = 1u << 23;
-}
-
-void bsx_sig_hist_pass(const HeavyArgsRaw &R, hipStream_t stream, bool groups, uint32_t tile)
+
+struct SigxRec { uint32_t key, n, flags, pad0, pad1, off, slk; };
+__global__ __launch_bounds__(256) void k_sigx_pack(const HTask *tasks, const HState *state, uint32_t n, SigxRec *out)
+{
+    for (uint32_t i = blockIdx.x * 256 + threadIdx.x; i < n; i += gridDim.x * 256) {
+        const HTask tk = tasks[i];
+        SigxRec r = {tk.key, tk.n, tk.flags, tk.pad[0], tk.pad[1], tk.sub_h ^ 0x80000000u, 0u};
+        if (tk.n && (tk.flags & 2u) && !(tk.flags & 4u) && ((tk.flags >> 8) & 15u) == 5u) {
+            const uint32_t len = state[tk.h & 0x3fffffffu].req[tk.h >> 30].len;
+            r.slk = 0x100u | (len >= 129u && len <= 160u ? 160u - len : 0u);
+        }
+        out[i] = r;
+    }
+}
+struct SigxAcc { unsigned long long cand[32], tasks[32], ev, ch; };
+SigxAcc g_sigx[2][3];
+bool g_sigx_any = false;
+SigxRec *g_sigx_dev = nullptr;
+size_t g_sigx_cap = 0;
+inline bool sigx_less(const SigxRec &a, const SigxRec &b)
+{
+    if (a.key != b.key) return a.key < b.key;
+    if (a.n != b.n) return a.n < b.n;
+    if (a.flags != b.flags) return a.flags < b.flags;
+    if (a.pad0 != b.pad0) return a.pad0 < b.pad0;
+    if (a.pad1 != b.pad1) return a.pad1 < b.pad1;
+    return a.off < b.off;
+}
+inline bool sigx_same_window(const SigxRec &a, const SigxRec &b) { return a.key == b.key && a.n == b.n && a.flags == b.flags && a.pad0 == b.pad0 && a.pad1 == b.pad1; }
+void sigx_cut_range(const SigxRec *v, size_t lo, size_t hi, uint32_t D, uint32_t Rg, uint32_t T, SigxAcc acc[2][3])
+{
+    std::vector<uint32_t> slk, perm, head, setn;
+    for (int tiled = 0; tiled < 2; tiled++)
+        for (size_t i = lo; i < hi;) {
+            size_t e = i + 1;
+            while (e < hi && sigx_same_window(v[i], v[e]) && !(tiled && e % T == 0)) e++;
+            const uint32_t n = (uint32_t)(e - i), cand = v[i].n;
+            const bool inside = (v[i].flags & 2u) != 0, shifts = (v[i].slk & 0x100u) != 0;
+            slk.resize(n); perm.resize(n); head.resize(n); setn.resize(n);
+            for (uint32_t j = 0; j < n; j++) slk[j] = v[i + j].slk & 31u;
+            for (int rule = 0; rule < 3; rule++) {
+                SigxAcc &a = acc[tiled][rule];
+                if (!inside) {
+                    a.cand[31] += (unsigned long long)n * cand; a.tasks[31] += n; a.ev += (unsigned long long)n * cand; a.ch += (unsigned long long)n * ((cand + 63u) / 64u);
+                    continue;
+                }
+                bsx_group_cut_sub(&v[i].off, sizeof(SigxRec) / 4u, slk.data(), 1u, n, shifts && rule != 1 ? D : 0u, shifts && rule != 0 ? 31u : 0u, Rg, perm.data(), 1u, head.data(), 1u, setn.data());
+                for (uint32_t q = 0; q < n; q++) {
+                    const uint32_t k = head[q], N = setn[q];
+                    if (!k) continue;
+                    const uint32_t b = N <= 1 ? 0u : 32u - (uint32_t)__builtin_clz(N - 1u);
+                    a.cand[b] += (unsigned long long)k * cand; a.tasks[b] += k; a.ev += (unsigned long long)k * cand; a.ch += (cand + 63u) / 64u;
+                }
+            }
+            i = e;
+        }
+}
+void sigx_pass(const HeavyArgsRaw &R, hipStream_t stream, uint32_t D, uint32_t Rg, uint32_t T)
+{
+    uint32_t n = 0;
+    if (hipStreamSynchronize(stream) != hipSuccess || hipMemcpy(&n, R.n_tasks, 4, hipMemcpyDeviceToHost) != hipSuccess) return;
+    n = std::min(n, R.task_cap);
+    if (!n) return;
+    if (n > g_sigx_cap) {
+        if (g_sigx_dev) (void)hipFree(g_sigx_dev);
+        g_sigx_cap = 0;
+        if (hipMalloc((void **)&g_sigx_dev, (size_t)n * sizeof(SigxRec)) != hipSuccess) { g_sigx_dev = nullptr; return; }
+        g_sigx_cap = n;
+    }
+    hipLaunchKernelGGL(k_sigx_pack, dim3(1024), dim3(256), 0, stream, (const HTask *)R.tasks, (const HState *)R.state, n, g_sigx_dev);
+    std::vector<SigxRec> v(n);
+    if (hipStreamSynchronize(stream) != hipSuccess || hipMemcpy(v.data(), g_sigx_dev, (size_t)n * sizeof(SigxRec), hipMemcpyDeviceToHost) != hipSuccess) return;
+    v.erase(std::remove_if(v.begin(), v.end(), [](const SigxRec &r) { return r.n == 0; }), v.end());
+    constexpr size_t P = 8;
+    const size_t m = v.size();
+    size_t cut[P + 1];
+    for (size_t p = 0; p <= P; p++) cut[p] = m * p / P;
+    {
+        std::vector<std::thread> th;
+        for (size_t p = 0; p < P; p++) th.emplace_back([&, p] { std::sort(v.begin() + cut[p], v.begin() + cut[p + 1], sigx_less); });
+        for (auto &t : th) t.join();
+        for (size_t w = 1; w < P; w <<= 1) {
+            std::vector<std::thread> tm;
+            for (size_t p = 0; p + w < P; p += 2 * w) tm.emplace_back([&, p, w] { std::inplace_merge(v.begin() + cut[p], v.begin() + cut[p + w], v.begin() + cut[std::min(P, p + 2 * w)], sigx_less); });
+            for (auto &t : tm) t.join();
+        }
+    }
+    for (size_t p = 1; p < P; p++) {
+        size_t c = std::max(cut[p], cut[p - 1]);
+        while (c && c < m && sigx_same_window(v[c - 1], v[c])) c++;
+        cut[p] = c;
+    }
+    std::vector<std::thread> th;
+    static SigxAcc part[P][2][3];
+    memset(part, 0, sizeof part);
+    for (size_t p = 0; p < P; p++) th.emplace_back([&, p] { if (cut[p] < cut[p + 1]) sigx_cut_range(v.data(), cut[p], cut[p + 1], D, Rg, T, part[p]); });
+    for (auto &t : th) t.join();
+    for (size_t p = 0; p < P; p++)
+        for (int a = 0; a < 2; a++)
+            for (int r = 0; r < 3; r++) {
+                for (int k = 0; k < 32; k++) { g_sigx[a][r].cand[k] += part[p][a][r].cand[k]; g_sigx[a][r].tasks[k] += part[p][a][r].tasks[k]; }
+                g_sigx[a][r].ev += part[p][a][r].ev; g_sigx[a][r].ch += part[p][a][r].ch;
+            }
+    g_sigx_any = true;
+}
+void sigx_report(void)
+{
+    if (!g_sigx_any) return;
+    static const char *const rule_name[3] = {"P: offsets congruent mod 32, offset / 32 within D of the frame (today's groups)", "A: offset within 160 - L of the frame, no classes",
+                                             "B: offset / 32 within D of the frame and offset mod 32 within 160 - L"};
+    for (int tiled = 0; tiled < 2; tiled++)
+        for (int r = 0; r < 3; r++) {
+            const SigxAcc &a = g_sigx[tiled][r];
+            unsigned long long tot = 0, tt = 0;
+            for (int k = 0; k < 32; k++) { tot += a.cand[k]; tt += a.tasks[k]; }
+            fprintf(stderr, "[sighist] same window, %s; %s: candidates %llu tasks %llu, groups cut at the cap: reads per fetch %.2f (%llu evaluations, %llu group chunks)\n", rule_name[r],
+                    tiled ? "runs ended at the tile's multiples of the sorted pass" : "whole runs", tot, tt, (double)a.ev / (64.0 * (double)std::max(1ull, a.ch)), a.ev, a.ch);
+            for (int k = 0; k < 32; k++)
+                if (a.tasks[k])
+                    fprintf(stderr, "[sighist]   %s %-6u cand %.4f tasks %.4f\n", k == 31 ? "spanning" : "N <=", k == 31 ? 0u : 1u << k, (double)a.cand[k] / (double)std::max(1ull, tot), (double)a.tasks[k] / (double)std::max(1ull, tt));
+        }
+    memset(g_sigx, 0, sizeof g_sigx);
+    g_sigx_any = false;
+}
+}
+
+void bsx_sig_hist_pass(const HeavyArgsRaw &R, hipStream_t stream, bool groups, uint32_t tile, uint32_t same_d, uint32_t same_r)
 {
     if (!g_sig_tab) {
         if (hipMalloc((void **)&g_sig_tab, (size_t)SIG_SLOTS * 16) != hipSuccess || hipMalloc((void **)&g_sig_hist, (SIG_KINDS * 64 + 4) * 8) != hipSuccess) { g_sig_tab = nullptr; return; }
@@ -3531,6 +3737,7 @@
         (void)hipMemsetAsync(g_sig_tab, 0, (size_t)SIG_SLOTS * 16, stream);
         for (int pass = 0; pass < 2; pass++)
             hipLaunchKernelGGL(k_sigc_tiles, dim3(1024), dim3(256), 0, stream, (const HTask *)R.tasks, R.n_tasks, R.task_cap, R.order, g_sig_tab, SIG_SLOTS - 1, bsx_group_tile(tile), pass, g_sig_hist + 64 * SIG_KINDS);
+        sigx_pass(R, stream, std::min<uint32_t>(same_d, HG_D), same_r ? std::min<uint32_t>(same_r, HG_R) : HG_R, bsx_group_tile(tile));
     }
 }
 
@@ -3555,6 +3762,7 @@
                 fprintf(stderr, "[sighist]   %s %-6u cand %.4f tasks %.4f\n", k == 31 ? "spanning" : k == 30 && with_h >= 2 ? "beyond" : "R <=", k == 31 || (k == 30 && with_h >= 2) ? 0u : 1u << k, (double)h[64 * with_h + k] / (double)std::max(1ull, tot), (double)h[64 * with_h + 32 + k] / (double)std::max(1ull, tt));
     }
     (void)hipMemset(g_sig_hist, 0, (SIG_KINDS * 64 + 4) * 8);
+    sigx_report();
 }
 
 void bsx_sector_pass(const bsx_ref *r, hipStream_t stream)
diff --git a/bsmap_amd/csrc/bsx_api.hip b/bsmap_amd/csrc/bsx_api.hip
--- a/bsmap_amd/csrc/bsx_api.hip
+++ b/bsmap_amd/csrc/bsx_api.hip
@@ -244,7 +244,7 @@
 struct BatchKnobs {
     uint32_t kcap, heavy_kcap, bin_log2;
     int n_groups, chunk_passes, hctrl_blocks, same, work_counters;
-    uint32_t xcd_map, tail_tasks, tail_grid_tasks, same_d, same_r, group_tile, group_big, spread;
+    uint32_t xcd_map, tail_tasks, tail_grid_tasks, same_d, same_r, same_s, group_tile, group_big, spread;
     bool spread_set, trace, sig_hist, sector_stats, poison;
 };
 static long knob(const char *name, long dflt, long lo, long hi, bool *set = nullptr)
@@ -270,6 +270,7 @@
     K.tail_grid_tasks = (uint32_t)knob("BSX_TAIL_GRID", 4096, 64, any);
     K.same_d = (uint32_t)knob("BSX_SAME_D", (long)bsx_same_d_max(), 0, (long)bsx_same_d_max());
     K.same_r = (uint32_t)knob("BSX_SAME_R", (long)bsx_same_r_max(), 1, (long)bsx_same_r_max());
+    K.same_s = (uint32_t)knob("BSX_SAME_S", 31, 0, 31);
     K.group_tile = (uint32_t)knob("BSX_GROUP_TILE", none, 0, 0x7fffffffffffffffL);
     K.group_big = (uint32_t)knob("BSX_GROUP_BIG", none, 0, 0x7fffffffffffffffL);
     K.spread = (uint32_t)knob("BSX_SPREAD", none, -any - 1, any, &K.spread_set);
@@ -403,7 +404,7 @@
     b.slab_bytes = slab_size(P, b.paired, b.rowcap, b.kcap, hset_bits(P));
     b.hslab_bytes = slab_size(P, b.paired, b.rowcap, b.hkcap, BSX_HSET_BITS);
     b.same_kernel = P.rrbs ? b.K.same == 2 : b.K.same != 0;
-    b.spread = b.K.spread_set ? b.K.spread : (b.same_kernel ? (b.K.same_d ? 2u : 1u) : 0u);
+    b.spread = b.K.spread_set ? b.K.spread : (b.same_kernel ? (b.K.same_d ? (b.K.same_s ? 3u : 2u) : 1u) : 0u);
 }
 
 struct PlanRow {
@@ -856,9 +857,9 @@
     if (b->stage_timing) HIP_TRY(hipEventRecord(b->ctrl_ev[b->ctrl_ev_used + 1], hw.s_ctrl));
     q.H.order = hw.d_order; q.H.xcd_map = b->K.xcd_map; q.H.ghead = hw.d_rank; q.H.glist = hw.d_glist;
     bsx_launch_task_order(q.H, b->bin_shift, b->n_bins, hw.d_bins, hw.d_bstart, hw.d_chunk_tot, hw.d_rank, hw.d_order, in, hw.s_ctrl, b->spread, b->same_kernel, b->K.same_d, b->K.same_r,
-                          b->K.group_tile, b->K.group_big);
+                          b->K.group_tile, b->K.group_big, b->K.same_s);
     if (b->stage_timing) { HIP_TRY(hipEventRecord(b->ctrl_ev[b->ctrl_ev_used + 2], hw.s_ctrl)); b->ctrl_ev_used += 3; }
-    if (b->K.sig_hist) bsx_sig_hist_pass(q.H, hw.s_ctrl, b->same_kernel, b->K.group_tile);
+    if (b->K.sig_hist) bsx_sig_hist_pass(q.H, hw.s_ctrl, b->same_kernel, b->K.group_tile, b->K.same_d, b->K.same_r);
     hipStream_t s_scan = b->stream;
     if (q.tail) s_scan = hw.s_ctrl;
     else {
diff --git a/bsmap_amd/csrc/bsx_groups.h b/bsmap_amd/csrc/bsx_groups.h
--- a/bsmap_amd/csrc/bsx_groups.h
+++ b/bsmap_amd/csrc/bsx_groups.h
@@ -20,3 +20,36 @@
     }
     return groups;
 }
+
+__host__ __device__ inline bool bsx_sub_member(uint32_t delta, uint32_t slack, uint32_t D, uint32_t S)
+{
+    const uint32_t s = delta & 31u;
+    return (delta >> 5) <= D && s <= S && s <= slack;
+}
+__host__ __device__ inline uint32_t bsx_group_cut_sub(const uint32_t *off, uint32_t stride, const uint32_t *slk, uint32_t sstride, uint32_t n, uint32_t D, uint32_t S, uint32_t Rg,
+                                                      uint32_t *perm, uint32_t pstride, uint32_t *head, uint32_t hstride, uint32_t *setn)
+{
+    if (Rg == 0) Rg = 1;
+    if (S > 31u) S = 31u;
+    const uint32_t reach = 32u * D + S;
+    for (uint32_t i = 0; i < n; i++) perm[(size_t)i * pstride] = 0;
+    uint32_t groups = 0;
+    for (uint32_t p = 0, q = 0; p < n; groups++) {
+        const uint32_t frame = off[(size_t)p * stride];
+        uint32_t N = 0, e = p;
+        for (; e < n && off[(size_t)e * stride] - frame <= reach; e++)
+            if (!(perm[(size_t)e * pstride] >> 31) && bsx_sub_member(off[(size_t)e * stride] - frame, slk[(size_t)e * sstride], D, S)) N++;
+        const uint32_t G = (N + Rg - 1u) / Rg, k = (N + G - 1u) / G;
+        for (uint32_t j = p, t = 0; t < k; j++) {
+            if ((perm[(size_t)j * pstride] >> 31) || !bsx_sub_member(off[(size_t)j * stride] - frame, slk[(size_t)j * sstride], D, S)) continue;
+            perm[(size_t)j * pstride] |= 0x80000000u;
+            perm[(size_t)(q + t) * pstride] = (perm[(size_t)(q + t) * pstride] & 0x80000000u) | j;
+            head[(size_t)(q + t) * hstride] = t ? 0u : k;
+            if (setn) setn[(size_t)(q + t) * hstride] = t ? 0u : N;
+            t++;
+        }
+        q += k;
+        while (p < n && (perm[(size_t)p * pstride] >> 31)) p++;
+    }
+    return groups;
+}
diff --git a/bsmap_amd/csrc/bsx_kernel_args.h b/bsmap_amd/csrc/bsx_kernel_args.h
--- a/bsmap_amd/csrc/bsx_kernel_args.h
+++ b/bsmap_amd/csrc/bsx_kernel_args.h
@@ -88,10 +88,10 @@
 void bsx_launch_hscan_shared(const AlignArgs &A, const HeavyArgsRaw &H, hipStream_t stream, uint32_t max_tasks = 0);
 uint32_t bsx_bin_chunks(uint32_t n_bins);
 void bsx_launch_task_order(const HeavyArgsRaw &H, uint32_t shift, uint32_t n_bins, uint32_t *bins, uint32_t *bstart, uint32_t *chunk_tot, uint32_t *rank, uint32_t *order,
-                           uint32_t *zero_blk, hipStream_t stream, uint32_t spread = 0, bool groups = false, uint32_t same_d = 0, uint32_t same_r = 0, uint32_t tile = 0, uint32_t big = 0);
+                           uint32_t *zero_blk, hipStream_t stream, uint32_t spread = 0, bool groups = false, uint32_t same_d = 0, uint32_t same_r = 0, uint32_t tile = 0, uint32_t big = 0, uint32_t same_s = 0);
 uint32_t bsx_same_d_max(void);
 uint32_t bsx_same_r_max(void);
-void bsx_sig_hist_pass(const HeavyArgsRaw &H, hipStream_t stream, bool groups = false, uint32_t tile = 0);
+void bsx_sig_hist_pass(const HeavyArgsRaw &H, hipStream_t stream, bool groups = false, uint32_t tile = 0, uint32_t same_d = ~0u, uint32_t same_r = 0);
 bool bsx_sig_group_stats(unsigned long long st[4]);
 uint32_t bsx_group_tile(uint32_t tile);
 void bsx_sig_hist_report(void);
diff --git a/bsmap_amd/csrc/bsx_rows.h b/bsmap_amd/csrc/bsx_rows.h
--- a/bsmap_amd/csrc/bsx_rows.h
+++ b/bsmap_amd/csrc/bsx_rows.h
@@ -19,6 +19,16 @@
     row[4] = px[4]; row[5] = py[4]; row[6] = pm[4]; row[7] = pm[1];
     row[8] = px[3]; row[9] = py[3]; row[10] = pm[3]; row[11] = px[2];
     row[12] = py[2]; row[13] = pm[2]; row[14] = px[1]; row[15] = py[1];
+}
+
+BSX_ROWS_HD inline void bsx_row_shift(const uint32_t *px, const uint32_t *py, const uint32_t *pm, uint32_t s, uint32_t *sx, uint32_t *sy, uint32_t *sm)
+{
+    for (int j = 4; j >= 0; j--) {
+        const uint32_t ax = j ? px[j - 1] : 0u, ay = j ? py[j - 1] : 0u, am = j ? pm[j - 1] : 0u;
+        sx[j] = s ? (ax << (32u - s)) | (px[j] >> s) : px[j];
+        sy[j] = s ? (ay << (32u - s)) | (py[j] >> s) : py[j];
+        sm[j] = s ? (am << (32u - s)) | (pm[j] >> s) : pm[j];
+    }
 }
 
 template <class Q> BSX_ROWS_HD inline uint32_t bsx_row_t(const Q &q0) { return q0.w; }
```

Result: faster. 53.63 million reads/s, median of 6 (+7.5%).
